# rgl-epfl/large-steps-pytorch

Measured on AMD Instinct MI355X. Metric: from_differential_solves_per_sec, higher is better.
Workload: dtype f32; 1 GPU; cfg4_plane1m: 1000x1000 plane, V=1000000, nnz(M)=6992002, M=I+50*L_uniform, u=M v, k=3, factor once (not timed), re-solve timed; method=nested-dissection, device=AMD Radeon Graphics

## Files before the change

include/largesteps_hip.h:

```cpp
#ifndef LARGESTEPS_HIP_H
#define LARGESTEPS_HIP_H

#include <stddef.h>
#include <stdint.h>

#ifdef __cplusplus
extern "C" {
#endif

#define LS_VERSION 110

#define LS_OK 0
#define LS_E_INVALID (-1)
#define LS_E_INDEX (-2)
#define LS_E_WORKSPACE (-3)
#define LS_E_OVERFLOW (-4)
#define LS_E_STATE (-5)
#define LS_E_NOT_CONVERGED (-6)

#define LS_LAPLACIAN_UNIFORM 0
#define LS_LAPLACIAN_COT 1

int ls_version(void);
const char* ls_last_error(void);

int ls_assemble_workspace_bytes(int64_t V, int64_t F, size_t* h_bytes);
int ls_assemble_pattern(const void* faces, int idx_bytes, int64_t F, int64_t V, const float* verts,
                        int kind, float a, float b, void* workspace, size_t workspace_bytes,
                        int32_t* rowptr, int64_t* h_nnz, int device, void* stream);
int ls_assemble_fill(const void* workspace, size_t workspace_bytes, int64_t V, int64_t F, const int32_t* rowptr,
                     int32_t* col, float* val, int64_t* coo_idx, int64_t nnz, float* dinv, int device,
                     void* stream);

int ls_csr_from_coo(const int64_t* coo_rows, const int64_t* coo_cols, const float* vals, int64_t nnz,
                    int64_t V, int32_t* rowptr, int32_t* col, float* dinv, void* scratch,
                    size_t scratch_bytes, int device, void* stream);

int ls_spmv(const int32_t* rowptr, const int32_t* col, const float* val, int64_t V, int64_t nnz,
            const float* x, float* y, int k, int variant, int device, void* stream);

typedef struct ls_solver ls_solver;

typedef struct ls_solve_info {
    int32_t iterations;
    int32_t converged;
    double  rnorm[4];
    double  bnorm[4];
} ls_solve_info;

int ls_solver_create(const int32_t* rowptr, const int32_t* col, const float* val, int64_t V,
                     int64_t nnz, int kmax, int device, void* stream, ls_solver** h_out);
int ls_solver_destroy(ls_solver* s);
int ls_solver_solve(ls_solver* s, const float* b, const float* x0, float* x, int k, double rtol,
                    double atol, int max_iter, ls_solve_info* h_info, void* stream);
int ls_solver_set_spectrum(ls_solver* s, double a_min);
int ls_solver_set_uniform(ls_solver* s, float a, float b, void* stream);
int ls_solver_spectrum(const ls_solver* s, double* h_lmin, double* h_lmax);
int ls_solver_set_patches(ls_solver* s, const int32_t* h_table, int n_patches, const int32_t* h_ghost_gid, int64_t n_gid,
                          const uint16_t* h_cols16, int64_t n_cols, const float* h_diag, int64_t n_diag,
                          const int32_t* h_perm, int depth, int max_local, int max_rows, void* stream);
int ls_solver_chebyshev_iterations(const ls_solver* s, double reduction, int* h_n);
int ls_solver_solve_chebyshev(ls_solver* s, const float* b, const float* x0, float* x, int k, double rtol,
                              double atol, int max_iter, ls_solve_info* h_info, void* stream);
int ls_solver_set(ls_solver* s, const char* name, int value);
int ls_solver_profile(const ls_solver* s, double* h_ms3, int* h_iters);
int ls_solver_sell(ls_solver* s, const int32_t** h_slice_ptr, const void** h_cv, int64_t* h_entries);
int ls_solver_workspace_bytes(const ls_solver* s, size_t* h_bytes);

int ls_solver_create_ext(const int32_t* rowptr, const int32_t* col, const float* val, int64_t n_rows,
                         int64_t n_cols, int64_t nnz, int kmax, int device, void* stream, ls_solver** h_out);
int ls_solver_phase(ls_solver* s, int phase, const float* b, float* x, int k, double rtol, double atol,
                    int it, void* stream);
int ls_solver_buffers(ls_solver* s, float** h_p, double** h_part, int* h_grid, int* h_part_stride);
int ls_solver_bind(ls_solver* s, float* p_ext, double* part);
int ls_shard_cheb_steps(ls_solver* s, const float* b, float* xa, float* xb, int k, int it0, int nsteps,
                        const float* h_c1, const float* h_c2, int64_t n_rows, void* stream);
int ls_shard_resnorm(ls_solver* s, const float* b, const float* x, int k, int64_t n_rows, void* stream);
int ls_solver_poll(ls_solver* s, int k, int n_enqueued, ls_solve_info* h_info, void* stream);
int ls_gather_rows(const float* src, const int32_t* idx, int64_t n, int k, float* dst, int device, void* stream);

typedef struct ls_patch_plan ls_patch_plan;
int ls_patch_plan_create(int64_t V, const int32_t* h_rowptr, const int32_t* h_col, const float* h_diag, const float* h_positions,
                         int patch_size, int depth, int cap_local, int min_depth, int cap_rows, ls_patch_plan** out);
int ls_patch_plan_destroy(ls_patch_plan* p);
int ls_patch_plan_info(const ls_patch_plan* p, int* n_patches, int* depth, int* max_local, int* max_rows, int* max_width, int64_t* n_gid,
                       int64_t* n_cols, int64_t* n_diag, double* seconds);
int ls_patch_plan_arrays(const ls_patch_plan* p, int32_t* table, int32_t* ghost_gid, uint16_t* cols16, float* diag, int32_t* perm);

typedef struct ls_shard_plan ls_shard_plan;
int ls_shard_plan_create(int64_t V, const int32_t* h_rowptr, const int32_t* h_col, const float* h_val, int P, int rank, int depth,
                         ls_shard_plan** out);
int ls_shard_plan_destroy(ls_shard_plan* s);
int ls_shard_plan_info(const ls_shard_plan* s, int64_t* lo, int64_t* hi, int64_t* n_inner, int64_t* n_ghosts, int64_t* n_entries,
                       int* n_recv, int* n_send, int64_t* n_send_ids);
int ls_shard_plan_arrays(const ls_shard_plan* s, int32_t* rowptr, int32_t* col, float* val, int32_t* ghosts, int32_t* recv3,
                         int32_t* send_ptr, int32_t* send_dst, int32_t* send_ids);
int ls_shard_layer_sizes(int64_t V, const int32_t* h_rowptr, const int32_t* h_col, int64_t lo, int64_t hi, int depth, int64_t* h_sizes);

typedef struct ls_nd_plan ls_nd_plan;
int ls_nd_plan_create(int64_t V, const int32_t* h_rowptr, const int32_t* h_col, const float* h_positions, int leaf_size,
                      int arity, int smooth, ls_nd_plan** out);
int ls_nd_plan_create_device(const int32_t* d_rowptr, const int32_t* d_col, const float* d_positions, int64_t V, int64_t nnz,
                             int leaf_size, int arity, int smooth, int device, void* stream, ls_nd_plan** out);
#define LS_ND_ORDER_AUTO (-1)
#define LS_ND_ORDER_LONGEST 0
#define LS_ND_ORDER_MINSEP 1
int ls_nd_plan_create_ordered(int64_t V, const int32_t* h_rowptr, const int32_t* h_col, const float* h_positions, int leaf_size,
                              int arity, int smooth, int ordering, ls_nd_plan** out);
int ls_nd_plan_create_device_ordered(const int32_t* d_rowptr, const int32_t* d_col, const float* d_positions, int64_t V, int64_t nnz,
                                     int leaf_size, int arity, int smooth, int ordering, int device, void* stream, ls_nd_plan** out);
int ls_nd_plan_quality(const ls_nd_plan* p, int* h_ordering, double* h_words_per_vertex, double* h_spread, double* h_words_other);
int ls_nd_plan_destroy(ls_nd_plan* p);
int ls_nd_plan_info(const ls_nd_plan* p, int* levels, int* arity, int* n_nodes, int64_t* n_bnd, int64_t* n_front, double* seconds);
int ls_nd_plan_arrays(const ls_nd_plan* p, int32_t* perm, int32_t* s, int32_t* b, int32_t* own_start, int32_t* parent,
                      int32_t* bnd, int32_t* ppos, int32_t* push_ptr, int32_t* push_tgt);

typedef struct ls_direct ls_direct;
#define LS_DIRECT_NODE_COLS 12
typedef struct ls_direct_arrays {
    int64_t V;
    int32_t levels, arity;
    const int64_t* h_nodes;
    const int32_t* h_perm;
    const int32_t* h_ppos;
    int64_t n_bnd;
    const int32_t* h_push_ptr;
    const int32_t* h_push_tgt;
    int64_t n_front;
    const float* d_finv;
    const float* d_wf;
    const float* d_wb;
    const float* d_u4;
    const float* d_d4;
    const float* d_tri;
    const int32_t* d_sp_ptr;
    const void* d_sp_ent;
    int64_t n_sp_ptr, n_sp_ent;
    int32_t shard_rank, shard_count;
    int32_t tier_waves;
} ls_direct_arrays;
int ls_direct_create(const ls_direct_arrays* arrays, int device, void* stream, ls_direct** out);
int ls_direct_pick_tree(int64_t V, int* leaf_size, int* arity);
int ls_direct_tier_lds_bytes(int levels, int arity, const int32_t* h_s, const int32_t* h_b, const int32_t* h_own_start, int tier_levels,
                             int sparse_leaves, int waves, size_t* h_bytes);
int ls_direct_factor(const int32_t* d_rowptr, const int32_t* d_col, const float* d_val, int64_t V, int64_t nnz,
                     const float* d_positions, int leaf_size, int arity, int tier_levels, int sparse_leaves, int shard_rank,
                     int shard_count, int device, void* stream, ls_direct** out);
typedef struct ls_direct_options {
    int32_t struct_bytes;
    int32_t leaf_size, arity, tier_levels, sparse_leaves, shard_rank, shard_count;
    int32_t ordering;
    int32_t tier_waves;
} ls_direct_options;
int ls_direct_options_default(ls_direct_options* opt);
int ls_direct_factor_ex(const int32_t* d_rowptr, const int32_t* d_col, const float* d_val, int64_t V, int64_t nnz,
                        const float* d_positions, const ls_direct_options* opt, int device, void* stream, ls_direct** out);
int ls_direct_factor_refactorable(const int32_t* d_rowptr, const int32_t* d_col, const float* d_val, int64_t V, int64_t nnz,
                                  const float* d_positions, const ls_direct_options* opt, int device, void* stream, ls_direct** out);
int ls_direct_refactor(ls_direct* d, const int32_t* d_rowptr, const int32_t* d_col, const float* d_val, int64_t V, int64_t nnz,
                       void* stream);
int ls_direct_refactorable(const ls_direct* d, int* h_yes, size_t* h_retained_device_bytes);
int ls_release_scratch(int device);
int ls_direct_shape(const ls_direct* d, int* h_levels, int* h_arity, int* h_tier_levels, int* h_tier_workgroups,
                    int64_t* h_words_up, int64_t* h_words_down, int64_t* h_n_bnd);
int ls_direct_level_words(const ls_direct* d, int cap, int64_t* h_up, int64_t* h_down);
int ls_direct_level_rows(const ls_direct* d, int cap, int64_t* h_rows, int64_t* h_bnd);
int ls_direct_level_index_bytes(const ls_direct* d, int cap, int64_t* h_up, int64_t* h_down);
int ls_direct_tier_balance(const ls_direct* d, double* h_words4);
int ls_direct_launch_profile(const ls_direct* d, int cap, int* h_n, double* h_ms, int64_t* h_words, int32_t* h_level_lo,
                             int32_t* h_level_hi, int32_t* h_sweep);
int ls_direct_plan_quality(const ls_direct* d, int* h_ordering, double* h_words_per_vertex, double* h_spread, double* h_words_other);
int ls_direct_factor_seconds(const ls_direct* d, double* h_s3);
int ls_csr_is_symmetric(const int32_t* d_rowptr, const int32_t* d_col, const float* d_val, int64_t V, int64_t nnz, float tol,
                        int* h_symmetric, int device, void* stream);
int ls_direct_destroy(ls_direct* d);
int ls_direct_solve(ls_direct* d, const float* b, float* x, int k, void* stream);
int ls_direct_solve_part(ls_direct* d, const float* b, float* x, int k, int part, float* exchange, void* stream);
int ls_direct_shard_info(const ls_direct* d, int* h_rank, int* h_count, int* h_cut_level, int64_t* h_exchange_floats_per_column,
                         unsigned char* h_owned_rows);
int ls_direct_exchange_region(ls_direct* d, int k, float** h_region, int64_t* h_floats);

typedef struct ls_dist ls_dist;
int ls_dist_unique_id(void* h_id128);
int ls_dist_create(const void* h_id128, int rank, int world, int device, ls_dist** out);
int ls_dist_destroy(ls_dist* c);
int ls_dist_allreduce_sum(ls_dist* c, float* d_buf, int64_t n, void* stream);
int ls_dist_info(const ls_dist* c, int* h_rank, int* h_world);
int ls_dist_direct_solve(ls_dist* c, ls_direct* d, const float* b, float* x, int k, void* stream);
int ls_direct_set(ls_direct* d, const char* name, int value);
int ls_direct_info(const ls_direct* d, int64_t* h_factor_entries, int* h_launches, double* h_ms3);

int ls_remove_duplicates_workspace_bytes(int64_t V, size_t* h_bytes);
int ls_remove_duplicates(const float* verts, int64_t V, const void* faces, int idx_bytes, int64_t F, float* unique_verts,
                         int64_t* inverse, int64_t* new_faces, int64_t* h_n_unique, void* workspace, size_t ws_bytes, int device,
                         void* stream);

int ls_csr_transpose_workspace_bytes(int64_t V, int64_t nnz, size_t* h_bytes);
int ls_csr_transpose(const int32_t* rowptr, const int32_t* col, const float* val, int64_t V, int64_t nnz, int32_t* t_rowptr,
                     int32_t* t_col, float* t_val, void* workspace, size_t ws_bytes, int device, void* stream);
int ls_corner_ranks_workspace_bytes(int64_t F, int64_t V, size_t* h_bytes);
int ls_corner_ranks(const void* faces, int idx_bytes, int64_t F, int64_t V, int32_t* vptr, int32_t* cpos, void* workspace,
                    size_t ws_bytes, int device, void* stream);

int ls_normals_workspace_bytes(int64_t F, int64_t V, size_t* h_bytes);
int ls_face_normals(const float* verts, const void* faces, int idx_bytes, int64_t F, int64_t V, float* fn, int device, void* stream);
int ls_face_normals_backward(const float* verts, const void* faces, int idx_bytes, int64_t F, int64_t V, const int32_t* vptr,
                             const int32_t* cpos, const float* g_fn, float* grad_verts, void* workspace, size_t ws_bytes,
                             int device, void* stream);
int ls_vertex_normals(const float* verts, const void* faces, int idx_bytes, int64_t F, int64_t V, const int32_t* vptr,
                      const int32_t* cpos, const float* fn, float* out, float* raw, float* norms, void* workspace,
                      size_t ws_bytes, int device, void* stream);
int ls_vertex_normals_backward(const float* verts, const void* faces, int idx_bytes, int64_t F, int64_t V, const int32_t* vptr,
                               const int32_t* cpos, const float* fn, const float* raw, const float* norms, const float* g_out,
                               float* grad_verts, float* grad_fn, void* workspace, size_t ws_bytes, int device, void* stream);
int ls_face_normals_with_norms(const float* verts, const void* faces, int idx_bytes, int64_t F, int64_t V, float* fn, float* norms,
                               void* workspace, size_t ws_bytes, int device, void* stream);
int ls_vertex_normals_from_norms(const float* verts, const void* faces, int idx_bytes, int64_t F, int64_t V, const int32_t* vptr,
                                 const int32_t* cpos, const float* norms, float* out, float* raw, void* workspace, size_t ws_bytes,
                                 int device, void* stream);
int ls_vertex_normals_gathered(const float* verts, const void* faces, int idx_bytes, int64_t F, int64_t V, const int32_t* vptr,
                               const int32_t* order, const float* norms, float* out, float* raw, int device, void* stream);
int ls_normals_pair_backward_faces(const float* verts, const void* faces, int idx_bytes, int64_t F, int64_t V, const float* raw,
                                   const float* norms, const float* g_out, float* g_raw, float* gN, float* grad_fn, void* workspace,
                                   size_t ws_bytes, int device, void* stream);
int ls_normals_pair_backward_verts(const float* verts, const void* faces, int idx_bytes, int64_t F, int64_t V, const int32_t* vptr,
                                   const int32_t* cpos, const float* norms, const float* g_raw, const float* gN, const float* g_fn,
                                   float* grad_verts, void* workspace, size_t ws_bytes, int device, void* stream);

int ls_meshgeom_workspace_bytes(int64_t F, int64_t V, size_t* h_bytes);
int ls_massmatrix_voronoi(const float* verts, const void* faces, int idx_bytes, int64_t F, int64_t V, const int32_t* vptr,
                          const int32_t* order, float* mass, int device, void* stream);
int ls_massmatrix_voronoi_backward(const float* verts, const void* faces, int idx_bytes, int64_t F, int64_t V, const int32_t* vptr,
                                   const int32_t* cpos, const float* g_mass, float* grad_verts, void* workspace, size_t ws_bytes,
                                   int device, void* stream);
int ls_average_edge_length(const float* verts, const void* faces, int idx_bytes, int64_t F, int64_t V, float* out, void* workspace,
                           size_t ws_bytes, int device, void* stream);
int ls_average_edge_length_backward(const float* verts, const void* faces, int idx_bytes, int64_t F, int64_t V, const int32_t* vptr,
                                    const int32_t* cpos, const float* g_out, float* grad_verts, void* workspace, size_t ws_bytes,
                                    int device, void* stream);

#define LS_REMESH_SPLIT 0
#define LS_REMESH_COLLAPSE 1
#define LS_REMESH_FLIP 2
#define LS_REMESH_RELAX 3
#define LS_REMESH_PROJECT 4
int ls_remesh_create(const float* verts, int64_t V, const void* faces, int idx_bytes, int64_t F, float h, int project, int device,
                     void* stream, void** handle);
int ls_remesh_run(void* handle, int iterations);
int ls_remesh_phase(void* handle, int phase, int max_rounds);
int ls_remesh_info(void* handle, int64_t* V, int64_t* F, int64_t* counters, double* seconds);
int ls_remesh_copy_out(void* handle, float* verts, void* faces, int idx_bytes);
int ls_remesh_destroy(void* handle);

int ls_mesh_distance_create(const float* verts, int64_t V, const void* faces, int idx_bytes, int64_t F, int device, void* stream,
                            void** handle);
int ls_mesh_distance_query(void* handle, const float* P, int64_t n, double* sqrD, int64_t* I, double* C, void* stream);
int ls_mesh_distance_max(void* handle, const float* P, int64_t n, double* out_sqd, void* stream);
int ls_mesh_distance_destroy(void* handle);
int ls_mesh_distance_weights(void* handle, const float* P, int64_t n, const int64_t* I, double* W, void* stream);
int ls_mesh_distance_backward_workspace_bytes(int64_t n, int64_t F, size_t* bytes);
int ls_mesh_distance_backward(void* handle, const float* P, int64_t n, const int64_t* I, const double* C, const double* g,
                              const int32_t* vptr, const int32_t* corner_order, float* gP, float* gV, void* ws, size_t ws_bytes,
                              void* stream);
int ls_mesh_distance_update(void* handle, const float* verts, void* stream);

int ls_adam_uniform_step(float* param, const float* grad, float* g1, float* g2, int64_t n, float lr,
                         float beta1, float beta2, int step, void* scratch, int device, void* stream);
int ls_adam_uniform_step_device(float* param, const float* grad, float* g1, float* g2, int64_t n, float lr, float beta1,
                                float beta2, int32_t* d_step, void* scratch, int device, void* stream);

int ls_raster_workspace_bytes(int64_t B, int64_t F, int H, int W, int C, size_t* bytes);
int ls_raster_forward(const float* pos, int64_t B, int64_t V, const int32_t* tri, int64_t F, int H, int W, float* rast, void* ws,
                      size_t ws_bytes, int device, void* stream);
int ls_raster_pixel_order(const float* rast, int64_t B, int64_t F, int H, int W, int32_t* order, int32_t* seg, void* ws, size_t ws_bytes,
                          int device, void* stream);
int ls_raster_backward(const float* pos, int64_t B, int64_t V, const int32_t* tri, int64_t F, int H, int W, const float* grad_rast,
                       const int32_t* order, const int32_t* seg, const int32_t* vptr, const int32_t* corner_order, float* grad_pos,
                       void* ws, size_t ws_bytes, int device, void* stream);
int ls_raster_interpolate(const float* attr, int64_t attr_batch, int64_t V, int C, const float* rast, int64_t B, int H, int W,
                          const int32_t* tri, int64_t F, float* out, int device, void* stream);
int ls_raster_interpolate_backward(const float* attr, int64_t attr_batch, int64_t V, int C, const float* rast, int64_t B, int H, int W,
                                   const int32_t* tri, int64_t F, const float* grad_out, const int32_t* order, const int32_t* seg,
                                   const int32_t* vptr, const int32_t* corner_order, float* grad_attr, float* grad_rast, void* ws,
                                   size_t ws_bytes, int device, void* stream);
int ls_raster_adjacency_workspace_bytes(int64_t F, size_t* bytes);
int ls_raster_adjacency(const int32_t* tri, int64_t F, int32_t* adj, void* ws, size_t ws_bytes, int device, void* stream);
int ls_raster_antialias(const float* color, int C, const float* rast, const float* pos, int64_t B, int64_t V, int H, int W,
                        const int32_t* tri, int64_t F, const int32_t* adj, float* out, int device, void* stream);
int ls_raster_antialias_backward(const float* color, int C, const float* rast, const float* pos, int64_t B, int64_t V, int H, int W,
                                 const int32_t* tri, int64_t F, const int32_t* adj, const float* grad_out, float boost,
                                 const int32_t* order, const int32_t* seg, const int32_t* vptr, const int32_t* corner_order,
                                 float* grad_color, float* grad_pos, void* ws, size_t ws_bytes, int device, void* stream);

#define LS_TEXTURE_NEAREST 0
#define LS_TEXTURE_LINEAR 1
#define LS_TEXTURE_WRAP 0
#define LS_TEXTURE_CLAMP 1
#define LS_TEXTURE_ZERO 2
int ls_texture_workspace_bytes(int64_t B, int H, int W, size_t* bytes);
int ls_texture_forward(const float* tex, int64_t Bt, int Ht, int Wt, int C, const float* uv, int64_t B, int H, int W, int filter,
                       int boundary, float* out, int device, void* stream);
int ls_texture_order(const float* uv, int64_t B, int H, int W, int64_t Bt, int Ht, int Wt, int filter, int boundary, int32_t* order,
                     int32_t* seg, void* ws, size_t ws_bytes, int device, void* stream);
int ls_texture_backward(const float* tex, int64_t Bt, int Ht, int Wt, int C, const float* uv, int64_t B, int H, int W, int filter,
                        int boundary, const float* grad_out, const int32_t* order, const int32_t* seg, float* grad_tex, float* grad_uv,
                        int device, void* stream);

#define LS_MIP_NEAREST 0
#define LS_MIP_LINEAR 1
int ls_mip_workspace_bytes(int64_t B, int H, int W, size_t* bytes);
int ls_mip_build(const float* tex, int64_t Bt, int Ht, int Wt, int C, int Lmax, float* pyr, int device, void* stream);
int ls_mip_fold(float* grad_tex, int64_t Bt, int Ht, int Wt, int C, int Lmax, float* grad_pyr, int device, void* stream);
int ls_mip_pixel_differentials(const float* rast, const float* pos, int64_t B, int64_t V, const int32_t* tri, int64_t F, int H, int W,
                               float* out, int device, void* stream);
int ls_mip_interpolate_da(const float* attr, int64_t attr_batch, int64_t V, int C, const float* rast, const float* rast_db, int64_t B,
                          int H, int W, const int32_t* tri, int64_t F, float* out, int device, void* stream);
int ls_mip_forward(const float* tex, const float* pyr, int64_t Bt, int Ht, int Wt, int C, int Lmax, const float* uv, const float* uv_da,
// ... 13 lines not shown
```

large-steps-pytorch_amd/csrc/direct.hip:

```cpp
#include "common.h"
#include <vector>
#include <chrono>
#include <algorithm>
#include <atomic>
#include <string.h>
#include <memory>
#include <mutex>

namespace ls {

struct alignas(64) Tile {
    int store;
    int row0, s, b, own_start, bnd_off, front_off;
    int leaf;
    int pfront_off, cix;
    int forward;
    int arity;
    long long finv_off, w_off;
};

static_assert(sizeof(Tile) == 64, "Tile layout");
__device__ __forceinline__ Tile load_tile(const Tile* __restrict__ tiles, int idx) {
    const int lane = threadIdx.x & 63;
    const int w = lane < 16 ? reinterpret_cast<const int*>(tiles)[(size_t)idx * 16 + lane] : 0;
// ... 565 lines not shown
        const size_t g = perm ? (size_t)perm[first + r] : (size_t)(first + r);
        float v[K];
#pragma unroll
        for (int q = 0; q < K; ++q) v[q] = b_in[g * K + q];
        if (!t.leaf) {
            const size_t f = (size_t)(t.d[h].front_off + j);
            float raw[A * K], u[K];
            load_slots<K, A>(slots, f, raw);
            sum_slots<K, A>(raw, mask[f], u);
#pragma unroll
            for (int q = 0; q < K; ++q) v[q] -= u[q];
        }
#pragma unroll
        for (int q = 0; q < K; ++q) { sb[r * K + q] = v[q]; bprime[(size_t)(first + r) * K + q] = v[q]; }
    }
}

template <int K>
__global__ __launch_bounds__(64) void k_nd_up_p(const PackedTile* __restrict__ tiles, const int* __restrict__ perm,
                                                const unsigned char* __restrict__ mask, const int* __restrict__ ppos,
                                                const float* __restrict__ wf, const float* __restrict__ b_in,
                                                float* __restrict__ bprime, float* slots) {
    extern __shared__ __attribute__((aligned(16))) float sm[];
    float* sb = sm;
    const PackedTile& t = tiles[blockIdx.x];
    const int lane = threadIdx.x;
    const bool row = lane < t.row0[t.n];
    const int g = find_group(t.row0, t.n, lane);
    const NodeP d = t.d[g];
    const int i = lane - t.row0[g];
    const float* __restrict__ col = wf + d.w_off + (row ? i : 0);
    float pre[LS_ND_UNROLL];
    prefetch_strided<false>(col, (size_t)d.b, 0, row ? d.s : 0, pre);
    int pp = 0;
    float pass[K];
#pragma unroll
    for (int q = 0; q < K; ++q) pass[q] = 0.0f;
    if (row) {
        pp = ppos[d.bnd_off + i];
        if (!t.leaf) pull_slots<K>(slots, mask, (size_t)(d.front_off + d.s + i), t.arity, pass);
    }
    if (t.arity == 4) packed_fill<K, 4>(t, perm, mask, slots, b_in, bprime, sb);
    else if (t.arity == 2) packed_fill<K, 2>(t, perm, mask, slots, b_in, bprime, sb);
    else packed_fill<K, 8>(t, perm, mask, slots, b_in, bprime, sb);
    __syncthreads();
    if (row) {
        float acc[K];
#pragma unroll
        for (int q = 0; q < K; ++q) acc[q] = 0.0f;
        dot_strided<K, false>(col, (size_t)d.b, 0, d.s, sb + (size_t)t.sb0[g] * K, pre, acc);
        const size_t dst = ((size_t)(d.pfront_off + pp) * t.arity + d.cix) * K;
#pragma unroll
        for (int q = 0; q < K; ++q) slots[dst + q] = acc[q] + pass[q];
    }
}

template <int K>
__global__ __launch_bounds__(64) void k_nd_down_p(const PackedTile* __restrict__ tiles, const int* __restrict__ perm,
                                                  const int* __restrict__ push_ptr, const int* __restrict__ push_tgt,
                                                  const float* __restrict__ finv, const float* __restrict__ wb,
                                                  const float* __restrict__ bprime, float* xb, float* __restrict__ x_out, int s_sum_cap) {
    extern __shared__ __attribute__((aligned(16))) float sm[];
    float* sb = sm;
    float* sx = sm + (size_t)s_sum_cap * K;
    const PackedTile& t = tiles[blockIdx.x];
    const int lane = threadIdx.x;
    const bool row = lane < t.row0[t.n];
    const int g = find_group(t.row0, t.n, lane);
    const NodeP d = t.d[g];
    const int j = lane - t.row0[g];
    const float* __restrict__ fcol = finv + d.finv_off + (row ? j : 0);
    const float* __restrict__ wcol = wb + d.w_off + (row ? j : 0);
    float pre_f[LS_ND_UNROLL], pre_w[LS_ND_UNROLL];
    prefetch_strided<false>(fcol, (size_t)d.s, 0, row ? d.s : 0, pre_f);
    prefetch_strided<false>(wcol, (size_t)d.s, 0, row ? d.b : 0, pre_w);
    int p0 = 0, p1 = 0;
    size_t gx = 0;
    if (row) {
        gx = (size_t)perm[d.own_start + j];
        if (!t.leaf) { p0 = push_ptr[d.front_off + j]; p1 = push_ptr[d.front_off + j + 1]; }
    }
    const int S = t.sb0[t.n], B = t.sx0[t.n], first = t.d[0].own_start, bfirst = t.d[0].bnd_off;
    for (int r = threadIdx.x; r < S; r += blockDim.x) {
#pragma unroll
        for (int q = 0; q < K; ++q) sb[r * K + q] = bprime[(size_t)(first + r) * K + q];
    }
    for (int r = threadIdx.x; r < B; r += blockDim.x) {
#pragma unroll
        for (int q = 0; q < K; ++q) sx[r * K + q] = -xb[(size_t)(bfirst + r) * K + q];
    }
    __syncthreads();
    if (!t.leaf) {
        for (int r = threadIdx.x; r < B; r += blockDim.x) {
            const int h = find_group(t.sx0, t.n, r);
            const size_t f = (size_t)(t.d[h].front_off + t.d[h].s + (r - t.sx0[h]));
            const int q0 = push_ptr[f], q1 = push_ptr[f + 1];
            float v[K];
#pragma unroll
            for (int q = 0; q < K; ++q) v[q] = -sx[r * K + q];
            push_down<K>(push_tgt, q0, q1, xb, v);
        }
    }
    if (row) {
        float acc[K];
#pragma unroll
        for (int q = 0; q < K; ++q) acc[q] = 0.0f;
        dot_strided<K, false>(fcol, (size_t)d.s, 0, d.s, sb + (size_t)t.sb0[g] * K, pre_f, acc);
        dot_strided<K, false>(wcol, (size_t)d.s, 0, d.b, sx + (size_t)t.sx0[g] * K, pre_w, acc);
#pragma unroll
        for (int q = 0; q < K; ++q) x_out[gx * K + q] = acc[q];
        push_down<K>(push_tgt, p0, p1, xb, acc);
    }
}

}
#include "nd_tier.h"
namespace ls {

struct LevelPlan { int up_first = 0, up_tiles = 0, up_nw = 1, down_first = 0, down_tiles = 0, down_nw = 1, s_cap = 0, b_cap = 0, up_b = 0, down_b = 0, up_chunks = 1, down_chunks = 1, up_s = 0,
                   up_p = 0, down_p = 0, up_p_first = 0, up_p_tiles = 0, down_p_first = 0, down_p_tiles = 0, up_p_lds = 0, down_p_s = 0, down_p_lds = 0; };

}

using namespace ls;

namespace ls {
struct RefactorState;
void refactor_state_free(RefactorState* R);
size_t refactor_state_bytes(const RefactorState* R);
int refactor_run(RefactorState* R, const int32_t* d_rowptr, const int32_t* d_col, const float* d_val, int64_t V, int64_t nnz, hipStream_t st,
                 bool* touched);
}

struct ls_direct {
    int device = 0, levels = 0, arity = 2, n_nodes = 0, kmax = 4;
    int64_t V = 0, n_bnd = 0, n_front = 0;
    int *perm = nullptr, *ppos = nullptr, *push_ptr = nullptr, *push_tgt = nullptr;
    unsigned char* mask = nullptr;
    Tile* tiles = nullptr;
    PackedTile* ptiles = nullptr;
    const float *finv = nullptr, *wf = nullptr, *wb = nullptr;
    const float *u4 = nullptr, *d4 = nullptr;
    const float* tri = nullptr;
    const int* sp_ptr = nullptr;
    const SpEnt* sp_ent = nullptr;
    float* braw = nullptr;
    float *bp = nullptr, *slots = nullptr, *xb = nullptr;
    int upper_lo = 0;
    int tier_root = 0, tier_phases = 0, tier_wgs = 0, tier_region = 0, tier_vec = 0, tier_tri = 0, tier_waves = TIER_WAVES;
    TierItem* d_items = nullptr;
    int* pull = nullptr;
    int64_t pull_base = 0;
    TierWG* d_wgs = nullptr;
    hipEvent_t busy = nullptr;
    hipStream_t last_stream = nullptr;
    bool used = false;
    std::vector<std::pair<void*, size_t>> tables;
    ls::RefactorState* refac = nullptr;
    bool factored = true;
    int shard_rank = 0, shard_count = 1, cut = 0;
    int64_t exch_f0 = 0, exch_f1 = 0;
    std::vector<unsigned char> owned_rows;
    bool nt_levels = false, nt_tier = false, nt_rule[2] = {false, false};
    double factor_s[3] = {0, 0, 0};
    double plan_q[4] = {0, 0, 0, 0};
    std::vector<LevelPlan> plan;
    int64_t factor_entries = 0, words_up = 0, words_down = 0;
    int profile = 0;
    std::vector<hipEvent_t> ev;
    struct LaunchMeta { int lo, hi, sweep; };
    std::vector<hipEvent_t> lev;
    std::vector<LaunchMeta> lmeta;
    std::vector<double> launch_ms;
    std::vector<int64_t> lvl_up, lvl_down;
    std::vector<int64_t> lvl_rows, lvl_bnd;
    std::vector<int64_t> lvl_idx_up, lvl_idx_down;
    double tier_balance[4] = {0, 0, 0, 0};
    double prof_ms[3] = {0, 0, 0};
#ifdef LS_TIER_STAMPS
    long long* stamps = nullptr;
#endif
};

static int pick_nw(int len, int target) {
    int nw = 1;
    while (nw < 16 && len > nw * target) nw *= 2;
    return nw;
}

namespace ls {
hipStream_t side_stream(int device, int which) {
    static std::mutex mu;
    static hipStream_t streams[64][2] = {{nullptr, nullptr}};
    if (device < 0 || device >= 64 || which < 0 || which > 1) return nullptr;
    std::lock_guard<std::mutex> lk(mu);
    if (!streams[device][which]) {
        DeviceGuard dg(device);
        if (dg.err != hipSuccess || hipStreamCreateWithFlags(&streams[device][which], hipStreamNonBlocking) != hipSuccess) streams[device][which] = nullptr;
    }
    return streams[device][which];
}
namespace {
struct DevicePool {
    std::mutex mu;
    struct Entry { void* p; size_t bytes; int device; };
    std::vector<Entry> held;
    static size_t cap(int device) {
        double gb = env_pool_gb();
        if (!(gb > 0.0)) return 0;
        static std::mutex mu;
        static double total_gb[64];
        double t = 0.0;
        if (device >= 0 && device < 64) {
            std::lock_guard<std::mutex> lk(mu);
            if (total_gb[device] == 0.0) {
                size_t free_b = 0, total_b = 0;
                DeviceGuard dg(device);
                total_gb[device] = (hipMemGetInfo(&free_b, &total_b) == hipSuccess && total_b) ? (double)total_b / 1073741824.0 : -1.0;
            }
            t = total_gb[device];
        }
        if (t > 0.0) gb = std::min(gb, t / 4.0);
        return (size_t)(gb * 1073741824.0);
    }
};
DevicePool g_pool;
}

void* pool_take(int device, size_t bytes, size_t* capacity) {
    if (bytes < POOL_FROM) return nullptr;
    std::lock_guard<std::mutex> g(g_pool.mu);
    int best = -1;
    for (int i = 0; i < (int)g_pool.held.size(); ++i) {
        const DevicePool::Entry& e = g_pool.held[(size_t)i];
        if (e.device == device && e.bytes >= bytes && e.bytes <= bytes + bytes / 2 + POOL_SLACK && (best < 0 || e.bytes < g_pool.held[(size_t)best].bytes)) best = i;
    }
    if (best < 0) return nullptr;
    void* p = g_pool.held[(size_t)best].p;
    if (capacity) *capacity = g_pool.held[(size_t)best].bytes;
    g_pool.held.erase(g_pool.held.begin() + best);
    return p;
}

bool pool_give(int device, void* p, size_t bytes) {
    if (!p || bytes < POOL_FROM) return false;
    const size_t limit = DevicePool::cap(device);
    if (bytes > limit) return false;
    std::lock_guard<std::mutex> g(g_pool.mu);
    size_t total = bytes;
    for (const DevicePool::Entry& e : g_pool.held) if (e.device == device) total += e.bytes;
    size_t count = 1;
    for (const DevicePool::Entry& e : g_pool.held) if (e.device == device) ++count;
    for (size_t i = 0; (total > limit || count > 512) && i < g_pool.held.size();) {
        if (g_pool.held[i].device != device) { ++i; continue; }
        --count;
        total -= g_pool.held[i].bytes;
        DeviceGuard dg(device);
        (void)hipFree(g_pool.held[i].p);
        g_pool.held.erase(g_pool.held.begin() + (long)i);
    }
    g_pool.held.push_back(DevicePool::Entry{p, bytes, device});
    return true;
}

std::atomic<long long> g_malloc_calls{0}, g_malloc_us{0}, g_malloc_bytes{0};
hipError_t pool_alloc(int device, void** p, size_t bytes) {
    const auto t0 = std::chrono::steady_clock::now();
    hipError_t e = hipMalloc(p, bytes);
    g_malloc_calls += 1; g_malloc_bytes += (long long)bytes;
    g_malloc_us += (long long)std::chrono::duration<double, std::micro>(std::chrono::steady_clock::now() - t0).count();
    if (e != hipErrorOutOfMemory && e != hipErrorMemoryAllocation) return e;
    (void)hipGetLastError();
    (void)ls_release_scratch(device);
    return hipMalloc(p, bytes);
}
}

extern "C" int ls_release_scratch(int device) {
    std::lock_guard<std::mutex> g(ls::g_pool.mu);
    for (size_t i = 0; i < ls::g_pool.held.size();) {
        if (device < 0 || ls::g_pool.held[i].device == device) {
            ls::DeviceGuard dg(ls::g_pool.held[i].device);
            (void)hipFree(ls::g_pool.held[i].p);
            ls::g_pool.held.erase(ls::g_pool.held.begin() + (long)i);
        } else ++i;
    }
    return LS_OK;
}

static size_t plan_tier(const std::vector<NodeD>& nd, const std::vector<int64_t>& level_off, int levels, int arity, int root, int64_t q_lo,
                        int64_t q_hi, std::vector<TierItem>& items, std::vector<TierWG>& wgs, int& vec_floats, int& tri_floats, int waves = TIER_WAVES) {
    const int H = levels - root;
    items.clear(); wgs.assign((size_t)(q_hi - q_lo), TierWG());
    int vec_need = 0, pbuf_need = 0, leaf_need = 0, tri_cap = 0;
    for (int64_t i = level_off[levels - 1]; i < level_off[levels]; ++i)
        if (nd[i].flags & NODE_SPARSE) {
            const int sc = (nd[i].s + 15) & ~15;
            tri_cap = std::max(tri_cap, (sc * (sc + 1) / 2 + 3) & ~3);
        }
    tri_floats = tri_cap;
    for (int64_t q = q_lo; q < q_hi; ++q) {
        TierWG& g = wgs[(size_t)(q - q_lo)];
        g.up_split = g.down_split = g.up_leaf = g.down_leaf = 0;
        g.n_dense = 0; g.pad = 0;
        for (int t = 0; t < 2 * TIER_MAX_H; ++t) g.dense_rng[t] = 0;
        for (int lv = root, t = 0; lv < levels - 1; ++lv, ++t) {
            int64_t span = 1;
            for (int u = root; u < lv; ++u) span *= arity;
            const int64_t first = level_off[lv] + q * span;
            int lo = -1, hi = -1;
            for (int64_t i = first; i < first + span; ++i)
                if (!(nd[i].flags & NODE_SPARSE) && nd[i].s > 0) { if (lo < 0) lo = nd[i].own_start; hi = nd[i].own_start + nd[i].s; }
            if (lo >= 0) { g.dense_rng[2 * t] = lo; g.dense_rng[2 * t + 1] = hi - lo; g.n_dense += hi - lo; }
        }
        for (int sweep = 0; sweep < 2; ++sweep) {
            const bool up = sweep == 0;
            int* off = up ? g.up_off : g.down_off;
            for (int ph = 0; ph < H; ++ph) {
                off[ph] = (int)items.size();
                const int lv = up ? levels - 1 - ph : root + ph;
                int64_t span = 1;
                for (int t = root; t < lv; ++t) span *= arity;
                const int64_t first = level_off[lv] + q * span;
                int base = 0;
                bool sparse = false;
                for (int64_t i = first; i < first + span; ++i) {
                    const NodeD& n = nd[i];
                    if (n.flags & NODE_SPARSE) { sparse = true; continue; }
                    if (n.s == 0 && n.b == 0) continue;
                    base += std::max(1, div_up(up ? n.b : n.s, WAVE));
                }
                bool all_sparse = span > 0;
                for (int64_t i = first; i < first + span; ++i) {
                    const NodeD& n = nd[i];
                    if (!(n.flags & NODE_SPARSE) && (n.s || n.b)) all_sparse = false;
                    TierItem it;
                    memset(&it, 0, sizeof(it));
                    it.s = n.s; it.b = n.b; it.own_start = n.own_start; it.bnd_off = n.bnd_off; it.front_off = n.front_off;
                    it.pfront_off = n.pfront_off; it.cix = n.cix; it.flags = n.flags | (lv > root ? NODE_UPC : 0); it.finv_off = n.finv_off; it.w_off = n.w_off;
                    it.spb_off = n.spb_off; it.sps_off = n.sps_off; it.nparts = 1;
                    if (n.flags & NODE_SPARSE) {
                        items.push_back(it);
                        leaf_need = std::max(leaf_need, std::max(tri_cap, (4 * n.b + 3) & ~3) + 256);
                        continue;
                    }
                    if (n.s == 0 && n.b == 0) continue;
                    const int rows = up ? n.b : n.s, L = up ? ((n.s + 3) & ~3) : ((n.s + 3) & ~3) + ((n.b + 3) & ~3);
                    int nparts = 1;
                    if (!sparse && base < waves) nparts = std::max(1, std::min(waves / std::max(base, 1), L / 16));
                    for (int r = 0; r < std::max(rows, 1); r += WAVE)
                        for (int pt = 0; pt < nparts; ++pt) {
                            it.row0 = r; it.r0 = (int)((int64_t)(L / 4) * pt / nparts) * 4; it.r1 = (int)((int64_t)(L / 4) * (pt + 1) / nparts) * 4;
                            it.part = pt; it.nparts = nparts;
                            items.push_back(it);
                            vec_need = std::max(vec_need, 4 * (it.r1 - it.r0 + 32));
                        }
                    if (nparts > 1) { if (up) g.up_split |= 1u << ph; else g.down_split |= 1u << ph; }
                }
                if (all_sparse) { if (up) g.up_leaf |= 1u << ph; else g.down_leaf |= 1u << ph; }
                else if (sparse) return 0;
                const int n_items = (int)items.size() - off[ph];
                if (((up ? g.up_split : g.down_split) >> ph) & 1u) pbuf_need = std::max(pbuf_need, div_up(n_items, waves) * 256);
            }
            off[H] = (int)items.size();
        }
    }
    vec_floats = (vec_need + 3) & ~3;
    return (size_t)std::max(vec_floats + pbuf_need, leaf_need);
}


static size_t direct_tier_lds(int levels, int arity, const int* s, const int* b, const int* own_start, int tier_levels, bool sparse_leaves, int waves) {
    std::vector<int64_t> level_off((size_t)levels + 1);
    int64_t cnt = 1, off = 1;
    for (int lv = 0; lv <= levels; ++lv) { level_off[lv] = off; off += cnt; cnt *= arity; }
    const int64_t n_nodes = level_off[levels] - 1;
    std::vector<NodeD> nd((size_t)n_nodes + 1);
    memset(nd.data(), 0, nd.size() * sizeof(NodeD));
    const int root = levels - tier_levels;
    for (int lv = root; lv < levels; ++lv)
        for (int64_t i = level_off[lv]; i < level_off[lv + 1]; ++i) {
            NodeD& q = nd[(size_t)i];
            q.s = s[i]; q.b = b[i]; q.own_start = own_start[i];
            const bool sparse = sparse_leaves && lv == levels - 1 && q.s >= 1;
            q.flags = (lv + 1 >= levels ? NODE_LEAF : 0) | (sparse ? NODE_SPARSE : NODE_QUAD);
        }
    std::vector<TierItem> items;
    std::vector<TierWG> wgs;
    int vec = 0, tri = 0;
    const size_t region = plan_tier(nd, level_off, levels, arity, root, 0, level_off[root + 1] - level_off[root], items, wgs, vec, tri, waves);
    return region ? ((region + 3) & ~(size_t)3) * sizeof(float) * waves : 0;
}

bool direct_tier_fits(int levels, int arity, const int* s, const int* b, const int* own_start, int tier_levels, bool sparse_leaves, int waves) {
    if (tier_levels <= 0) return true;
    if (tier_levels > levels || tier_levels > TIER_MAX_H) return false;
    const size_t bytes = direct_tier_lds(levels, arity, s, b, own_start, tier_levels, sparse_leaves, waves);
    return bytes && bytes <= (size_t)(waves == TIER_WAVES_FULL ? TIER_LDS_FULL : TIER_LDS);
}

extern "C" int ls_direct_tier_lds_bytes(int levels, int arity, const int32_t* h_s, const int32_t* h_b, const int32_t* h_own_start, int tier_levels,
                                        int sparse_leaves, int waves, size_t* h_bytes) {
    LS_REQUIRE(h_s && h_b && h_own_start && h_bytes && levels >= 1 && levels <= 30 && (arity == 2 || arity == 4 || arity == 8) &&
               tier_levels >= 1 && tier_levels <= levels && tier_levels <= TIER_MAX_H && (waves == TIER_WAVES || waves == TIER_WAVES_WIDE || waves == TIER_WAVES_FULL),
               LS_E_INVALID, "ls_direct_tier_lds_bytes: bad argument (1 <= tier_levels <= min(levels, %d); waves 4, 8 or 16)", TIER_MAX_H);
    *h_bytes = direct_tier_lds(levels, arity, h_s, h_b, h_own_start, tier_levels, sparse_leaves != 0, waves);
    return LS_OK;
}

bool direct_tier_full16(int64_t V, int arity, int levels, int tier_levels, int shard_count, int tier_waves) {
    if (tier_waves == TIER_WAVES_FULL) return tier_levels >= 2;
    if (tier_waves == TIER_WAVES || tier_waves == TIER_WAVES_WIDE) return false;
    return shard_count <= 1 && arity == 4 && levels >= 8 && V >= 800000 && tier_levels == levels - 4 && tier_levels <= TIER_MAX_H;
}


namespace {
struct CreatePlan {
    int levels = 0, arity = 0, cut = 0;
    int64_t sub_lo = 0, sub_hi = 1;
    std::vector<int64_t> level_off;
    std::vector<NodeD> nd;
    std::vector<int> parent;
    std::vector<unsigned char> mask;
    std::vector<TierItem> items;
    std::vector<TierWG> wgs;
    std::vector<int> pull;
    std::vector<Tile> tiles;
    std::vector<PackedTile> ptiles;
    int64_t span(int from, int to) const { int64_t s = 1; for (int t = from; t < to; ++t) s *= arity; return s; }
    bool active(int64_t i, int lv) const {
        if (lv < cut) return true;
        int64_t q = i - level_off[lv];
        for (int t = cut; t < lv; ++t) q /= arity;
        return q >= sub_lo && q < sub_hi;
    }
};

int read_nodes(const ls_direct_arrays* A, CreatePlan& T, ls_direct* d) {
    const int levels = T.levels, n_nodes = d->n_nodes;
    T.nd.assign((size_t)n_nodes + 1, NodeD());
    T.parent.assign((size_t)n_nodes + 1, 0);
    d->lvl_up.assign((size_t)levels, 0); d->lvl_down.assign((size_t)levels, 0); d->lvl_rows.assign((size_t)levels, 0); d->lvl_bnd.assign((size_t)levels, 0);
    int64_t fe = 0, fe_up = 0, fe_down = 0;
    for (int i = 1; i <= n_nodes; ++i) {
        const int64_t* r = A->h_nodes + (size_t)i * LS_DIRECT_NODE_COLS;
        NodeD& n = T.nd[i];
        n.s = (int)r[0]; n.b = (int)r[1]; n.own_start = (int)r[2]; n.bnd_off = (int)r[3]; n.front_off = (int)r[4];
        n.finv_off = r[5]; n.w_off = r[6];
        const int parent = T.parent[i] = (int)r[7];
        const bool sparse = r[8] >= 0, quad = r[11] != 0;
        if (n.s < 0 || n.b < 0 || n.own_start < 0 || (int64_t)n.own_start + n.s > d->V || (int64_t)n.bnd_off + n.b > d->n_bnd ||
            (int64_t)n.front_off + n.s + n.b > d->n_front || (i == 1 ? n.b != 0 : (parent < 1 || parent >= i)) ||
            (sparse && (i < T.level_off[levels - 1] || n.s > 64 || n.s < 1 || !A->d_tri || !A->d_sp_ptr || !A->d_sp_ent || (r[8] & 3))) ||
            (quad && (sparse || !A->d_u4 || !A->d_d4 || (n.finv_off & 3) || (n.w_off & 3)))) {
            set_error("ls_direct_create: node %d of the plan is inconsistent", i);
            return LS_E_INVALID;
        }
        const int64_t s4 = (n.s + 3) & ~3, b4 = (n.b + 3) & ~3, tri_w = ((int64_t)n.s * (n.s + 1) / 2 + 3) & ~(int64_t)3;
        const int64_t up_w = sparse ? tri_w : quad ? s4 * n.b : (int64_t)n.s * n.b;
        const int64_t down_w = sparse ? tri_w : quad ? (s4 + b4) * n.s : (int64_t)n.s * n.s + (int64_t)n.s * n.b;
        fe += up_w + down_w; fe_up += up_w; fe_down += down_w;
        int lv = 0;
        while (lv + 1 < levels && i >= T.level_off[lv + 1]) ++lv;
        d->lvl_up[(size_t)lv] += up_w; d->lvl_down[(size_t)lv] += down_w;
        d->lvl_rows[(size_t)lv] += n.s; d->lvl_bnd[(size_t)lv] += n.b;
        n.pfront_off = i > 1 ? T.nd[parent].front_off : -1;
        n.cix = lv ? (int)((i - T.level_off[lv]) % T.arity) : 0;
        n.flags = (lv + 1 >= levels ? NODE_LEAF : 0) | (sparse ? NODE_SPARSE : 0) | (quad ? NODE_QUAD : 0);
        if (sparse) n.finv_off = r[8];
        n.spb_off = (int)r[9]; n.sps_off = (int)r[10];
    }
    fe += 2 * A->n_sp_ent + A->n_sp_ptr;
    fe_up += A->n_sp_ent + A->n_sp_ptr / 2; fe_down += A->n_sp_ent + A->n_sp_ptr - A->n_sp_ptr / 2;
    d->lvl_up[(size_t)levels - 1] += A->n_sp_ent + A->n_sp_ptr / 2; d->lvl_down[(size_t)levels - 1] += A->n_sp_ent + A->n_sp_ptr - A->n_sp_ptr / 2;
    d->factor_entries = fe; d->words_up = fe_up; d->words_down = fe_down;
    {
        const double mb = 4e-6 * (double)fe;
        d->nt_rule[0] = d->nt_levels = mb > 256.0;
        d->nt_rule[1] = d->nt_tier = mb > 400.0;
    }
    for (int lv = 1; lv < levels; ++lv)
        for (int64_t i = T.level_off[lv]; i < T.level_off[lv + 1]; ++i) {
            const NodeD &n = T.nd[i], &p = T.nd[T.parent[i]];
            for (int k = 0; k < n.b; ++k) {
                const int pp = A->h_ppos[n.bnd_off + k];
                if (pp < 0 || pp >= p.s + p.b) {
                    set_error("ls_direct_create: ppos out of range at node %lld", (long long)i);
                    return LS_E_INVALID;
                }
                T.mask[(size_t)p.front_off + pp] |= (unsigned char)(1u << n.cix);
            }
        }
    return LS_OK;
}

int choose_tier(CreatePlan& T, const int32_t* h_ppos, int tier_waves, const NdEnv& env, ls_direct* d) {
    const int levels = T.levels;
    int root = levels;
    for (int lv = levels - 1; lv >= 0; --lv) {
        bool tiered = false, plain = false;
        for (int64_t i = T.level_off[lv]; i < T.level_off[lv + 1]; ++i) {
            if (T.nd[i].s == 0 && T.nd[i].b == 0) continue;
            if (T.nd[i].flags & (NODE_SPARSE | NODE_QUAD)) tiered = true; else plain = true;
        }
        if (tiered && plain) { set_error("ls_direct_create: level %d mixes tier-layout and plain nodes", lv); return LS_E_INVALID; }
        if (plain) break;
        if (tiered && root != lv + 1) { set_error("ls_direct_create: tier-layout levels must be the deepest ones"); return LS_E_INVALID; }
        if (tiered) root = lv;
    }
    for (int lv = 0; lv < root; ++lv)
        for (int64_t i = T.level_off[lv]; i < T.level_off[lv + 1]; ++i)
            if (T.nd[i].flags & (NODE_SPARSE | NODE_QUAD)) { set_error("ls_direct_create: tier-layout node above the tier"); return LS_E_INVALID; }
    d->tier_root = levels;
    if (root == levels) return LS_OK;
    const int H = levels - root;
    if (T.cut > root) { set_error("ls_direct_create: %d ranks need a cut below the tier's root level (tree too small)", d->shard_count); return LS_E_INVALID; }
    const int64_t span = T.span(T.cut, root), q_lo = T.sub_lo * span, q_hi = T.sub_hi * span;
    size_t region = 0;
    auto take_if_fits = [&](int waves, int budget) {
        std::vector<TierItem> items;
        std::vector<TierWG> wgs;
        int vec = 0, tri = 0;
        const size_t r = plan_tier(T.nd, T.level_off, levels, T.arity, root, q_lo, q_hi, items, wgs, vec, tri, waves);
        if (!r || ((r + 3) & ~(size_t)3) * sizeof(float) * waves > (size_t)budget) return;
        T.items.swap(items); T.wgs.swap(wgs); d->tier_vec = vec; d->tier_tri = tri; region = r; d->tier_waves = waves;
    };
    if (H <= TIER_MAX_H && direct_tier_full16(d->V, T.arity, levels, H, d->shard_count, tier_waves > 0 ? tier_waves : env.tier_waves.value_or(0)))
        take_if_fits(TIER_WAVES_FULL, TIER_LDS_FULL);
    if (!region) {
        region = H <= TIER_MAX_H ? plan_tier(T.nd, T.level_off, levels, T.arity, root, q_lo, q_hi, T.items, T.wgs, d->tier_vec, d->tier_tri) : 0;
        if (!region || region * sizeof(float) * TIER_WAVES > TIER_LDS) {
            set_error("ls_direct_create: a tier of %d levels does not fit the kernel (LDS per wave: %zu floats)", H, region);
            return LS_E_WORKSPACE;
        }
        if (H >= 2 && (int)T.wgs.size() <= 768 && (tier_waves > 0 ? tier_waves : env.tier_waves.value_or(TIER_WAVES_WIDE)) == TIER_WAVES_WIDE)
            take_if_fits(TIER_WAVES_WIDE, TIER_LDS_WIDE);
    }
    d->tier_root = root; d->tier_phases = H; d->tier_wgs = (int)T.wgs.size(); d->tier_region = (int)((region + 3) & ~(size_t)3);
    d->pull_base = T.nd[T.level_off[root]].front_off;
    T.pull.assign((size_t)std::max<int64_t>(0, T.nd[T.level_off[levels - 1]].front_off - d->pull_base) * T.arity, -1);
    for (int lv = root + 1; lv < levels; ++lv)
        for (int64_t i = T.level_off[lv]; i < T.level_off[lv + 1]; ++i) {
            const NodeD& n = T.nd[i];
            for (int k = 0; k < n.b; ++k) T.pull[(size_t)(n.pfront_off - d->pull_base + h_ppos[n.bnd_off + k]) * T.arity + n.cix] = n.bnd_off + k;
        }
    return LS_OK;
}

size_t plan_level(CreatePlan& T, int lv, int long_up, const NdEnv& env, int kmax, LevelPlan& p) {
    std::vector<Tile>& tiles = T.tiles;
    int64_t a0 = T.level_off[lv], a1 = T.level_off[lv + 1];
    if (lv >= T.cut) { const int64_t span = T.span(T.cut, lv); a0 = T.level_off[lv] + T.sub_lo * span; a1 = T.level_off[lv] + T.sub_hi * span; }
    auto tile_of = [&](int64_t i, int r, int forward) {
        const NodeD& n = T.nd[i];
        Tile t;
        t.store = 0; t.row0 = r; t.s = n.s; t.b = n.b; t.own_start = n.own_start; t.bnd_off = n.bnd_off; t.front_off = n.front_off;
        t.leaf = lv + 1 >= T.levels; t.pfront_off = n.pfront_off; t.cix = n.cix;
        t.forward = forward; t.arity = T.arity; t.finv_off = n.finv_off; t.w_off = n.w_off;
        return t;
    };
    int red_up = 0, red_down = 0;
    for (int64_t i = a0; i < a1; ++i) {
        p.s_cap = std::max(p.s_cap, T.nd[i].s); p.b_cap = std::max(p.b_cap, T.nd[i].b);
        red_up = std::max(red_up, T.nd[i].s); red_down = std::max(red_down, T.nd[i].s + T.nd[i].b);
    }
    p.up_b = red_up >= long_up; p.down_b = red_down >= env.long_red;
    const int up_bw = std::min(ND_BW, red_up >= 1400 ? 8 : 4), down_bw = std::min(ND_BW, red_down >= 1400 ? 8 : 4);
    p.up_nw = p.up_b ? up_bw : pick_nw(red_up, 32); p.down_nw = p.down_b ? down_bw : pick_nw(red_down, env.steps);
    int64_t rows_up = 0, rows_down = 0;
    for (int64_t i = a0; i < a1; ++i) { rows_up += T.nd[i].b; rows_down += T.nd[i].s; }
    auto pick_chunks = [&](int64_t rows, int bw) {
        int c = 4;
        while (c > 1 && rows / (ND_ROWS * bw * c) < 500) --c;
        return c;
    };
    p.up_chunks = pick_chunks(rows_up, up_bw);
    p.down_chunks = pick_chunks(rows_down, down_bw);
    const int up_rows = p.up_b ? ND_ROWS * up_bw * p.up_chunks : WAVE, down_rows = p.down_b ? ND_ROWS * down_bw * p.down_chunks : WAVE;
    const size_t up_s_bytes = ((size_t)p.s_cap * p.b_cap + (size_t)p.s_cap * kmax) * sizeof(float);
    p.up_s = p.b_cap <= 256 && p.s_cap <= 256 && up_s_bytes <= 40 * 1024 && !env.no_small;
    if (p.up_s) { p.up_b = 0; p.up_nw = std::max(1, div_up(p.b_cap, WAVE)); }
    p.up_p = !env.no_pack && p.b_cap <= WAVE && p.s_cap <= 256 && lv > 0;
    p.down_p = !env.no_pack && p.s_cap <= WAVE / 2;
    auto pack_level = [&](bool up_sweep, int& first, int& count, int& lds_rows_s, int& lds_rows_b) {
        first = (int)T.ptiles.size();
        lds_rows_s = lds_rows_b = 0;
        int64_t i = a0;
        while (i < a1) {
            PackedTile t;
            memset(&t, 0, sizeof(t));
            t.leaf = lv + 1 >= T.levels; t.arity = T.arity;
            int rows = 0;
            while (i < a1 && t.n < ND_PACK) {
                const NodeD& nd = T.nd[i];
                const int r = up_sweep ? nd.b : nd.s;
                if (t.n && rows + r > WAVE) break;
                NodeP& q = t.d[t.n];
                q.s = nd.s; q.b = nd.b; q.own_start = nd.own_start; q.bnd_off = nd.bnd_off; q.front_off = nd.front_off;
                q.pfront_off = nd.pfront_off; q.cix = nd.cix; q.pad = 0; q.finv_off = nd.finv_off; q.w_off = nd.w_off;
                t.row0[t.n + 1] = t.row0[t.n] + r;
                t.sb0[t.n + 1] = t.sb0[t.n] + nd.s;
                t.sx0[t.n + 1] = t.sx0[t.n] + nd.b;
                rows += r; ++t.n; ++i;
            }
            for (int c = t.n + 1; c <= ND_PACK; ++c) { t.row0[c] = t.row0[t.n]; t.sb0[c] = t.sb0[t.n]; t.sx0[c] = t.sx0[t.n]; }
            lds_rows_s = std::max(lds_rows_s, t.sb0[t.n]); lds_rows_b = std::max(lds_rows_b, t.sx0[t.n]);
            T.ptiles.push_back(t);
        }
        count = (int)T.ptiles.size() - first;
    };
    int dummy = 0;
    if (p.up_p) { pack_level(true, p.up_p_first, p.up_p_tiles, p.up_p_lds, dummy); p.up_s = 0; p.up_b = 0; }
    if (p.down_p) { pack_level(false, p.down_p_first, p.down_p_tiles, p.down_p_s, p.down_p_lds); p.down_b = 0; }
    p.up_first = (int)tiles.size();
    const int up_threads = WAVE * p.up_nw;
    std::vector<int> up_nodes;
    for (int64_t i = a0; i < a1; ++i) {
        const bool store_tiles = !p.up_s && T.nd[i].s > 2 * up_threads;
        const int rows = std::max(T.nd[i].b, (T.nd[i].s && !store_tiles) ? 1 : 0);
        for (int r = 0; r < rows; r += (p.up_s ? 1 << 30 : up_rows)) {
            tiles.push_back(tile_of(i, r, 0));
            tiles.back().store = (r == 0 && !store_tiles) ? 1 : 0;
            up_nodes.push_back((int)(i - a0));
        }
        if (store_tiles)
            for (int r = 0; r < T.nd[i].s; r += up_threads) { tiles.push_back(tile_of(i, r, 0)); tiles.back().store = 2; up_nodes.push_back((int)(i - a0)); }
    }
    auto xcd_order = [&](int first, std::vector<int>& node_of_tile) {
        const int n = (int)tiles.size() - first;
        if (a1 - a0 < 8 || n < 16) return;
        std::vector<std::vector<Tile>> bucket(8);
        for (int t = 0; t < n; ++t) bucket[(size_t)(node_of_tile[(size_t)t] & 7)].push_back(tiles[(size_t)(first + t)]);
        size_t longest = 0;
        for (auto& bk : bucket) longest = std::max(longest, bk.size());
        Tile idle;
        memset(&idle, 0, sizeof(idle));
        idle.store = 3; idle.forward = 2;
        tiles.resize((size_t)first);
        for (size_t r = 0; r < longest; ++r)
            for (int x = 0; x < 8; ++x) tiles.push_back(r < bucket[(size_t)x].size() ? bucket[(size_t)x][r] : idle);
    };
    xcd_order(p.up_first, up_nodes);
    p.up_tiles = (int)tiles.size() - p.up_first;
    p.down_first = (int)tiles.size();
    std::vector<int> down_nodes;
    for (int64_t i = a0; i < a1; ++i)
        for (int r = 0; r < T.nd[i].s; r += down_rows) { tiles.push_back(tile_of(i, r, 0)); down_nodes.push_back((int)(i - a0)); }
    if (lv + 1 < T.levels)
        for (int64_t i = a0; i < a1; ++i)
            for (int r = 0; r < T.nd[i].b; r += WAVE * p.down_nw) { tiles.push_back(tile_of(i, r, 1)); down_nodes.push_back((int)(i - a0)); }
    xcd_order(p.down_first, down_nodes);
    p.down_tiles = (int)tiles.size() - p.down_first;
    return ((size_t)p.s_cap + p.b_cap + 16 * WAVE) * kmax * sizeof(float);
}

void account_index_bytes(const CreatePlan& T, ls_direct* d) {
    const int levels = T.levels, arity = T.arity;
    d->lvl_idx_up.assign((size_t)levels, 0); d->lvl_idx_down.assign((size_t)levels, 0);
    std::vector<int64_t> fpos((size_t)levels, 0), bsum((size_t)levels + 1, 0);
    for (int lv = 0; lv < levels; ++lv)
        for (int64_t i = T.level_off[lv]; i < T.level_off[lv + 1]; ++i)
            if (T.active(i, lv)) { fpos[(size_t)lv] += T.nd[i].s + T.nd[i].b; bsum[(size_t)lv] += T.nd[i].b; }
    for (int lv = 0; lv < d->tier_root; ++lv) {
        const LevelPlan& p = d->plan[lv];
        d->lvl_idx_up[(size_t)lv] = (p.up_p ? (int64_t)p.up_p_tiles * (int64_t)sizeof(PackedTile) : (int64_t)p.up_tiles * (int64_t)sizeof(Tile)) + fpos[(size_t)lv] + 4 * bsum[(size_t)lv];
        d->lvl_idx_down[(size_t)lv] = (p.down_p ? (int64_t)p.down_p_tiles * (int64_t)sizeof(PackedTile) : (int64_t)p.down_tiles * (int64_t)sizeof(Tile)) + 4 * fpos[(size_t)lv] +
                                      4 * bsum[(size_t)lv + 1];
    }
    if (d->tier_root >= levels) return;
    const int H = levels - d->tier_root;
    for (const TierWG& g : T.wgs)
        for (int ph = 0; ph < H; ++ph) {
            d->lvl_idx_up[(size_t)(levels - 1 - ph)] += (int64_t)(g.up_off[ph + 1] - g.up_off[ph]) * (int64_t)sizeof(TierItem);
            d->lvl_idx_down[(size_t)(d->tier_root + ph)] += (int64_t)(g.down_off[ph + 1] - g.down_off[ph]) * (int64_t)sizeof(TierItem);
        }
    d->lvl_idx_up[(size_t)d->tier_root] += (int64_t)T.wgs.size() * (int64_t)sizeof(TierWG);
    d->lvl_idx_down[(size_t)d->tier_root] += (int64_t)T.wgs.size() * (int64_t)sizeof(TierWG);
    for (int lv = d->tier_root; lv < levels; ++lv) {
        const bool inner = lv + 1 < levels;
        if (inner) d->lvl_idx_up[(size_t)lv] += 4 * (int64_t)arity * fpos[(size_t)lv];
        if (lv == d->tier_root || !inner) d->lvl_idx_up[(size_t)lv] += 4 * bsum[(size_t)lv];
        if (inner) d->lvl_idx_down[(size_t)lv] += 4 * fpos[(size_t)lv] + 4 * bsum[(size_t)lv + 1];
    }
    const int64_t q0 = T.sub_lo * T.span(T.cut, d->tier_root);
    double mx[2] = {0, 0}, sum[2] = {0, 0};
    for (size_t w = 0; w < T.wgs.size(); ++w) {
        double wu = 0, wd = 0;
        int64_t span = 1;
        for (int lv = d->tier_root; lv < levels; ++lv) {
            const int64_t first = T.level_off[lv] + (q0 + (int64_t)w) * span;
            for (int64_t i = first; i < first + span; ++i) {
                const NodeD& n = T.nd[i];
                const double s4 = (n.s + 3) & ~3, b4 = (n.b + 3) & ~3, tri_w = ((int64_t)n.s * (n.s + 1) / 2 + 3) & ~(int64_t)3;
                if (n.flags & NODE_SPARSE) { wu += tri_w + 3.0 * n.b; wd += tri_w + 3.0 * n.b; }
                else { wu += s4 * n.b; wd += (s4 + b4) * n.s; }
            }
            span *= arity;
        }
        mx[0] = std::max(mx[0], wu); mx[1] = std::max(mx[1], wd); sum[0] += wu; sum[1] += wd;
    }
    const double nw = (double)std::max<size_t>(T.wgs.size(), 1);
    d->tier_balance[0] = mx[0]; d->tier_balance[1] = sum[0] / nw; d->tier_balance[2] = mx[1]; d->tier_balance[3] = sum[1] / nw;
}

}

extern "C" int ls_direct_create(const ls_direct_arrays* A, int device, void* stream, ls_direct** out) {
    LS_REQUIRE(A && out, LS_E_INVALID, "ls_direct_create: null argument");
    LS_REQUIRE(A->tier_waves == 0 || A->tier_waves == TIER_WAVES || A->tier_waves == TIER_WAVES_WIDE || A->tier_waves == TIER_WAVES_FULL, LS_E_INVALID,
               "ls_direct_create: tier_waves must be 0 (library's rule), 4, 8 or 16");
    const int64_t V = A->V, n_bnd = A->n_bnd, n_front = A->n_front;
    const int levels = A->levels, arity = A->arity;
    LS_REQUIRE(A->h_nodes && A->h_perm && A->h_push_ptr && V > 0 && levels >= 1 && levels <= 30 && n_bnd >= 0 && n_front >= V &&
               (arity == 2 || arity == 4 || arity == 8), LS_E_INVALID, "ls_direct_create: bad argument");
    LS_REQUIRE(V < INT32_MAX && n_bnd < INT32_MAX && n_front * arity < INT32_MAX, LS_E_OVERFLOW, "ls_direct_create: plan exceeds int32 offsets");
    *out = nullptr;
    CreatePlan T{levels, arity};
    T.level_off.resize((size_t)levels + 1);
    {
        int64_t cnt = 1, off = 1;
        for (int lv = 0; lv <= levels; ++lv) {
            T.level_off[lv] = off; off += cnt; cnt *= arity;
            LS_REQUIRE(off < ((int64_t)1 << 30), LS_E_OVERFLOW, "ls_direct_create: tree too large");
        }
    }
    DeviceGuard g(device);
    LS_HIP(g.err);
    hipStream_t st = (hipStream_t)stream;
    const bool timing = env_plan_timing();
    const NdEnv env = nd_env();
    const auto t_create = std::chrono::steady_clock::now();
    auto lap = [&](const char* what) { if (timing) fprintf(stderr, "[ls_direct_create] %-28s %.2f ms\n", what, std::chrono::duration<double, std::milli>(std::chrono::steady_clock::now() - t_create).count()); };
    std::unique_ptr<ls_direct, int (*)(ls_direct*)> d(new ls_direct(), ls_direct_destroy);
    d->device = device; d->levels = levels; d->arity = arity; d->n_nodes = (int)(T.level_off[levels] - 1); d->V = V; d->n_bnd = n_bnd; d->n_front = n_front;
    d->finv = A->d_finv; d->wf = A->d_wf; d->wb = A->d_wb;
    d->u4 = A->d_u4; d->d4 = A->d_d4;
    d->tri = A->d_tri; d->sp_ptr = A->d_sp_ptr; d->sp_ent = (const SpEnt*)A->d_sp_ent;
    const int n_ranks = std::max(1, (int)A->shard_count), rank = std::min(std::max(0, (int)A->shard_rank), n_ranks - 1);
    int cut = 0;
    while (cut + 1 < levels && T.level_off[cut + 1] - T.level_off[cut] < n_ranks) ++cut;
    if (n_ranks == 1) cut = 0;
    const int64_t n_sub = T.level_off[cut + 1] - T.level_off[cut];
    T.sub_lo = n_sub * rank / n_ranks; T.sub_hi = n_sub * (rank + 1) / n_ranks;
    d->shard_rank = rank; d->shard_count = n_ranks; d->cut = T.cut = cut;
    T.mask.assign((size_t)n_front, 0);
    int rc = LS_OK;
    if ((rc = read_nodes(A, T, d.get())) || (rc = choose_tier(T, A->h_ppos, A->tier_waves, env, d.get()))) return rc;
    d->upper_lo = (d->tier_root < levels && d->tier_root > 0) ? T.nd[T.level_off[d->tier_root - 1]].own_start : (int)V;
    d->plan.resize(levels);
    size_t lds_max = 0;
    const int long_up = env.long_up > 0 ? env.long_up : levels >= 8 ? 256 : 64;
    for (int lv = 0; lv < d->tier_root; ++lv) lds_max = std::max(lds_max, plan_level(T, lv, long_up, env, d->kmax, d->plan[lv]));
    account_index_bytes(T, d.get());
    if (lds_max > LEVEL_LDS) {
        set_error("ls_direct_create: a front needs %zu bytes of LDS (separator too large for this kernel)", lds_max);
        return LS_E_INVALID;
    }
    if (n_ranks > 1 && cut >= 1) {
        d->exch_f0 = T.nd[T.level_off[cut - 1]].front_off;
        d->exch_f1 = T.nd[T.level_off[cut]].front_off;
    }
    if (n_ranks > 1) {
        d->owned_rows.assign((size_t)V, 0);
        for (int lv = 0; lv < levels; ++lv)
            for (int64_t i = T.level_off[lv]; i < T.level_off[lv + 1]; ++i)
                if (lv < cut ? rank == 0 : T.active(i, lv))
                    for (int r = 0; r < T.nd[i].s; ++r) d->owned_rows[(size_t)A->h_perm[T.nd[i].own_start + r]] = 1;
    }
    lap("tables built (host)");
    hipStream_t su = side_stream(device, 0);
    LS_REQUIRE(su, LS_E_STATE, "ls_direct_create: no side stream on this device");
    auto table = [&](void** dst, size_t bytes) -> hipError_t {
        size_t cap = bytes;
        *dst = pool_take(device, bytes, &cap);
        if (!*dst) { const hipError_t e = pool_alloc(device, dst, bytes); if (e != hipSuccess) return e; }
        d->tables.emplace_back(*dst, cap);
        return hipSuccess;
    };
    auto up = [&](auto** dst, const auto* src, size_t n) -> int {
        LS_HIP(table((void**)dst, std::max<size_t>(n, 1) * sizeof(**dst)));
        if (n) LS_HIP(hipMemcpyAsync(*dst, src, n * sizeof(**dst), hipMemcpyHostToDevice, su));
        return LS_OK;
    };
    if ((rc = up(&d->tiles, T.tiles.data(), T.tiles.size())) || (rc = up(&d->ptiles, T.ptiles.data(), T.ptiles.size())) ||
        (rc = up(&d->perm, A->h_perm, (size_t)V)) ||
        (rc = up(&d->ppos, A->h_ppos, (size_t)n_bnd)) || (rc = up(&d->push_ptr, A->h_push_ptr, (size_t)n_front + 1)) ||
        (rc = up(&d->push_tgt, A->h_push_tgt, (size_t)n_bnd)) || (rc = up(&d->mask, T.mask.data(), T.mask.size())) ||
        (rc = up(&d->d_items, T.items.data(), T.items.size())) || (rc = up(&d->pull, T.pull.data(), T.pull.size())) ||
        (rc = up(&d->d_wgs, T.wgs.data(), T.wgs.size())))
        return rc;
    hipError_t e = table((void**)&d->bp, sizeof(float) * (size_t)V * d->kmax);
    if (e == hipSuccess) e = table((void**)&d->braw, sizeof(float) * (size_t)V * d->kmax);
    if (e == hipSuccess) e = table((void**)&d->slots, sizeof(float) * (size_t)n_front * d->arity * d->kmax);
    if (e == hipSuccess) e = table((void**)&d->xb, sizeof(float) * (size_t)std::max<int64_t>(n_bnd, 1) * d->kmax);
    if (e == hipSuccess) e = hipEventCreateWithFlags(&d->busy, hipEventDisableTiming);
    lap("uploads enqueued, vectors allocated");
    if (e == hipSuccess) e = hipEventRecord(d->busy, su);
    if (e == hipSuccess) e = hipStreamWaitEvent(st, d->busy, 0);
    if (e == hipSuccess) e = hipStreamSynchronize(su);
    lap("uploads done");
    if (e != hipSuccess) return hip_fail(e, "ls_direct_create allocations", __FILE__, __LINE__);
    static const void* const kernels[] = {
#define LS_OPTIN(KK)                                                                                                                \
        (const void*)k_nd_up<KK, false>, (const void*)k_nd_down<KK, false>, (const void*)k_nd_up_b<KK, false>,                      \
        (const void*)k_nd_down_b<KK, false>, (const void*)k_nd_up<KK, true>, (const void*)k_nd_down<KK, true>,                      \
        (const void*)k_nd_up_b<KK, true>, (const void*)k_nd_down_b<KK, true>, (const void*)k_nd_up_s<KK>,
        LS_OPTIN(1) LS_OPTIN(2) LS_OPTIN(3) LS_OPTIN(4)
#undef LS_OPTIN
#define LS_OPTIN(KK)                                                                                                                \
        (const void*)k_nd_tier<KK, true, TIER_WAVES, false>, (const void*)k_nd_tier<KK, false, TIER_WAVES, false>,                  \
        (const void*)k_nd_tier<KK, true, TIER_WAVES, true>, (const void*)k_nd_tier<KK, false, TIER_WAVES, true>,                    \
        (const void*)k_nd_tier<KK, true, TIER_WAVES_WIDE, false>, (const void*)k_nd_tier<KK, false, TIER_WAVES_WIDE, false>,        \
        (const void*)k_nd_tier<KK, true, TIER_WAVES_FULL, false>, (const void*)k_nd_tier<KK, false, TIER_WAVES_FULL, false>,        \
        (const void*)k_nd_tier<KK, true, TIER_WAVES_FULL, true>, (const void*)k_nd_tier<KK, false, TIER_WAVES_FULL, true>,
        LS_OPTIN(1) LS_OPTIN(2) LS_OPTIN(3) LS_OPTIN(4)
#undef LS_OPTIN
    };
    for (const void* k : kernels) (void)hipFuncSetAttribute(k, hipFuncAttributeMaxDynamicSharedMemorySize, LDS_OPTIN);
    lap("kernel attributes set");
    *out = d.release();
    return LS_OK;
}

extern "C" int ls_direct_destroy(ls_direct* d) {
    if (!d) return LS_OK;
    DeviceGuard g(d->device);
    if (d->busy) (void)hipEventDestroy(d->busy);
    if (!d->tables.empty()) (void)hipDeviceSynchronize();
    for (const auto& t : d->tables)
        if (!ls::pool_give(d->device, t.first, t.second)) (void)hipFree(t.first);
    ls::refactor_state_free(d->refac);
    for (hipEvent_t e : d->ev) (void)hipEventDestroy(e);
#ifdef LS_TIER_STAMPS
    if (d->stamps) (void)hipFree(d->stamps);
#endif
    for (hipEvent_t e : d->lev) (void)hipEventDestroy(e);
    delete d;
    return LS_OK;
}

template <int K>
static int direct_solve_k(ls_direct* d, const float* b, float* x, hipStream_t st, int part, float* exchange) {
    const int top = d->tier_root - 1;
    TierArgs ta;
    ta.items = d->d_items; ta.wgs = d->d_wgs; ta.perm = d->perm; ta.mask = d->mask; ta.ppos = d->ppos;
    ta.pull = d->pull ? d->pull - (size_t)d->pull_base * d->arity : nullptr; ta.push_ptr = d->push_ptr; ta.push_tgt = d->push_tgt; ta.u4 = d->u4; ta.d4 = d->d4; ta.tri = d->tri;
    ta.sp_ptr = d->sp_ptr; ta.sp_ent = d->sp_ent; ta.bprime = d->bp; ta.braw = d->braw; ta.slots = d->slots; ta.xb = d->xb;
    ta.arity = d->arity; ta.phases = d->tier_phases; ta.region_floats = d->tier_region; ta.vec_floats = d->tier_vec;
    ta.upper_lo = d->upper_lo; ta.upper_hi = (int)d->V;
#ifdef LS_TIER_STAMPS
    const size_t stamp_n = (size_t)d->tier_wgs * d->tier_waves * TIER_STAMP_SLOTS;
    if (d->profile == 2 && !d->stamps && stamp_n) LS_HIP(hipMalloc((void**)&d->stamps, 2 * stamp_n * sizeof(long long)));
    if (d->profile == 2 && d->stamps) LS_HIP(hipMemsetAsync(d->stamps, 0, 2 * stamp_n * sizeof(long long), st));
    ta.stamps = d->profile == 2 ? d->stamps : nullptr;
#endif
    const size_t tier_lds = (size_t)d->tier_region * d->tier_waves * sizeof(float);
    const bool nt_tier = d->nt_tier && d->tier_waves != TIER_WAVES_WIDE, nt = d->nt_levels;
    int n_mark = 0;
    auto mark = [&](int lo, int hi, int sweep) -> hipError_t {
        if (d->profile != 3) return hipSuccess;
        while ((int)d->lev.size() <= n_mark + 1) { hipEvent_t e; const hipError_t r = hipEventCreate(&e); if (r != hipSuccess) return r; d->lev.push_back(e); }
        if ((int)d->lmeta.size() <= n_mark) d->lmeta.resize((size_t)n_mark + 1);
        d->lmeta[(size_t)n_mark] = {lo, hi, sweep};
        return hipEventRecord(d->lev[(size_t)n_mark++], st);
    };
    auto mark_end = [&]() -> hipError_t {
        if (d->profile != 3) return hipSuccess;
        hipError_t r = hipEventRecord(d->lev[(size_t)n_mark], st);
        if (r == hipSuccess) r = hipStreamSynchronize(st);
        d->launch_ms.assign((size_t)n_mark, 0.0);
        d->lmeta.resize((size_t)n_mark);
        for (int i = 0; i < n_mark && r == hipSuccess; ++i) { float ms = 0; r = hipEventElapsedTime(&ms, d->lev[(size_t)i], d->lev[(size_t)i + 1]); d->launch_ms[(size_t)i] = ms; }
        return r;
    };
    const size_t exch_off = (size_t)d->exch_f0 * d->arity * K, exch_n = (size_t)(d->exch_f1 - d->exch_f0) * d->arity * K;
    if (part != 1) {
    if (d->profile) LS_HIP(hipEventRecord(d->ev[0], st));
    if (part == 0 && exch_n) LS_HIP(hipMemsetAsync(d->slots + exch_off, 0, exch_n * sizeof(float), st));
    if (d->tier_wgs) {
        LS_HIP(mark(d->tier_root, d->levels - 1, 0));
        if (d->tier_waves == TIER_WAVES_FULL && nt_tier) hipLaunchKernelGGL((k_nd_tier<K, true, TIER_WAVES_FULL, true>), dim3(d->tier_wgs), dim3(WAVE * TIER_WAVES_FULL), tier_lds, st, ta, b, x, d->tier_tri);
        else if (d->tier_waves == TIER_WAVES_FULL) hipLaunchKernelGGL((k_nd_tier<K, true, TIER_WAVES_FULL, false>), dim3(d->tier_wgs), dim3(WAVE * TIER_WAVES_FULL), tier_lds, st, ta, b, x, d->tier_tri);
        else if (d->tier_waves == TIER_WAVES_WIDE) hipLaunchKernelGGL((k_nd_tier<K, true, TIER_WAVES_WIDE, false>), dim3(d->tier_wgs), dim3(WAVE * TIER_WAVES_WIDE), tier_lds, st, ta, b, x, d->tier_tri);
        else if (nt_tier) hipLaunchKernelGGL((k_nd_tier<K, true, TIER_WAVES, true>), dim3(d->tier_wgs), dim3(WAVE * TIER_WAVES), tier_lds, st, ta, b, x, d->tier_tri);
        else hipLaunchKernelGGL((k_nd_tier<K, true, TIER_WAVES, false>), dim3(d->tier_wgs), dim3(WAVE * TIER_WAVES), tier_lds, st, ta, b, x, d->tier_tri);
    }
    }
    if (part == 1 && exch_n && exchange != d->slots + exch_off)
        LS_HIP(hipMemcpyAsync(d->slots + exch_off, exchange, exch_n * sizeof(float), hipMemcpyDeviceToDevice, st));
    const int* up_perm = d->tier_wgs ? nullptr : d->perm;
    const float* up_b = d->tier_wgs ? d->braw : b;
    const bool fuse_root = top >= 0 && !d->plan[0].down_p;
    const RootFill rf = fuse_root ? RootFill{up_perm, d->mask, d->slots, up_b} : RootFill{nullptr, nullptr, nullptr, nullptr};
    for (int lv = (part == 1 ? std::min(top, d->cut - 1) : top); lv >= (part == 0 ? d->cut : 0); --lv) {
        const LevelPlan& p = d->plan[lv];
        if (!(p.up_p ? p.up_p_tiles : p.up_tiles)) continue;
        if (lv == 0 && fuse_root) continue;
        LS_HIP(mark(lv, lv, 0));
        if (p.up_p)
            hipLaunchKernelGGL(k_nd_up_p<K>, dim3(p.up_p_tiles), dim3(WAVE), (size_t)std::max(p.up_p_lds, 1) * K * sizeof(float), st,
                               d->ptiles + p.up_p_first, up_perm, d->mask, d->ppos, d->wf, up_b, d->bp, d->slots);
        else if (p.up_s)
            hipLaunchKernelGGL(k_nd_up_s<K>, dim3(p.up_tiles), dim3(WAVE * p.up_nw), ((size_t)p.s_cap * p.b_cap + (size_t)p.s_cap * K) * sizeof(float), st,
                               d->tiles + p.up_first, up_perm, d->mask, d->ppos, d->wf, up_b, d->bp, d->slots, p.s_cap, p.b_cap);
        else if (p.up_b)
            hipLaunchKernelGGL((nt ? k_nd_up_b<K, true> : k_nd_up_b<K, false>), dim3(p.up_tiles), dim3(WAVE * p.up_nw), ((size_t)p.s_cap * K + 16) * sizeof(float), st,
                               d->tiles + p.up_first, up_perm, d->mask, d->ppos, d->wb, up_b, d->bp, d->slots, p.s_cap, p.up_chunks);
        else
            hipLaunchKernelGGL((nt ? k_nd_up<K, true> : k_nd_up<K, false>), dim3(p.up_tiles), dim3(WAVE * p.up_nw),
                               ((size_t)p.s_cap + (size_t)(p.up_nw - 1) * WAVE) * K * sizeof(float),
                               st, d->tiles + p.up_first, up_perm, d->mask, d->ppos, d->wf, up_b, d->bp, d->slots, p.s_cap);
    }
    if (part == 0) {
        if (exch_n && exchange != d->slots + exch_off)
            LS_HIP(hipMemcpyAsync(exchange, d->slots + exch_off, exch_n * sizeof(float), hipMemcpyDeviceToDevice, st));
        LS_HIP(hipGetLastError());
        return LS_OK;
    }
    if (d->profile) LS_HIP(hipEventRecord(d->ev[1], st));
    for (int lv = 0; lv <= top; ++lv) {
        const LevelPlan& p = d->plan[lv];
        if (!(p.down_p ? p.down_p_tiles : p.down_tiles)) continue;
        LS_HIP(mark(lv, lv, 1));
        if (p.down_p)
            hipLaunchKernelGGL(k_nd_down_p<K>, dim3(p.down_p_tiles), dim3(WAVE), (size_t)std::max(p.down_p_s + p.down_p_lds, 1) * K * sizeof(float), st,
                               d->ptiles + p.down_p_first, d->perm, d->push_ptr, d->push_tgt, d->finv, d->wb, (const float*)d->bp, d->xb, x,
                               p.down_p_s);
        else if (p.down_b)
            hipLaunchKernelGGL((nt ? k_nd_down_b<K, true> : k_nd_down_b<K, false>), dim3(p.down_tiles), dim3(WAVE * p.down_nw), (((size_t)p.s_cap + p.b_cap) * K + 32) * sizeof(float), st,
                               d->tiles + p.down_first, d->perm, d->push_ptr, d->push_tgt, d->finv, d->wf, (const float*)d->bp, d->xb, x,
                               p.s_cap, p.b_cap, p.down_chunks, lv == 0 ? rf : RootFill{nullptr, nullptr, nullptr, nullptr});
        else
            hipLaunchKernelGGL((nt ? k_nd_down<K, true> : k_nd_down<K, false>), dim3(p.down_tiles), dim3(WAVE * p.down_nw),
                               ((size_t)p.s_cap + p.b_cap + (size_t)(p.down_nw - 1) * WAVE) * K * sizeof(float), st, d->tiles + p.down_first,
                               d->perm, d->push_ptr, d->push_tgt, d->finv, d->wb, (const float*)d->bp, d->xb, x, p.s_cap, p.b_cap,
                               lv == 0 ? rf : RootFill{nullptr, nullptr, nullptr, nullptr});
    }
#ifdef LS_TIER_STAMPS
    if (ta.stamps) ta.stamps += stamp_n;
#endif
    if (d->tier_wgs) {
        LS_HIP(mark(d->tier_root, d->levels - 1, 1));
        if (d->tier_waves == TIER_WAVES_FULL && nt_tier) hipLaunchKernelGGL((k_nd_tier<K, false, TIER_WAVES_FULL, true>), dim3(d->tier_wgs), dim3(WAVE * TIER_WAVES_FULL), tier_lds, st, ta, b, x, d->tier_tri);
        else if (d->tier_waves == TIER_WAVES_FULL) hipLaunchKernelGGL((k_nd_tier<K, false, TIER_WAVES_FULL, false>), dim3(d->tier_wgs), dim3(WAVE * TIER_WAVES_FULL), tier_lds, st, ta, b, x, d->tier_tri);
        else if (d->tier_waves == TIER_WAVES_WIDE) hipLaunchKernelGGL((k_nd_tier<K, false, TIER_WAVES_WIDE, false>), dim3(d->tier_wgs), dim3(WAVE * TIER_WAVES_WIDE), tier_lds, st, ta, b, x, d->tier_tri);
        else if (nt_tier) hipLaunchKernelGGL((k_nd_tier<K, false, TIER_WAVES, true>), dim3(d->tier_wgs), dim3(WAVE * TIER_WAVES), tier_lds, st, ta, b, x, d->tier_tri);
        else hipLaunchKernelGGL((k_nd_tier<K, false, TIER_WAVES, false>), dim3(d->tier_wgs), dim3(WAVE * TIER_WAVES), tier_lds, st, ta, b, x, d->tier_tri);
    }
    if (d->profile) LS_HIP(hipEventRecord(d->ev[2], st));
    LS_HIP(hipGetLastError());
    LS_HIP(mark_end());
    if (d->profile) {
        LS_HIP(hipStreamSynchronize(st));
        float a = 0, c = 0;
        LS_HIP(hipEventElapsedTime(&a, d->ev[0], d->ev[1]));
        LS_HIP(hipEventElapsedTime(&c, d->ev[1], d->ev[2]));
        d->prof_ms[0] = a; d->prof_ms[1] = c; d->prof_ms[2] = 0.0;
    }
    return LS_OK;
}

extern "C" int ls_direct_solve(ls_direct* d, const float* b, float* x, int k, void* stream) {
    LS_REQUIRE(d && b && x && k >= 1 && k <= d->kmax, LS_E_INVALID, "ls_direct_solve: bad argument (1 <= k <= %d)", d ? d->kmax : 4);
    LS_REQUIRE(b != x, LS_E_INVALID, "ls_direct_solve: b and x must not alias");
    LS_REQUIRE(d->factored, LS_E_STATE, "ls_direct_solve: the handle is unfactored (its last ls_direct_refactor failed)");
    DeviceGuard g(d->device);
    LS_HIP(g.err);
    hipStream_t st = (hipStream_t)stream;
    hipStreamCaptureStatus cap = hipStreamCaptureStatusNone;
    if (st) (void)hipStreamIsCapturing(st, &cap);
    const bool capturing = cap == hipStreamCaptureStatusActive;
    if (!capturing && d->used && st != d->last_stream) LS_HIP(hipStreamWaitEvent(st, d->busy, 0));
    int rc;
    switch (k) {
        case 1: rc = direct_solve_k<1>(d, b, x, st, -1, nullptr); break;
        case 2: rc = direct_solve_k<2>(d, b, x, st, -1, nullptr); break;
        case 3: rc = direct_solve_k<3>(d, b, x, st, -1, nullptr); break;
        default: rc = direct_solve_k<4>(d, b, x, st, -1, nullptr); break;
    }
    if (rc == LS_OK && !capturing) { LS_HIP(hipEventRecord(d->busy, st)); d->last_stream = st; d->used = true; }
    return rc;
}

extern "C" int ls_direct_solve_part(ls_direct* d, const float* b, float* x, int k, int part, float* exchange, void* stream) {
    LS_REQUIRE(d && b && x && k >= 1 && k <= d->kmax && (part == 0 || part == 1), LS_E_INVALID, "ls_direct_solve_part: bad argument");
    LS_REQUIRE(b != x, LS_E_INVALID, "ls_direct_solve_part: b and x must not alias");
    LS_REQUIRE(d->factored, LS_E_STATE, "ls_direct_solve_part: the handle is unfactored (its last ls_direct_refactor failed)");
    LS_REQUIRE(exchange || d->exch_f1 == d->exch_f0, LS_E_INVALID, "ls_direct_solve_part: the exchange buffer is missing");
    DeviceGuard g(d->device);
    LS_HIP(g.err);
    hipStream_t st = (hipStream_t)stream;
    hipStreamCaptureStatus cap = hipStreamCaptureStatusNone;
    if (st) (void)hipStreamIsCapturing(st, &cap);
    const bool capturing = cap == hipStreamCaptureStatusActive;
    if (!capturing && d->used && st != d->last_stream) LS_HIP(hipStreamWaitEvent(st, d->busy, 0));
    int rc;
    switch (k) {
        case 1: rc = direct_solve_k<1>(d, b, x, st, part, exchange); break;
        case 2: rc = direct_solve_k<2>(d, b, x, st, part, exchange); break;
        case 3: rc = direct_solve_k<3>(d, b, x, st, part, exchange); break;
        default: rc = direct_solve_k<4>(d, b, x, st, part, exchange); break;
    }
    if (rc == LS_OK && !capturing) { LS_HIP(hipEventRecord(d->busy, st)); d->last_stream = st; d->used = true; }
    return rc;
}

extern "C" int ls_direct_exchange_region(ls_direct* d, int k, float** region, int64_t* floats) {
    LS_REQUIRE(d && region && floats && k >= 1 && k <= d->kmax, LS_E_INVALID, "ls_direct_exchange_region: bad argument");
    *region = d->slots + (size_t)d->exch_f0 * d->arity * k;
    *floats = (d->exch_f1 - d->exch_f0) * d->arity * k;
    return LS_OK;
}

extern "C" int ls_direct_shard_info(const ls_direct* d, int* h_rank, int* h_count, int* h_cut_level, int64_t* h_exchange_floats_per_column,
                                    unsigned char* h_owned_rows) {
    LS_REQUIRE(d, LS_E_INVALID, "ls_direct_shard_info: bad argument");
    if (h_rank) *h_rank = d->shard_rank;
    if (h_count) *h_count = d->shard_count;
    if (h_cut_level) *h_cut_level = d->cut;
    if (h_exchange_floats_per_column) *h_exchange_floats_per_column = (d->exch_f1 - d->exch_f0) * d->arity;
    if (h_owned_rows) { if (d->owned_rows.empty()) memset(h_owned_rows, 1, (size_t)d->V); else memcpy(h_owned_rows, d->owned_rows.data(), (size_t)d->V); }
    return LS_OK;
}

extern "C" int ls_direct_set(ls_direct* d, const char* name, int value) {
    LS_REQUIRE(d && name, LS_E_INVALID, "ls_direct_set: bad argument");
    if (!strcmp(name, "profile")) {
        DeviceGuard g(d->device);
        LS_HIP(g.err);
#ifndef LS_TIER_STAMPS
        LS_REQUIRE(value != 2, LS_E_INVALID, "ls_direct_set: profile 2 (per-wave clock stamps of the tier kernels) exists in the experiments build only (tools/build_variant.sh stamps -DLS_TIER_STAMPS)");
#endif
        d->profile = value < 0 ? 0 : std::min(value, 3);
        while (d->profile && d->ev.size() < 4) { hipEvent_t e; LS_HIP(hipEventCreate(&e)); d->ev.push_back(e); }
        return LS_OK;
    }
    if (!strcmp(name, "nt")) {
        d->nt_levels = value < 0 ? d->nt_rule[0] : value != 0;
        d->nt_tier = value < 0 ? d->nt_rule[1] : value != 0;
        return LS_OK;
    }
    set_error("ls_direct_set: unknown option '%s'", name);
    return LS_E_INVALID;
}

int ls_direct_adopt(ls_direct* d, std::vector<std::pair<void*, size_t>> owned, const double* seconds3, const double* quality4, ls::RefactorState* refac) {
    d->tables.insert(d->tables.end(), owned.begin(), owned.end());
    d->refac = refac;
    for (int i = 0; i < 3; ++i) d->factor_s[i] = seconds3[i];
    for (int i = 0; i < 4; ++i) d->plan_q[i] = quality4[i];
    return LS_OK;
}

extern "C" int ls_direct_refactor(ls_direct* d, const int32_t* d_rowptr, const int32_t* d_col, const float* d_val, int64_t V, int64_t nnz,
                                  void* stream) {
    LS_REQUIRE(d && d_rowptr && d_col && d_val && V > 0 && nnz > 0, LS_E_INVALID, "ls_direct_refactor: bad argument");
    LS_REQUIRE(d->refac, LS_E_STATE, "ls_direct_refactor: %s", d->shard_count > 1 ? "a sharded handle cannot refactor"
                                                                                  : "the handle was not made by ls_direct_factor_refactorable");
    DeviceGuard g(d->device);
    LS_HIP(g.err);
    hipStream_t st = (hipStream_t)stream;
    hipStreamCaptureStatus cap = hipStreamCaptureStatusNone;
    if (st) (void)hipStreamIsCapturing(st, &cap);
    LS_REQUIRE(cap == hipStreamCaptureStatusNone, LS_E_STATE, "ls_direct_refactor: not capturable (it synchronises the stream)");
    if (d->used && st != d->last_stream) LS_HIP(hipStreamWaitEvent(st, d->busy, 0));
    bool touched = false;
    const int rc = ls::refactor_run(d->refac, d_rowptr, d_col, d_val, V, nnz, st, &touched);
    if (rc == LS_OK) d->factored = true;
    else if (touched) d->factored = false;
    return rc;
}

extern "C" int ls_direct_refactorable(const ls_direct* d, int* h_yes, size_t* h_retained_device_bytes) {
    LS_REQUIRE(d, LS_E_INVALID, "ls_direct_refactorable: bad argument");
    if (h_yes) *h_yes = d->refac ? 1 : 0;
    if (h_retained_device_bytes) *h_retained_device_bytes = ls::refactor_state_bytes(d->refac);
    return LS_OK;
}

extern "C" int ls_direct_plan_quality(const ls_direct* d, int* h_ordering, double* h_words_per_vertex, double* h_spread, double* h_words_other) {
    LS_REQUIRE(d, LS_E_INVALID, "ls_direct_plan_quality: bad argument");
    if (h_ordering) *h_ordering = (int)d->plan_q[0];
    if (h_words_per_vertex) *h_words_per_vertex = d->plan_q[1];
    if (h_spread) *h_spread = d->plan_q[2];
    if (h_words_other) *h_words_other = d->plan_q[3];
    return LS_OK;
}

extern "C" int ls_direct_shape(const ls_direct* d, int* h_levels, int* h_arity, int* h_tier_levels, int* h_tier_workgroups,
                               int64_t* h_words_up, int64_t* h_words_down, int64_t* h_n_bnd) {
    LS_REQUIRE(d, LS_E_INVALID, "ls_direct_shape: bad argument");
    if (h_words_up) *h_words_up = d->words_up;
    if (h_words_down) *h_words_down = d->words_down;
    if (h_n_bnd) *h_n_bnd = d->n_bnd;
    if (h_levels) *h_levels = d->levels;
    if (h_arity) *h_arity = d->arity;
    if (h_tier_levels) *h_tier_levels = d->tier_phases;
    if (h_tier_workgroups) *h_tier_workgroups = d->tier_wgs;
    return LS_OK;
}

extern "C" int ls_direct_factor_seconds(const ls_direct* d, double* h_s3) {
    LS_REQUIRE(d && h_s3, LS_E_INVALID, "ls_direct_factor_seconds: bad argument");
    for (int i = 0; i < 3; ++i) h_s3[i] = d->factor_s[i];
    return LS_OK;
}

extern "C" int ls_direct_level_words(const ls_direct* d, int cap, int64_t* h_up, int64_t* h_down) {
    LS_REQUIRE(d && cap >= 0, LS_E_INVALID, "ls_direct_level_words: bad argument");
    for (int lv = 0; lv < cap && lv < d->levels; ++lv) {
        if (h_up) h_up[lv] = lv < (int)d->lvl_up.size() ? d->lvl_up[(size_t)lv] : 0;
        if (h_down) h_down[lv] = lv < (int)d->lvl_down.size() ? d->lvl_down[(size_t)lv] : 0;
    }
    return LS_OK;
}

extern "C" int ls_direct_level_rows(const ls_direct* d, int cap, int64_t* h_rows, int64_t* h_bnd) {
    LS_REQUIRE(d && cap >= 0, LS_E_INVALID, "ls_direct_level_rows: bad argument");
    for (int lv = 0; lv < cap && lv < d->levels; ++lv) {
        if (h_rows) h_rows[lv] = lv < (int)d->lvl_rows.size() ? d->lvl_rows[(size_t)lv] : 0;
        if (h_bnd) h_bnd[lv] = lv < (int)d->lvl_bnd.size() ? d->lvl_bnd[(size_t)lv] : 0;
    }
    return LS_OK;
}

#ifdef LS_TIER_STAMPS
extern "C" int ls_direct_tier_stamps(ls_direct* d, long long* h_out, int64_t n) {
    LS_REQUIRE(d && h_out && d->stamps, LS_E_STATE, "ls_direct_tier_stamps: no stamps (solve with \"profile\" = 2 first)");
    const int64_t have = 2 * (int64_t)d->tier_wgs * d->tier_waves * TIER_STAMP_SLOTS;
    LS_REQUIRE(n >= have, LS_E_WORKSPACE, "ls_direct_tier_stamps: %lld entries needed", (long long)have);
    DeviceGuard g(d->device);
    LS_HIP(hipDeviceSynchronize());
    LS_HIP(hipMemcpy(h_out, d->stamps, (size_t)have * sizeof(long long), hipMemcpyDeviceToHost));
    return LS_OK;
}
#endif

extern "C" int ls_direct_level_index_bytes(const ls_direct* d, int cap, int64_t* h_up, int64_t* h_down) {
    LS_REQUIRE(d && cap >= 0, LS_E_INVALID, "ls_direct_level_index_bytes: bad argument");
    for (int lv = 0; lv < cap && lv < d->levels; ++lv) {
        if (h_up) h_up[lv] = lv < (int)d->lvl_idx_up.size() ? d->lvl_idx_up[(size_t)lv] : 0;
        if (h_down) h_down[lv] = lv < (int)d->lvl_idx_down.size() ? d->lvl_idx_down[(size_t)lv] : 0;
    }
    return LS_OK;
}

extern "C" int ls_direct_tier_balance(const ls_direct* d, double* h_words4) {
    LS_REQUIRE(d && h_words4, LS_E_INVALID, "ls_direct_tier_balance: bad argument");
    for (int i = 0; i < 4; ++i) h_words4[i] = d->tier_balance[i];
    return LS_OK;
}

extern "C" int ls_direct_launch_profile(const ls_direct* d, int cap, int* h_n, double* h_ms, int64_t* h_words, int32_t* h_level_lo,
                                        int32_t* h_level_hi, int32_t* h_sweep) {
    LS_REQUIRE(d && cap >= 0, LS_E_INVALID, "ls_direct_launch_profile: bad argument");
    const int n = (int)d->launch_ms.size();
    if (h_n) *h_n = n;
    for (int i = 0; i < n && i < cap; ++i) {
        const ls_direct::LaunchMeta m = d->lmeta[(size_t)i];
        int64_t w = 0;
        for (int lv = std::max(m.lo, 0); lv <= m.hi && lv < d->levels; ++lv) {
            if (m.sweep != 1) w += d->lvl_up[(size_t)lv];
            if (m.sweep != 0) w += d->lvl_down[(size_t)lv];
        }
        if (h_ms) h_ms[i] = d->launch_ms[(size_t)i];
        if (h_words) h_words[i] = w;
        if (h_level_lo) h_level_lo[i] = m.lo;
        if (h_level_hi) h_level_hi[i] = m.hi;
        if (h_sweep) h_sweep[i] = m.sweep;
    }
    return LS_OK;
}

extern "C" int ls_direct_info(const ls_direct* d, int64_t* h_factor_entries, int* h_launches, double* h_ms3) {
    LS_REQUIRE(d, LS_E_INVALID, "ls_direct_info: bad argument");
    if (h_factor_entries) *h_factor_entries = d->factor_entries;
    if (h_launches) {
        int n = 0;
        for (int lv = 0; lv < d->levels; ++lv) {
            const LevelPlan& p = d->plan[lv];
            const bool fused = lv == 0 && d->tier_root > 0 && !p.down_p;
            n += (((p.up_p ? p.up_p_tiles : p.up_tiles) && !fused) ? 1 : 0) + ((p.down_p ? p.down_p_tiles : p.down_tiles) ? 1 : 0);
        }
        *h_launches = n + (d->tier_wgs ? 2 : 0);
    }
    if (h_ms3) for (int i = 0; i < 3; ++i) h_ms3[i] = d->prof_ms[i];
    return LS_OK;
}
```

large-steps-pytorch_amd/csrc/nd_tier.h:

```cpp
#pragma once

namespace ls {

constexpr int TIER_MAX_H = 6;
constexpr int TIER_WAVES = 4;
constexpr int TIER_WAVES_WIDE = 8;
constexpr int TIER_WAVES_FULL = 16;
constexpr int TIER_LDS_FULL = 160 * 1024;
constexpr int TIER_LDS = 150 * 1024;
constexpr int TIER_LDS_WIDE = 80 * 1024;
constexpr int LEVEL_LDS = 150 * 1024;
constexpr int LDS_OPTIN = 160 * 1024;
constexpr int TIER_TRI4 = 9;
constexpr int TIER_SPE = 4;

enum : int { NODE_LEAF = 1, NODE_SPARSE = 2, NODE_QUAD = 4, NODE_UPC = 8 };

struct SpEnt { float val; int idx; };

struct NodeD {
    int s, b, own_start, bnd_off, front_off, pfront_off, cix, flags;
    long long finv_off, w_off;
    int spb_off, sps_off;
};

struct alignas(32) TierItem {
    int s, b, own_start, bnd_off, front_off, pfront_off, cix, flags;
    long long finv_off, w_off;
    int spb_off, sps_off;
    int row0, r0, r1, part, nparts, pad0, pad1, pad2;
};
static_assert(sizeof(TierItem) == 96, "TierItem layout");

struct alignas(64) TierWG {
    int up_off[TIER_MAX_H + 1];
    int down_off[TIER_MAX_H + 1];
    unsigned up_split, down_split;
    unsigned up_leaf, down_leaf;
    int n_dense, pad;
    int dense_rng[2 * TIER_MAX_H];
};
static_assert(sizeof(TierWG) == 128, "TierWG layout (read as 32 dwords)");

struct TierArgs {
    const TierItem* items;
    const TierWG* wgs;
    const int* perm;
    const unsigned char* mask;
    const int* ppos;
    const int* pull;
    const int* push_ptr;
    const int* push_tgt;
    const float* u4;
    const float* d4;
    const float* tri;
    const int* sp_ptr;
    const SpEnt* sp_ent;
    float* bprime;
    int upper_lo, upper_hi;
    float* braw;
    float* slots;
    float* xb;
    int arity, phases, region_floats, vec_floats;
#ifdef LS_TIER_STAMPS
    long long* stamps;
#endif
};

constexpr int TIER_STAMP_SLOTS = 32;
#ifdef LS_TIER_STAMPS
#define LS_STAMP(slot) do { if (a.stamps && lane == 0) stamp_base[(slot)] = (long long)wall_clock64(); } while (0)
#define LS_STAMP_VAL(slot, v) do { if (a.stamps && lane == 0) stamp_base[(slot)] = (long long)(v); } while (0)
#else
#define LS_STAMP(slot) do { } while (0)
#define LS_STAMP_VAL(slot, v) do { } while (0)
#endif

constexpr int ITEM_DWORDS = 24;
__device__ __forceinline__ int rec_load(const TierItem* items, int k, int lane) {
    return lane < ITEM_DWORDS ? reinterpret_cast<const int*>(items)[(size_t)k * ITEM_DWORDS + lane] : 0;
}
__device__ __forceinline__ int rl(int v, int i) { return __builtin_amdgcn_readlane(v, i); }
__device__ __forceinline__ TierItem rec_unpack(int r) {
    TierItem t;
    t.s = rl(r, 0); t.b = rl(r, 1); t.own_start = rl(r, 2); t.bnd_off = rl(r, 3); t.front_off = rl(r, 4); t.pfront_off = rl(r, 5);
    t.cix = rl(r, 6); t.flags = rl(r, 7);
    t.finv_off = (long long)(((unsigned long long)(unsigned)rl(r, 9) << 32) | (unsigned)rl(r, 8));
    t.w_off = (long long)(((unsigned long long)(unsigned)rl(r, 11) << 32) | (unsigned)rl(r, 10));
    t.spb_off = rl(r, 12); t.sps_off = rl(r, 13); t.row0 = rl(r, 14); t.r0 = rl(r, 15); t.r1 = rl(r, 16); t.part = rl(r, 17);
    t.nparts = rl(r, 18); t.pad0 = t.pad1 = t.pad2 = 0;
    return t;
}

__device__ __forceinline__ void wave_lds_sync() {
    __builtin_amdgcn_fence(__ATOMIC_RELEASE, "wavefront");
    __builtin_amdgcn_wave_barrier();
    __builtin_amdgcn_fence(__ATOMIC_ACQUIRE, "wavefront");
}

__device__ __forceinline__ float bcast_lane(float v, int c) {
    return __int_as_float(__builtin_amdgcn_readlane(__float_as_int(v), c));
}

template <int K>
__device__ __forceinline__ void pull_compact(const TierArgs& a, size_t f, float (&v)[K]) {
#pragma unroll
    for (int q = 0; q < K; ++q) v[q] = 0.0f;
    const int* pl = a.pull + f * a.arity;
    for (int c = 0; c < a.arity; ++c) {
        const int idx = pl[c];
        if (idx >= 0) {
#pragma unroll
            for (int q = 0; q < K; ++q) v[q] += a.xb[(size_t)idx * K + q];
        }
    }
}

template <int K>
__device__ __forceinline__ void pull_values(const TierArgs& a, const int (&pl)[4], float (&v)[K]) {
#pragma unroll
    for (int q = 0; q < K; ++q) v[q] = 0.0f;
#pragma unroll
    for (int c = 0; c < 4; ++c) {
        if (pl[c] >= 0) {
#pragma unroll
            for (int q = 0; q < K; ++q) v[q] += a.xb[(size_t)pl[c] * K + q];
        }
    }
}
__device__ __forceinline__ void pull_indices(const TierArgs& a, size_t f, bool on, int (&pl)[4]) {
#pragma unroll
    for (int c = 0; c < 4; ++c) pl[c] = on ? a.pull[f * 4 + c] : -1;
}

struct LeafIdx {
    int g, p0, p1, pp;
};
template <int K>
struct LeafDat {
    float4 t[TIER_TRI4];
    float v[K];
    float xv[K];
    SpEnt e[TIER_SPE];
};

template <bool UP>
__device__ __forceinline__ void leaf_idx(const TierArgs& a, const TierItem& n, int lane, LeafIdx& ix) {
    ix.g = lane < n.s ? a.perm[n.own_start + lane] : 0;
    if (UP) {
        const bool r = lane < n.b;
        ix.p0 = r ? a.sp_ptr[n.spb_off + lane] : 0;
        ix.p1 = r ? a.sp_ptr[n.spb_off + lane + 1] : 0;
        ix.pp = r ? a.ppos[n.bnd_off + lane] : 0;
    } else {
        const bool r = lane < n.s;
        ix.p0 = r ? a.sp_ptr[n.sps_off + lane] : 0;
        ix.p1 = r ? a.sp_ptr[n.sps_off + lane + 1] : 0;
        ix.pp = 0;
    }
}

template <int K, bool UP, bool NT>
__device__ __forceinline__ void leaf_dat(const TierArgs& a, const TierItem& n, const LeafIdx& ix, const float* __restrict__ b_in,
                                         int lane, LeafDat<K>& d) {
    if (!UP) {
#pragma unroll
        for (int q = 0; q < K; ++q) d.xv[q] = lane < n.b ? a.xb[(size_t)(n.bnd_off + lane) * K + q] : 0.0f;
    }
    const float2* __restrict__ ent = reinterpret_cast<const float2*>(a.sp_ent);
    if (!UP) {
#pragma unroll
        for (int t = 0; t < TIER_SPE; ++t) {
            const bool ok = ix.p0 + t < ix.p1;
            const float2 r = ld_stream2<NT>(ent + (ok ? ix.p0 + t : 0));
            d.e[t].val = ok ? r.x : 0.0f;
            d.e[t].idx = ok ? __float_as_int(r.y) : 0;
        }
    }
    const float4* __restrict__ p = reinterpret_cast<const float4*>(a.tri + n.finv_off);
    const int n4 = (n.s * (n.s + 1) / 2 + 3) >> 2;
#pragma unroll
    for (int e = 0; e < TIER_TRI4; ++e) {
        const int i = lane + e * 64;
        d.t[e] = i < n4 ? p[i] : make_float4(0.f, 0.f, 0.f, 0.f);
    }
#pragma unroll
    for (int q = 0; q < K; ++q) {
        if (UP) d.v[q] = lane < n.s ? b_in[(size_t)ix.g * K + q] : 0.0f;
        else d.v[q] = lane < n.s ? a.bprime[(size_t)(n.own_start + lane) * K + q] : 0.0f;
    }
    if (UP) {
#pragma unroll
        for (int t = 0; t < TIER_SPE; ++t) {
            const bool ok = ix.p0 + t < ix.p1;
            const float2 r = ld_stream2<NT>(ent + (ok ? ix.p0 + t : 0));
// ... 21 lines not shown
    return __builtin_amdgcn_mfma_f32_4x4x1f32(vec16, m, acc, 4, E, 0);
}

template <int C>
__device__ __forceinline__ float tri_select(float lo, float hi) {
    if (C == 0) return lo;
    unsigned long long mask;
    asm volatile("s_lshl_b64 %0, -1, %1" : "=s"(mask) : "n"(C) : "scc");
    return __builtin_amdgcn_inverse_ballot_w64(mask) ? lo : hi;
}
template <int T, int E>
__device__ __forceinline__ float tri_element(const float* stage, int j, int tj) {
    constexpr int c = 16 * T + E;
    const float lo = stage[tj + c];
    if (c == 0) return lo;
    const float hi = stage[c * (c + 1) / 2 + j];
    return tri_select<c>(lo, hi);
}
template <int T>
__device__ __forceinline__ void tri_chunk(const float* stage, const float* vec4, int s, int lane, int j, int tj, f32x4& a0, f32x4& a1) {
    if (16 * T >= s) return;
    const float v16 = vec4[64 * T + lane];
    float m[16];
    {
    m[0] = tri_element<T, 0>(stage, j, tj);   m[1] = tri_element<T, 1>(stage, j, tj);   m[2] = tri_element<T, 2>(stage, j, tj);   m[3] = tri_element<T, 3>(stage, j, tj);
    m[4] = tri_element<T, 4>(stage, j, tj);   m[5] = tri_element<T, 5>(stage, j, tj);   m[6] = tri_element<T, 6>(stage, j, tj);   m[7] = tri_element<T, 7>(stage, j, tj);
    m[8] = tri_element<T, 8>(stage, j, tj);   m[9] = tri_element<T, 9>(stage, j, tj);   m[10] = tri_element<T, 10>(stage, j, tj); m[11] = tri_element<T, 11>(stage, j, tj);
    m[12] = tri_element<T, 12>(stage, j, tj); m[13] = tri_element<T, 13>(stage, j, tj); m[14] = tri_element<T, 14>(stage, j, tj); m[15] = tri_element<T, 15>(stage, j, tj);
    }
    a0 = mv_step<0>(v16, m[0], a0);   a1 = mv_step<1>(v16, m[1], a1);   a0 = mv_step<2>(v16, m[2], a0);   a1 = mv_step<3>(v16, m[3], a1);
    a0 = mv_step<4>(v16, m[4], a0);   a1 = mv_step<5>(v16, m[5], a1);   a0 = mv_step<6>(v16, m[6], a0);   a1 = mv_step<7>(v16, m[7], a1);
    a0 = mv_step<8>(v16, m[8], a0);   a1 = mv_step<9>(v16, m[9], a1);   a0 = mv_step<10>(v16, m[10], a0); a1 = mv_step<11>(v16, m[11], a1);
    a0 = mv_step<12>(v16, m[12], a0); a1 = mv_step<13>(v16, m[13], a1); a0 = mv_step<14>(v16, m[14], a0); a1 = mv_step<15>(v16, m[15], a1);
}
template <int K>
__device__ __forceinline__ void tri_matvec(const float* stage, const float* vec4, int s, int lane, float (&acc)[K]) {
    const int j = min(lane, s - 1);
    const int tj = j * (j + 1) / 2;
    f32x4 a0 = {0.f, 0.f, 0.f, 0.f}, a1 = {0.f, 0.f, 0.f, 0.f};
    tri_chunk<0>(stage, vec4, s, lane, j, tj, a0, a1);
    tri_chunk<1>(stage, vec4, s, lane, j, tj, a0, a1);
    tri_chunk<2>(stage, vec4, s, lane, j, tj, a0, a1);
    tri_chunk<3>(stage, vec4, s, lane, j, tj, a0, a1);
#pragma unroll
    for (int q = 0; q < K; ++q) acc[q] = a0[q] + a1[q];
}

template <int K>
__device__ __forceinline__ void sparse_row(const TierArgs& a, const LeafIdx& ix, const SpEnt (&e)[TIER_SPE], const float* vec4, float (&u)[K]) {
#pragma unroll
    for (int q = 0; q < K; ++q) u[q] = 0.0f;
#pragma unroll
    for (int t = 0; t < TIER_SPE; ++t) {
        if (ix.p0 + t < ix.p1) {
#pragma unroll
            for (int q = 0; q < K; ++q) u[q] = fmaf(e[t].val, vec4[e[t].idx * 4 + q], u[q]);
        }
    }
    for (int p = ix.p0 + TIER_SPE; p < ix.p1; ++p) {
        const SpEnt z = a.sp_ent[p];
#pragma unroll
        for (int q = 0; q < K; ++q) u[q] = fmaf(z.val, vec4[z.idx * 4 + q], u[q]);
    }
}

template <int K>
__device__ __forceinline__ void leaf_up_compute(const TierArgs& a, const TierItem& n, const LeafIdx& ix, const float (&bj)[K],
                                                const SpEnt (&e)[TIER_SPE], float* region, int tri_floats) {
    const int lane = threadIdx.x & 63, s = n.s, b = n.b;
    float* yv = region + tri_floats;
    {
        float4 w = make_float4(0.f, 0.f, 0.f, 0.f);
        if (lane < s) { w.x = bj[0]; if (K > 1) w.y = bj[K > 1 ? 1 : 0]; if (K > 2) w.z = bj[K > 2 ? 2 : 0]; if (K > 3) w.w = bj[K > 3 ? 3 : 0]; }
        reinterpret_cast<float4*>(yv)[lane] = w;
    }
    wave_lds_sync();
    float y[K];
    tri_matvec<K>(region, yv, s, lane, y);
    wave_lds_sync();
    if (lane < s) {
#pragma unroll
        for (int q = 0; q < K; ++q) { yv[lane * 4 + q] = y[q]; a.bprime[(size_t)(n.own_start + lane) * K + q] = y[q]; }
    }
    wave_lds_sync();
    if (n.pfront_off >= 0) {
        const bool upc = n.flags & NODE_UPC;
        if (lane < b) {
            float u[K];
            sparse_row<K>(a, ix, e, yv, u);
            const size_t dst = upc ? (size_t)(n.bnd_off + lane) * K : ((size_t)(n.pfront_off + ix.pp) * a.arity + n.cix) * K;
            float* out = upc ? a.xb : a.slots;
#pragma unroll
            for (int q = 0; q < K; ++q) out[dst + q] = u[q];
        }
        for (int i = lane + 64; i < b; i += 64) {
            const int p0 = a.sp_ptr[n.spb_off + i], p1 = a.sp_ptr[n.spb_off + i + 1], pp = a.ppos[n.bnd_off + i];
            float u[K];
#pragma unroll
            for (int q = 0; q < K; ++q) u[q] = 0.0f;
            for (int p = p0; p < p1; ++p) {
                const SpEnt z = a.sp_ent[p];
#pragma unroll
                for (int q = 0; q < K; ++q) u[q] = fmaf(z.val, yv[z.idx * 4 + q], u[q]);
            }
            const size_t dst = upc ? (size_t)(n.bnd_off + i) * K : ((size_t)(n.pfront_off + pp) * a.arity + n.cix) * K;
            float* out = upc ? a.xb : a.slots;
#pragma unroll
            for (int q = 0; q < K; ++q) out[dst + q] = u[q];
        }
    }
    wave_lds_sync();
}

template <int K>
__device__ __forceinline__ void leaf_down_head(const TierArgs& a, const TierItem& n, const LeafIdx& ix, const float (&xv)[K],
                                               const SpEnt (&e)[TIER_SPE], float* region, float (&t)[K]) {
    const int lane = threadIdx.x & 63, b = n.b;
    float* xbv = region;
    if (lane < b) {
#pragma unroll
        for (int q = 0; q < K; ++q) xbv[lane * 4 + q] = xv[q];
    }
    for (int i = lane + 64; i < b; i += 64) {
#pragma unroll
        for (int q = 0; q < K; ++q) xbv[i * 4 + q] = a.xb[(size_t)(n.bnd_off + i) * K + q];
    }
    wave_lds_sync();
    sparse_row<K>(a, ix, e, xbv, t);
    wave_lds_sync();
}

template <int K>
__device__ __forceinline__ void leaf_down_vec(const TierItem& n, const float (&t)[K], float* region, int tri_floats) {
    const int lane = threadIdx.x & 63;
    float4 w = make_float4(0.f, 0.f, 0.f, 0.f);
    if (lane < n.s) { w.x = t[0]; if (K > 1) w.y = t[K > 1 ? 1 : 0]; if (K > 2) w.z = t[K > 2 ? 2 : 0]; if (K > 3) w.w = t[K > 3 ? 3 : 0]; }
    reinterpret_cast<float4*>(region + tri_floats)[lane] = w;
}

template <int K>
__device__ __forceinline__ void leaf_down_tail(const TierItem& n, const LeafIdx& ix, const float (&yj)[K], float* __restrict__ x_out,
                                               float* region, int tri_floats) {
    const int lane = threadIdx.x & 63, s = n.s;
    float z[K];
    tri_matvec<K>(region, region + tri_floats, s, lane, z);
    if (lane < s) {
#pragma unroll
        for (int q = 0; q < K; ++q) x_out[(size_t)ix.g * K + q] = yj[q] - z[q];
    }
    wave_lds_sync();
}

template <int K, bool UP, int W, bool NT>
__device__ __forceinline__ void leaf_phase(const TierArgs& a, int k0, int k1, const float* __restrict__ b_in, float* __restrict__ x_out,
                                           float* region, int tri_floats, long long* stamp_base) {
    const int lane = threadIdx.x & 63;
    int leaf_no = 0;
    (void)leaf_no; (void)stamp_base;
    if (k0 >= k1) return;
    constexpr int S = W;
    TierItem it = rec_unpack(rec_load(a.items, k0, lane));
    int rec_n = k0 + S < k1 ? rec_load(a.items, k0 + S, lane) : 0;
    LeafIdx ix;
    leaf_idx<UP>(a, it, lane, ix);
    for (int k = k0; k < k1; k += S) {
        float v[K];
        SpEnt e[TIER_SPE];
        float t[K];
        {
            LeafDat<K> d;
            leaf_dat<K, UP, NT>(a, it, ix, b_in, lane, d);
            if (!UP) leaf_down_head<K>(a, it, ix, d.xv, d.e, region, t);
            tri_stage<K>(d, it.s, lane, region);
#pragma unroll
            for (int q = 0; q < K; ++q) v[q] = d.v[q];
#pragma unroll
            for (int u = 0; u < TIER_SPE; ++u) e[u] = d.e[u];
        }
        if (!UP) leaf_down_vec<K>(it, t, region, tri_floats);
        wave_lds_sync();
        const bool more = k + S < k1;
        TierItem it_n = it;
        LeafIdx ix_n = ix;
        if (more) { it_n = rec_unpack(rec_n); leaf_idx<UP>(a, it_n, lane, ix_n); }
        rec_n = k + 2 * S < k1 ? rec_load(a.items, k + 2 * S, lane) : 0;
        if (UP) leaf_up_compute<K>(a, it, ix, v, e, region, tri_floats);
        else leaf_down_tail<K>(it, ix, v, x_out, region, tri_floats);
        if (leaf_no < 8) LS_STAMP(16 + leaf_no);
        ++leaf_no;
        it = it_n; ix = ix_n;
    }
}

#ifndef LS_TIER_Q
#define LS_TIER_Q 4
#endif
constexpr int TIER_Q = LS_TIER_Q;

template <bool NT>
__device__ __forceinline__ void tier_prefetch(const float4* __restrict__ col, size_t rows, int q0, int q1, float4 (&cur)[TIER_Q]) {
#pragma unroll
    for (int e = 0; e < TIER_Q; ++e) cur[e] = (q0 + e < q1) ? ld_stream4<NT>(col + (size_t)(q0 + e) * rows) : make_float4(0.f, 0.f, 0.f, 0.f);
}

__device__ __forceinline__ void tier_mv16(float v16, const float4& a, const float4& b, const float4& c, const float4& d, int n, f32x4& acc) {
    acc = mv_step<0>(v16, a.x, acc); acc = mv_step<1>(v16, a.y, acc); acc = mv_step<2>(v16, a.z, acc); acc = mv_step<3>(v16, a.w, acc);
    if (n > 1) { acc = mv_step<4>(v16, b.x, acc); acc = mv_step<5>(v16, b.y, acc); acc = mv_step<6>(v16, b.z, acc); acc = mv_step<7>(v16, b.w, acc); }
    if (n > 2) { acc = mv_step<8>(v16, c.x, acc); acc = mv_step<9>(v16, c.y, acc); acc = mv_step<10>(v16, c.z, acc); acc = mv_step<11>(v16, c.w, acc); }
    if (n > 3) { acc = mv_step<12>(v16, d.x, acc); acc = mv_step<13>(v16, d.y, acc); acc = mv_step<14>(v16, d.z, acc); acc = mv_step<15>(v16, d.w, acc); }
}

__device__ __forceinline__ void tier_mv_batch(const float* sv4, int base, int q, int q1, const float4 (&c)[TIER_Q], f32x4& acc) {
    const int lane = threadIdx.x & 63;
    const float4 z = make_float4(0.f, 0.f, 0.f, 0.f);
    if (TIER_Q == 2) tier_mv16(sv4[(4 * q - base) * 4 + lane], c[0], c[1], z, z, min(2, q1 - q), acc);
    if (TIER_Q >= 4) tier_mv16(sv4[(4 * q - base) * 4 + lane], c[0], c[1], c[TIER_Q >= 4 ? 2 : 0], c[TIER_Q >= 4 ? 3 : 0], q1 - q, acc);
    if (TIER_Q >= 8 && q + 4 < q1) tier_mv16(sv4[(4 * q + 16 - base) * 4 + lane], c[TIER_Q >= 8 ? 4 : 0], c[TIER_Q >= 8 ? 5 : 0],
                                             c[TIER_Q >= 8 ? 6 : 0], c[TIER_Q >= 8 ? 7 : 0], q1 - q - 4, acc);
}
template <bool NT>
__device__ __forceinline__ void tier_dot(const float4* __restrict__ col, size_t rows, int q0, int q1, const float* sv4, int base,
                                         float4 (&A)[TIER_Q], float4 (&B)[TIER_Q], f32x4& acc) {
    for (int q = q0; q < q1; q += 2 * TIER_Q) {
        tier_mv_batch(sv4, base, q, q1, A, acc);
        tier_prefetch<NT>(col, rows, q + 2 * TIER_Q, q1, A);
        if (q + TIER_Q < q1) tier_mv_batch(sv4, base, q + TIER_Q, q1, B, acc);
        tier_prefetch<NT>(col, rows, q + 3 * TIER_Q, q1, B);
    }
}

template <int K>
__device__ __forceinline__ void node_up_finish(const TierArgs& a, const TierItem& n, int i, int pp, const float (&acc)[K]) {
    if (i >= n.b || n.pfront_off < 0) return;
    if (n.flags & NODE_UPC) {
#pragma unroll
        for (int q = 0; q < K; ++q) a.xb[(size_t)(n.bnd_off + i) * K + q] = acc[q];
        return;
    }
    const size_t dst = ((size_t)(n.pfront_off + pp) * a.arity + n.cix) * K;
#pragma unroll
    for (int q = 0; q < K; ++q) a.slots[dst + q] = acc[q];
}

template <int K>
struct DensePre {
    float4 cur[TIER_Q];
    float v[K];
    int idx;
    int plo[4], plb[4];
    int fw0, fw1;
};

__device__ __forceinline__ void fwd_slice(const TierItem& it, int& f0, int& f1) {
    const int chunks = (max(it.s, 1) + 63) >> 6, total = chunks * it.nparts, ord = (it.row0 >> 6) * it.nparts + it.part;
    f0 = (int)((long long)it.b * ord / total);
    f1 = (int)((long long)it.b * (ord + 1) / total);
}

template <int K, bool NT>
__device__ __forceinline__ void node_up_pre(const TierArgs& a, const TierItem& it, DensePre<K>& P) {
    const int lane = threadIdx.x & 63, i = it.row0 + lane;
    const bool row = i < it.b;
    const float4* col = reinterpret_cast<const float4*>(a.u4 + it.w_off) + (row ? i : 0);
    tier_prefetch<NT>(col, (size_t)it.b, it.r0 >> 2, row ? it.r1 >> 2 : it.r0 >> 2, P.cur);
    const bool fin = it.part == 0 && row && it.pfront_off >= 0;
    P.idx = (fin && !(it.flags & NODE_UPC)) ? a.ppos[it.bnd_off + i] : 0;
    const bool inner = !(it.flags & NODE_LEAF) && a.arity == 4;
    const int j = it.r0 + lane;
    pull_indices(a, (size_t)(it.front_off + j), inner && j < it.r1 && j < it.s, P.plo);
    if (K <= 3) pull_indices(a, (size_t)(it.front_off + it.s + i), inner && fin, P.plb);
}

template <int K, bool NT>
__device__ __forceinline__ void node_up(const TierArgs& a, const TierItem& it, DensePre<K>& P, const float* __restrict__ b_in, float* region, float* pbuf) {
    const int lane = threadIdx.x & 63, b = it.b;
    const int i = it.row0 + lane;
    const bool row = i < b;
    float* sv4 = region;
    const float4* __restrict__ col = reinterpret_cast<const float4*>(a.u4 + it.w_off) + (row ? i : 0);
    float4 B[TIER_Q];
    tier_prefetch<NT>(col, (size_t)b, (it.r0 >> 2) + TIER_Q, it.r1 >> 2, B);
    float pass[K];
#pragma unroll
    for (int q = 0; q < K; ++q) pass[q] = 0.0f;
    const bool fin = it.part == 0 && row && it.pfront_off >= 0;
    const bool pre4 = a.arity == 4;
    if (fin && !(it.flags & NODE_LEAF)) {
        if (pre4 && K <= 3) pull_values<K>(a, P.plb, pass); else pull_compact<K>(a, (size_t)(it.front_off + it.s + i), pass);
    }
    for (int j = it.r0 + lane; j < it.r1; j += 64) {
        float v[K];
        if (j >= it.s) {
#pragma unroll
            for (int q = 0; q < K; ++q) sv4[(j - it.r0) * 4 + q] = 0.0f;
            continue;
        }
        if (it.flags & NODE_LEAF) {
            const size_t g = (size_t)a.perm[it.own_start + j];
#pragma unroll
            for (int q = 0; q < K; ++q) v[q] = b_in[g * K + q];
        } else {
#pragma unroll
            for (int q = 0; q < K; ++q) v[q] = a.braw[(size_t)(it.own_start + j) * K + q];
        }
        if (!(it.flags & NODE_LEAF)) {
            float u[K];
            if (pre4 && j == it.r0 + lane) pull_values<K>(a, P.plo, u); else pull_compact<K>(a, (size_t)(it.front_off + j), u);
#pragma unroll
            for (int q = 0; q < K; ++q) v[q] -= u[q];
        }
#pragma unroll
        for (int q = 0; q < K; ++q) sv4[(j - it.r0) * 4 + q] = v[q];
        if (it.row0 == 0) {
#pragma unroll
            for (int q = 0; q < K; ++q) a.bprime[(size_t)(it.own_start + j) * K + q] = v[q];
        }
    }
    wave_lds_sync();
    f32x4 a4 = {0.f, 0.f, 0.f, 0.f};
    tier_dot<NT>(col, (size_t)b, it.r0 >> 2, it.r1 >> 2, sv4, it.r0, P.cur, B, a4);
    float acc[K];
#pragma unroll
    for (int q = 0; q < K; ++q) acc[q] = a4[q];
    if (it.nparts == 1) {
        if (fin) {
            const bool upc = it.flags & NODE_UPC;
            const size_t dst = upc ? (size_t)(it.bnd_off + i) * K : ((size_t)(it.pfront_off + P.idx) * a.arity + it.cix) * K;
            float* out = upc ? a.xb : a.slots;
#pragma unroll
            for (int q = 0; q < K; ++q) out[dst + q] = acc[q] + pass[q];
        }
    } else {
#pragma unroll
        for (int q = 0; q < K; ++q) pbuf[lane * 4 + q] = acc[q] + pass[q];
    }
    wave_lds_sync();
}

template <int K>
__device__ __forceinline__ void node_down_store(const TierArgs& a, const TierItem& it, int g, int p0, int p1, const int (&tg)[4],
                                                float* __restrict__ x_out, const float (&acc)[K]) {
    const int j = it.row0 + (threadIdx.x & 63);
    if (j >= it.s) return;
#pragma unroll
    for (int q = 0; q < K; ++q) x_out[(size_t)g * K + q] = acc[q];
    if (it.flags & NODE_LEAF) return;
#pragma unroll
    for (int c = 0; c < 4; ++c) {
        if (tg[c] >= 0) {
#pragma unroll
            for (int q = 0; q < K; ++q) a.xb[(size_t)tg[c] * K + q] = acc[q];
        }
    }
    if (p1 - p0 > 4) push_down<K>(a.push_tgt, p0 + 4, p1, a.xb, acc);
}

template <int K>
__device__ __forceinline__ void node_down_finish(const TierArgs& a, const TierItem& it, float* __restrict__ x_out, const float (&acc)[K]) {
    const int j = it.row0 + (threadIdx.x & 63);
    if (j >= it.s) return;
    const size_t g = (size_t)a.perm[it.own_start + j];
#pragma unroll
    for (int q = 0; q < K; ++q) x_out[g * K + q] = acc[q];
    if (!(it.flags & NODE_LEAF)) push_down<K>(a.push_tgt, a.push_ptr[it.front_off + j], a.push_ptr[it.front_off + j + 1], a.xb, acc);
}

template <int K, bool NT>
__device__ __forceinline__ void node_down_pre(const TierArgs& a, const TierItem& it, DensePre<K>& P) {
    const int lane = threadIdx.x & 63, s = it.s, j = it.row0 + lane;
    const bool row = j < s;
    tier_prefetch<NT>(reinterpret_cast<const float4*>(a.d4 + it.finv_off) + (row ? j : 0), (size_t)s, it.r0 >> 2, row ? it.r1 >> 2 : it.r0 >> 2, P.cur);
    const int t = it.r0 + lane;
#pragma unroll
    for (int q = 0; q < K; ++q) P.v[q] = (t < it.r1 && t < s) ? a.bprime[(size_t)(it.own_start + t) * K + q] : 0.0f;
    const bool fin = it.part == 0 && row;
    const bool push = fin && !(it.flags & NODE_LEAF);
    P.idx = fin ? a.perm[it.own_start + j] : 0;
    P.plo[0] = push ? a.push_ptr[it.front_off + j] : 0;
    P.plo[1] = push ? a.push_ptr[it.front_off + j + 1] : 0;
    int f0, f1;
    fwd_slice(it, f0, f1);
    const bool fw = !(it.flags & NODE_LEAF) && f0 + lane < f1;
    P.fw0 = fw ? a.push_ptr[it.front_off + s + f0 + lane] : 1;
    P.fw1 = fw ? a.push_ptr[it.front_off + s + f0 + lane + 1] : 0;
}

template <int K, bool NT>
__device__ __forceinline__ void node_down(const TierArgs& a, const TierItem& it, DensePre<K>& P, float* __restrict__ x_out, float* region, float* pbuf) {
    const int lane = threadIdx.x & 63, s = it.s;
    const int j = it.row0 + lane;
    const bool row = j < s;
    float* sv4 = region;
    const float4* __restrict__ col = reinterpret_cast<const float4*>(a.d4 + it.finv_off) + (row ? j : 0);
    float4 B[TIER_Q];
    tier_prefetch<NT>(col, (size_t)s, (it.r0 >> 2) + TIER_Q, it.r1 >> 2, B);
    int f0, f1;
    fwd_slice(it, f0, f1);
    const bool fw = P.fw0 <= P.fw1;
    float fv[K];
    int ftg[2];
#pragma unroll
    for (int q = 0; q < K; ++q) fv[q] = fw ? a.xb[(size_t)(it.bnd_off + f0 + lane) * K + q] : 0.0f;
#pragma unroll
    for (int c = 0; c < 2; ++c) ftg[c] = (fw && P.fw0 + c < P.fw1) ? a.push_tgt[P.fw0 + c] : -1;
    const int s4 = (s + 3) & ~3;
    for (int t = it.r0 + lane; t < it.r1; t += 64) {
        float v[K];
        if (t < s) {
            if (t == it.r0 + lane) {
#pragma unroll
                for (int q = 0; q < K; ++q) v[q] = P.v[q];
            } else {
#pragma unroll
                for (int q = 0; q < K; ++q) v[q] = a.bprime[(size_t)(it.own_start + t) * K + q];
            }
        } else if (t >= s4 && t - s4 < it.b) {
#pragma unroll
            for (int q = 0; q < K; ++q) v[q] = -a.xb[(size_t)(it.bnd_off + t - s4) * K + q];
        } else {
#pragma unroll
            for (int q = 0; q < K; ++q) v[q] = 0.0f;
        }
#pragma unroll
        for (int q = 0; q < K; ++q) sv4[(t - it.r0) * 4 + q] = v[q];
    }
    wave_lds_sync();
#pragma unroll
    for (int c = 0; c < 4; ++c) P.plb[c] = (it.nparts == 1 && P.plo[0] + c < P.plo[1]) ? a.push_tgt[P.plo[0] + c] : -1;
    f32x4 a4 = {0.f, 0.f, 0.f, 0.f};
    tier_dot<NT>(col, (size_t)s, it.r0 >> 2, it.r1 >> 2, sv4, it.r0, P.cur, B, a4);
    float acc[K];
#pragma unroll
    for (int q = 0; q < K; ++q) acc[q] = a4[q];
    if (it.nparts == 1) node_down_store<K>(a, it, P.idx, P.plo[0], P.plo[1], P.plb, x_out, acc);
    else {
#pragma unroll
        for (int q = 0; q < K; ++q) pbuf[lane * 4 + q] = acc[q];
    }
#pragma unroll
    for (int c = 0; c < 2; ++c) {
        if (ftg[c] >= 0) {
#pragma unroll
            for (int q = 0; q < K; ++q) a.xb[(size_t)ftg[c] * K + q] = fv[q];
        }
    }
    if (fw && P.fw1 - P.fw0 > 2) push_down<K>(a.push_tgt, P.fw0 + 2, P.fw1, a.xb, fv);
    if (!(it.flags & NODE_LEAF)) {
        for (int i = f0 + 64 + lane; i < f1; i += 64) {
            const size_t f = (size_t)(it.front_off + s + i);
            const int p0 = a.push_ptr[f], p1 = a.push_ptr[f + 1];
            float v[K];
#pragma unroll
            for (int q = 0; q < K; ++q) v[q] = a.xb[(size_t)(it.bnd_off + i) * K + q];
            push_down<K>(a.push_tgt, p0, p1, a.xb, v);
        }
    }
    wave_lds_sync();
}

template <int K, bool UP, int W, bool NT>
__global__ __launch_bounds__(64 * W, 16 / W) void k_nd_tier(TierArgs a, const float* __restrict__ b_in, float* __restrict__ x_out,
                                                              int tri_floats) {
    extern __shared__ __attribute__((aligned(16))) float sm[];
    const int wave = __builtin_amdgcn_readfirstlane(threadIdx.x >> 6), lane = threadIdx.x & 63;
    float* region = sm + (size_t)wave * a.region_floats;
    for (int i = lane; 4 * i < a.region_floats; i += 64) reinterpret_cast<float4*>(region)[i] = make_float4(0.f, 0.f, 0.f, 0.f);
    wave_lds_sync();
    const int n_wg = (int)gridDim.x;
    const int sub = __builtin_expect((n_wg & 7) == 0, 1) ? (int)(blockIdx.x & 7) * (n_wg >> 3) + (int)(blockIdx.x >> 3) : (int)blockIdx.x;
#ifdef LS_TIER_STAMPS
    long long* stamp_base = a.stamps ? a.stamps + ((size_t)sub * W + wave) * TIER_STAMP_SLOTS : nullptr;
#else
    long long* stamp_base = nullptr;
#endif
    LS_STAMP(0);
    const int hdr = lane < 32 ? reinterpret_cast<const int*>(a.wgs + sub)[lane] : 0;
    const int obase = UP ? 0 : TIER_MAX_H + 1;
    const unsigned split = (unsigned)rl(hdr, UP ? 14 : 15), leafy = (unsigned)rl(hdr, UP ? 16 : 17);
    if (UP) {
        const int n_dense = rl(hdr, 18);
        for (int r = threadIdx.x; r < n_dense; r += blockDim.x) {
            int o = r, start = 0;
#pragma unroll
            for (int t = 0; t < TIER_MAX_H; ++t) {
                const int cnt = rl(hdr, 20 + 2 * t + 1);
                const bool here = o >= 0 && o < cnt;
                start = here ? rl(hdr, 20 + 2 * t) + o : start;
                o = here ? -1 : o - cnt;
            }
            const size_t g = (size_t)a.perm[start];
#pragma unroll
            for (int q = 0; q < K; ++q) a.braw[(size_t)start * K + q] = b_in[g * K + q];
        }
        for (int r = a.upper_lo + blockIdx.x * blockDim.x + threadIdx.x; r < a.upper_hi; r += gridDim.x * blockDim.x) {
            const size_t g = (size_t)a.perm[r];
#pragma unroll
            for (int q = 0; q < K; ++q) a.braw[(size_t)r * K + q] = b_in[g * K + q];
        }
    }
    LS_STAMP(1);
    DensePre<K> pre;
#pragma unroll
    for (int e = 0; e < TIER_Q; ++e) pre.cur[e] = make_float4(0.f, 0.f, 0.f, 0.f);
#pragma unroll
    for (int q = 0; q < K; ++q) pre.v[q] = 0.0f;
    pre.idx = 0; pre.fw0 = 1; pre.fw1 = 0;
#pragma unroll
    for (int c = 0; c < 4; ++c) { pre.plo[c] = -1; pre.plb[c] = -1; }
    TierItem it_pre = rec_unpack(0);
    bool pre_valid = false;
    for (int ph = 0; ph < a.phases; ++ph) {
        const int i0 = rl(hdr, obase + ph), i1 = rl(hdr, obase + ph + 1);
        int rec_nx = 0;
        bool has_nx = false;
        if (ph + 1 < a.phases && !((leafy >> (ph + 1)) & 1u)) {
            const int j0 = rl(hdr, obase + ph + 1) + wave;
            has_nx = j0 < rl(hdr, obase + ph + 2);
            if (has_nx) rec_nx = rec_load(a.items, j0, lane);
        }
        if ((leafy >> ph) & 1u) {
            leaf_phase<K, UP, W, NT>(a, i0 + wave, i1, b_in, x_out, region, tri_floats, stamp_base);
        } else {
            int rec = (!pre_valid && i0 + wave < i1) ? rec_load(a.items, i0 + wave, lane) : 0;
            int head_k = -1, head_idx = 0, head_p0 = 0, head_p1 = 0, head_flags = 0;
            for (int k = i0 + wave; k < i1; k += W) {
                const int rec_next = k + W < i1 ? rec_load(a.items, k + W, lane) : 0;
                const bool first = k == i0 + wave && pre_valid;
                const TierItem it = first ? it_pre : rec_unpack(rec);
                rec = rec_next;
                float* pbuf = region + a.vec_floats + ((k - i0) / W) * 256;
                if (!first) { if (UP) node_up_pre<K, NT>(a, it, pre); else node_down_pre<K, NT>(a, it, pre); }
                if (UP) node_up<K, NT>(a, it, pre, b_in, region, pbuf);
                else node_down<K, NT>(a, it, pre, x_out, region, pbuf);
                if (it.nparts > 1 && it.part == 0) {
                    head_k = k; head_idx = pre.idx; head_p0 = pre.plo[0]; head_p1 = pre.plo[1]; head_flags = it.flags;
                }
            }
            if ((split >> ph) & 1u) {
                const int rec_head = head_k >= 0 ? rec_load(a.items, head_k, lane) : 0;
                int head_tg[4];
#pragma unroll
                for (int c = 0; c < 4; ++c) head_tg[c] = (!UP && head_k >= 0 && head_p0 + c < head_p1 && !(head_flags & NODE_LEAF)) ? a.push_tgt[head_p0 + c] : -1;
                __syncthreads();
                for (int k = i0 + wave; k < i1; k += W) {
                    const bool mine = k == head_k;
                    const TierItem it = rec_unpack(mine ? rec_head : rec_load(a.items, k, lane));
                    if (it.nparts == 1 || it.part != 0) continue;
                    float acc[K];
#pragma unroll
                    for (int q = 0; q < K; ++q) acc[q] = 0.0f;
                    for (int p = 0; p < it.nparts; ++p) {
                        const int kp = k + p - i0;
                        const float* pb = sm + (size_t)(kp % W) * a.region_floats + a.vec_floats + (kp / W) * 256;
#pragma unroll
                        for (int q = 0; q < K; ++q) acc[q] += pb[lane * 4 + q];
                    }
                    if (UP) {
                        const int i = it.row0 + lane;
                        const int pp = mine ? head_idx : ((i < it.b && it.pfront_off >= 0 && !(it.flags & NODE_UPC)) ? a.ppos[it.bnd_off + i] : 0);
                        node_up_finish<K>(a, it, i, pp, acc);
                    } else if (mine) {
                        node_down_store<K>(a, it, head_idx, head_p0, head_p1, head_tg, x_out, acc);
                    }
                    else node_down_finish<K>(a, it, x_out, acc);
                }
            }
        }
        if (ph < 6) { LS_STAMP(2 + 2 * ph); LS_STAMP_VAL(24 + ph, (i1 - i0 - wave + W - 1) / W); }
        pre_valid = has_nx;
        it_pre = rec_unpack(rec_nx);
        if (pre_valid) {
            if (UP) node_up_pre<K, NT>(a, it_pre, pre); else node_down_pre<K, NT>(a, it_pre, pre);
        } else {
#pragma unroll
            for (int e = 0; e < TIER_Q; ++e) pre.cur[e] = make_float4(0.f, 0.f, 0.f, 0.f);
#pragma unroll
            for (int q = 0; q < K; ++q) pre.v[q] = 0.0f;
            pre.idx = 0; pre.fw0 = 1; pre.fw1 = 0;
#pragma unroll
            for (int c = 0; c < 4; ++c) { pre.plo[c] = -1; pre.plb[c] = -1; }
        }
        __syncthreads();
        if (ph < 6) LS_STAMP(3 + 2 * ph);
    }
}

}
```

large-steps-pytorch_amd/largesteps/_native.py:

```python
import ctypes
import os
import threading
import weakref

import torch

_HERE = os.path.dirname(os.path.abspath(__file__))
_LIB_PATH = os.environ.get("LARGESTEPS_HIP_LIB", os.path.join(_HERE, "..", "lib", "liblargesteps_hip.so"))

LS_E_INVALID, LS_E_INDEX, LS_E_WORKSPACE, LS_E_OVERFLOW, LS_E_STATE, LS_E_NOT_CONVERGED = -1, -2, -3, -4, -5, -6

_lib = None
_lib_lock = threading.Lock()

c_void_p, c_int, c_i64, c_float, c_double, c_size_t = (ctypes.c_void_p, ctypes.c_int, ctypes.c_int64, ctypes.c_float,
                                                        ctypes.c_double, ctypes.c_size_t)


class SolveInfo(ctypes.Structure):
    _fields_ = [("iterations", ctypes.c_int32), ("converged", ctypes.c_int32),
                ("rnorm", ctypes.c_double * 4), ("bnorm", ctypes.c_double * 4)]


class DirectOptions(ctypes.Structure):
    _fields_ = [("struct_bytes", ctypes.c_int32), ("leaf_size", ctypes.c_int32), ("arity", ctypes.c_int32), ("tier_levels", ctypes.c_int32),
                ("sparse_leaves", ctypes.c_int32), ("shard_rank", ctypes.c_int32), ("shard_count", ctypes.c_int32), ("ordering", ctypes.c_int32),
                ("tier_waves", ctypes.c_int32)]


_SIGNATURES = {
    "ls_version": (c_int, []),
    "ls_last_error": (ctypes.c_char_p, []),
    "ls_assemble_workspace_bytes": (c_int, [c_i64, c_i64, ctypes.POINTER(c_size_t)]),
    "ls_assemble_pattern": (c_int, [c_void_p, c_int, c_i64, c_i64, c_void_p, c_int, c_float, c_float, c_void_p, c_size_t,
                                    c_void_p, ctypes.POINTER(c_i64), c_int, c_void_p]),
    "ls_assemble_fill": (c_int, [c_void_p, c_size_t, c_i64, c_i64, c_void_p, c_void_p, c_void_p, c_void_p, c_i64, c_void_p,
                                 c_int, c_void_p]),
    "ls_csr_from_coo": (c_int, [c_void_p, c_void_p, c_void_p, c_i64, c_i64, c_void_p, c_void_p, c_void_p, c_void_p, c_size_t,
                                c_int, c_void_p]),
    "ls_spmv": (c_int, [c_void_p, c_void_p, c_void_p, c_i64, c_i64, c_void_p, c_void_p, c_int, c_int, c_int, c_void_p]),
    "ls_solver_create": (c_int, [c_void_p, c_void_p, c_void_p, c_i64, c_i64, c_int, c_int, c_void_p, ctypes.POINTER(c_void_p)]),
    "ls_solver_create_ext": (c_int, [c_void_p, c_void_p, c_void_p, c_i64, c_i64, c_i64, c_int, c_int, c_void_p,
                                     ctypes.POINTER(c_void_p)]),
    "ls_solver_phase": (c_int, [c_void_p, c_int, c_void_p, c_void_p, c_int, c_double, c_double, c_int, c_void_p]),
    "ls_solver_buffers": (c_int, [c_void_p, ctypes.POINTER(c_void_p), ctypes.POINTER(c_void_p), ctypes.POINTER(c_int),
                                  ctypes.POINTER(c_int)]),
    "ls_shard_cheb_steps": (c_int, [c_void_p, c_void_p, c_void_p, c_void_p, c_int, c_int, c_int, c_void_p, c_void_p, c_i64, c_void_p]),
    "ls_shard_resnorm": (c_int, [c_void_p, c_void_p, c_void_p, c_int, c_i64, c_void_p]),
    "ls_solver_bind": (c_int, [c_void_p, c_void_p, c_void_p]),
    "ls_solver_poll": (c_int, [c_void_p, c_int, c_int, ctypes.POINTER(SolveInfo), c_void_p]),
    "ls_gather_rows": (c_int, [c_void_p, c_void_p, c_i64, c_int, c_void_p, c_int, c_void_p]),
    "ls_solver_destroy": (c_int, [c_void_p]),
    "ls_direct_create": (c_int, [c_void_p, c_int, c_void_p, ctypes.POINTER(c_void_p)]),
    "ls_direct_destroy": (c_int, [c_void_p]),
    "ls_direct_solve": (c_int, [c_void_p, c_void_p, c_void_p, c_int, c_void_p]),
    "ls_direct_set": (c_int, [c_void_p, ctypes.c_char_p, c_int]),
    "ls_remove_duplicates_workspace_bytes": (c_int, [c_i64, ctypes.POINTER(c_size_t)]),
    "ls_remove_duplicates": (c_int, [c_void_p, c_i64, c_void_p, c_int, c_i64, c_void_p, c_void_p, c_void_p, ctypes.POINTER(c_i64), c_void_p,
                                     c_size_t, c_int, c_void_p]),
    "ls_csr_transpose_workspace_bytes": (c_int, [c_i64, c_i64, ctypes.POINTER(c_size_t)]),
    "ls_csr_transpose": (c_int, [c_void_p, c_void_p, c_void_p, c_i64, c_i64, c_void_p, c_void_p, c_void_p, c_void_p, c_size_t, c_int, c_void_p]),
    "ls_corner_ranks_workspace_bytes": (c_int, [c_i64, c_i64, ctypes.POINTER(c_size_t)]),
    "ls_corner_ranks": (c_int, [c_void_p, c_int, c_i64, c_i64, c_void_p, c_void_p, c_void_p, c_size_t, c_int, c_void_p]),
    "ls_normals_workspace_bytes": (c_int, [c_i64, c_i64, ctypes.POINTER(c_size_t)]),
    "ls_face_normals": (c_int, [c_void_p, c_void_p, c_int, c_i64, c_i64, c_void_p, c_int, c_void_p]),
    "ls_face_normals_backward": (c_int, [c_void_p, c_void_p, c_int, c_i64, c_i64, c_void_p, c_void_p, c_void_p, c_void_p, c_void_p,
                                         c_size_t, c_int, c_void_p]),
    "ls_vertex_normals": (c_int, [c_void_p, c_void_p, c_int, c_i64, c_i64, c_void_p, c_void_p, c_void_p, c_void_p, c_void_p, c_void_p,
                                  c_void_p, c_size_t, c_int, c_void_p]),
    "ls_vertex_normals_backward": (c_int, [c_void_p, c_void_p, c_int, c_i64, c_i64, c_void_p, c_void_p, c_void_p, c_void_p, c_void_p,
                                           c_void_p, c_void_p, c_void_p, c_void_p, c_size_t, c_int, c_void_p]),
    "ls_face_normals_with_norms": (c_int, [c_void_p, c_void_p, c_int, c_i64, c_i64, c_void_p, c_void_p, c_void_p, c_size_t, c_int, c_void_p]),
    "ls_vertex_normals_from_norms": (c_int, [c_void_p, c_void_p, c_int, c_i64, c_i64, c_void_p, c_void_p, c_void_p, c_void_p, c_void_p,
                                             c_void_p, c_size_t, c_int, c_void_p]),
    "ls_normals_pair_backward_faces": (c_int, [c_void_p, c_void_p, c_int, c_i64, c_i64, c_void_p, c_void_p, c_void_p, c_void_p, c_void_p,
                                               c_void_p, c_void_p, c_size_t, c_int, c_void_p]),
    "ls_normals_pair_backward_verts": (c_int, [c_void_p, c_void_p, c_int, c_i64, c_i64, c_void_p, c_void_p, c_void_p, c_void_p, c_void_p,
                                               c_void_p, c_void_p, c_void_p, c_size_t, c_int, c_void_p]),
    "ls_vertex_normals_gathered": (c_int, [c_void_p, c_void_p, c_int, c_i64, c_i64, c_void_p, c_void_p, c_void_p, c_void_p, c_void_p, c_int, c_void_p]),
    "ls_meshgeom_workspace_bytes": (c_int, [c_i64, c_i64, ctypes.POINTER(c_size_t)]),
    "ls_massmatrix_voronoi": (c_int, [c_void_p, c_void_p, c_int, c_i64, c_i64, c_void_p, c_void_p, c_void_p, c_int, c_void_p]),
    "ls_massmatrix_voronoi_backward": (c_int, [c_void_p, c_void_p, c_int, c_i64, c_i64, c_void_p, c_void_p, c_void_p, c_void_p, c_void_p,
                                               c_size_t, c_int, c_void_p]),
    "ls_average_edge_length": (c_int, [c_void_p, c_void_p, c_int, c_i64, c_i64, c_void_p, c_void_p, c_size_t, c_int, c_void_p]),
    "ls_average_edge_length_backward": (c_int, [c_void_p, c_void_p, c_int, c_i64, c_i64, c_void_p, c_void_p, c_void_p, c_void_p, c_void_p,
                                                c_size_t, c_int, c_void_p]),
    "ls_remesh_create": (c_int, [c_void_p, c_i64, c_void_p, c_int, c_i64, c_float, c_int, c_int, c_void_p, ctypes.POINTER(c_void_p)]),
    "ls_remesh_run": (c_int, [c_void_p, c_int]),
    "ls_remesh_phase": (c_int, [c_void_p, c_int, c_int]),
    "ls_remesh_info": (c_int, [c_void_p, ctypes.POINTER(c_i64), ctypes.POINTER(c_i64), ctypes.POINTER(c_i64 * 6), ctypes.POINTER(c_double * 5)]),
    "ls_remesh_copy_out": (c_int, [c_void_p, c_void_p, c_void_p, c_int]),
    "ls_remesh_destroy": (c_int, [c_void_p]),
    "ls_mesh_distance_create": (c_int, [c_void_p, c_i64, c_void_p, c_int, c_i64, c_int, c_void_p, ctypes.POINTER(c_void_p)]),
    "ls_mesh_distance_query": (c_int, [c_void_p, c_void_p, c_i64, c_void_p, c_void_p, c_void_p, c_void_p]),
    "ls_mesh_distance_max": (c_int, [c_void_p, c_void_p, c_i64, c_void_p, c_void_p]),
    "ls_mesh_distance_destroy": (c_int, [c_void_p]),
    "ls_mesh_distance_weights": (c_int, [c_void_p, c_void_p, c_i64, c_void_p, c_void_p, c_void_p]),
    "ls_mesh_distance_backward_workspace_bytes": (c_int, [c_i64, c_i64, ctypes.POINTER(c_size_t)]),
    "ls_mesh_distance_backward": (c_int, [c_void_p, c_void_p, c_i64, c_void_p, c_void_p, c_void_p, c_void_p, c_void_p, c_void_p, c_void_p,
                                          c_void_p, c_size_t, c_void_p]),
    "ls_mesh_distance_update": (c_int, [c_void_p, c_void_p, c_void_p]),
    "ls_shard_plan_create": (c_int, [c_i64, c_void_p, c_void_p, c_void_p, c_int, c_int, c_int, ctypes.POINTER(c_void_p)]),
    "ls_shard_plan_destroy": (c_int, [c_void_p]),
    "ls_shard_plan_info": (c_int, [c_void_p] + [ctypes.POINTER(c_i64)] * 5 + [ctypes.POINTER(c_int)] * 2 + [ctypes.POINTER(c_i64)]),
    "ls_shard_plan_arrays": (c_int, [c_void_p] + [c_void_p] * 8),
    "ls_shard_layer_sizes": (c_int, [c_i64, c_void_p, c_void_p, c_i64, c_i64, c_int, c_void_p]),
    "ls_patch_plan_create": (c_int, [c_i64, c_void_p, c_void_p, c_void_p, c_void_p, c_int, c_int, c_int, c_int, c_int, ctypes.POINTER(c_void_p)]),
    "ls_patch_plan_destroy": (c_int, [c_void_p]),
    "ls_patch_plan_info": (c_int, [c_void_p] + [ctypes.POINTER(c_int)] * 5 + [ctypes.POINTER(c_i64)] * 3 + [ctypes.POINTER(ctypes.c_double)]),
    "ls_patch_plan_arrays": (c_int, [c_void_p, c_void_p, c_void_p, c_void_p, c_void_p, c_void_p]),
    "ls_direct_level_words": (c_int, [c_void_p, c_int, c_void_p, c_void_p]),
    "ls_direct_tier_lds_bytes": (c_int, [c_int, c_int, c_void_p, c_void_p, c_void_p, c_int, c_int, c_int, ctypes.POINTER(c_size_t)]),
    "ls_direct_level_index_bytes": (c_int, [c_void_p, c_int, c_void_p, c_void_p]),
    "ls_direct_tier_balance": (c_int, [c_void_p, ctypes.POINTER(c_double * 4)]),
    "ls_direct_level_rows": (c_int, [c_void_p, c_int, c_void_p, c_void_p]),
    "ls_direct_exchange_region": (c_int, [c_void_p, c_int, ctypes.POINTER(c_void_p), ctypes.POINTER(c_i64)]),
    "ls_dist_unique_id": (c_int, [c_void_p]),
    "ls_dist_create": (c_int, [c_void_p, c_int, c_int, c_int, ctypes.POINTER(c_void_p)]),
    "ls_dist_destroy": (c_int, [c_void_p]),
    "ls_dist_allreduce_sum": (c_int, [c_void_p, c_void_p, c_i64, c_void_p]),
    "ls_dist_info": (c_int, [c_void_p, ctypes.POINTER(c_int), ctypes.POINTER(c_int)]),
    "ls_dist_direct_solve": (c_int, [c_void_p, c_void_p, c_void_p, c_void_p, c_int, c_void_p]),
    "ls_direct_launch_profile": (c_int, [c_void_p, c_int, c_void_p, c_void_p, c_void_p, c_void_p, c_void_p, c_void_p]),
    "ls_direct_factor": (c_int, [c_void_p, c_void_p, c_void_p, c_i64, c_i64, c_void_p, c_int, c_int, c_int, c_int, c_int, c_int, c_int,
                                 c_void_p, ctypes.POINTER(c_void_p)]),
    "ls_direct_factor_ex": (c_int, [c_void_p, c_void_p, c_void_p, c_i64, c_i64, c_void_p, c_void_p, c_int, c_void_p, ctypes.POINTER(c_void_p)]),
    "ls_direct_options_default": (c_int, [c_void_p]),
    "ls_direct_factor_refactorable": (c_int, [c_void_p, c_void_p, c_void_p, c_i64, c_i64, c_void_p, c_void_p, c_int, c_void_p,
                                              ctypes.POINTER(c_void_p)]),
    "ls_direct_refactor": (c_int, [c_void_p, c_void_p, c_void_p, c_void_p, c_i64, c_i64, c_void_p]),
    "ls_direct_refactorable": (c_int, [c_void_p, ctypes.POINTER(c_int), ctypes.POINTER(c_size_t)]),
    "ls_direct_solve_part": (c_int, [c_void_p, c_void_p, c_void_p, c_int, c_int, c_void_p, c_void_p]),
    "ls_direct_shard_info": (c_int, [c_void_p, ctypes.POINTER(c_int), ctypes.POINTER(c_int), ctypes.POINTER(c_int), ctypes.POINTER(c_i64),
                                     c_void_p]),
    "ls_direct_shape": (c_int, [c_void_p, ctypes.POINTER(c_int), ctypes.POINTER(c_int), ctypes.POINTER(c_int), ctypes.POINTER(c_int),
                                ctypes.POINTER(c_i64), ctypes.POINTER(c_i64), ctypes.POINTER(c_i64)]),
    "ls_direct_factor_seconds": (c_int, [c_void_p, ctypes.POINTER(c_double * 3)]),
    "ls_csr_is_symmetric": (c_int, [c_void_p, c_void_p, c_void_p, c_i64, c_i64, c_float, ctypes.POINTER(c_int), c_int, c_void_p]),
    "ls_direct_pick_tree": (c_int, [c_i64, ctypes.POINTER(c_int), ctypes.POINTER(c_int)]),
    "ls_release_scratch": (c_int, [c_int]),
    "ls_nd_plan_create": (c_int, [c_i64, c_void_p, c_void_p, c_void_p, c_int, c_int, c_int, ctypes.POINTER(c_void_p)]),
    "ls_nd_plan_create_device": (c_int, [c_void_p, c_void_p, c_void_p, c_i64, c_i64, c_int, c_int, c_int, c_int, c_void_p, ctypes.POINTER(c_void_p)]),
    "ls_nd_plan_create_ordered": (c_int, [c_i64, c_void_p, c_void_p, c_void_p, c_int, c_int, c_int, c_int, ctypes.POINTER(c_void_p)]),
    "ls_nd_plan_create_device_ordered": (c_int, [c_void_p, c_void_p, c_void_p, c_i64, c_i64, c_int, c_int, c_int, c_int, c_int, c_void_p, ctypes.POINTER(c_void_p)]),
    "ls_nd_plan_quality": (c_int, [c_void_p, ctypes.POINTER(c_int), ctypes.POINTER(c_double), ctypes.POINTER(c_double), ctypes.POINTER(c_double)]),
    "ls_direct_plan_quality": (c_int, [c_void_p, ctypes.POINTER(c_int), ctypes.POINTER(c_double), ctypes.POINTER(c_double), ctypes.POINTER(c_double)]),
    "ls_nd_plan_destroy": (c_int, [c_void_p]),
    "ls_nd_plan_info": (c_int, [c_void_p, ctypes.POINTER(c_int), ctypes.POINTER(c_int), ctypes.POINTER(c_int), ctypes.POINTER(c_i64),
                                ctypes.POINTER(c_i64), ctypes.POINTER(c_double)]),
    "ls_nd_plan_arrays": (c_int, [c_void_p] + [c_void_p] * 9),
    "ls_direct_info": (c_int, [c_void_p, ctypes.POINTER(c_i64), ctypes.POINTER(c_int), ctypes.POINTER(c_double * 3)]),
    "ls_solver_solve": (c_int, [c_void_p, c_void_p, c_void_p, c_void_p, c_int, c_double, c_double, c_int,
                                ctypes.POINTER(SolveInfo), c_void_p]),
    "ls_solver_set": (c_int, [c_void_p, ctypes.c_char_p, c_int]),
    "ls_solver_set_spectrum": (c_int, [c_void_p, c_double]),
    "ls_solver_chebyshev_iterations": (c_int, [c_void_p, c_double, ctypes.POINTER(c_int)]),
    "ls_solver_set_uniform": (c_int, [c_void_p, c_float, c_float, c_void_p]),
    "ls_solver_set_patches": (c_int, [c_void_p, c_void_p, c_int, c_void_p, c_i64, c_void_p, c_i64, c_void_p, c_i64, c_void_p, c_int,
                                      c_int, c_int, c_void_p]),
    "ls_solver_spectrum": (c_int, [c_void_p, ctypes.POINTER(c_double), ctypes.POINTER(c_double)]),
    "ls_solver_solve_chebyshev": (c_int, [c_void_p, c_void_p, c_void_p, c_void_p, c_int, c_double, c_double, c_int,
                                          ctypes.POINTER(SolveInfo), c_void_p]),
    "ls_solver_profile": (c_int, [c_void_p, ctypes.POINTER(c_double * 3), ctypes.POINTER(c_int)]),
    "ls_solver_sell": (c_int, [c_void_p, ctypes.POINTER(c_void_p), ctypes.POINTER(c_void_p), ctypes.POINTER(c_i64)]),
    "ls_solver_workspace_bytes": (c_int, [c_void_p, ctypes.POINTER(c_size_t)]),
    "ls_adam_uniform_step": (c_int, [c_void_p, c_void_p, c_void_p, c_void_p, c_i64, c_float, c_float, c_float, c_int,
                                     c_void_p, c_int, c_void_p]),
    "ls_adam_uniform_step_device": (c_int, [c_void_p, c_void_p, c_void_p, c_void_p, c_i64, c_float, c_float, c_float, c_void_p,
                                            c_void_p, c_int, c_void_p]),
    "ls_raster_workspace_bytes": (c_int, [c_i64, c_i64, c_int, c_int, c_int, ctypes.POINTER(c_size_t)]),
    "ls_raster_forward": (c_int, [c_void_p, c_i64, c_i64, c_void_p, c_i64, c_int, c_int, c_void_p, c_void_p, c_size_t, c_int, c_void_p]),
    "ls_raster_pixel_order": (c_int, [c_void_p, c_i64, c_i64, c_int, c_int, c_void_p, c_void_p, c_void_p, c_size_t, c_int, c_void_p]),
    "ls_raster_backward": (c_int, [c_void_p, c_i64, c_i64, c_void_p, c_i64, c_int, c_int, c_void_p, c_void_p, c_void_p, c_void_p, c_void_p,
                                   c_void_p, c_void_p, c_size_t, c_int, c_void_p]),
    "ls_raster_interpolate": (c_int, [c_void_p, c_i64, c_i64, c_int, c_void_p, c_i64, c_int, c_int, c_void_p, c_i64, c_void_p, c_int, c_void_p]),
    "ls_raster_interpolate_backward": (c_int, [c_void_p, c_i64, c_i64, c_int, c_void_p, c_i64, c_int, c_int, c_void_p, c_i64, c_void_p, c_void_p,
                                               c_void_p, c_void_p, c_void_p, c_void_p, c_void_p, c_void_p, c_size_t, c_int, c_void_p]),
    "ls_raster_adjacency_workspace_bytes": (c_int, [c_i64, ctypes.POINTER(c_size_t)]),
    "ls_raster_adjacency": (c_int, [c_void_p, c_i64, c_void_p, c_void_p, c_size_t, c_int, c_void_p]),
    "ls_raster_antialias": (c_int, [c_void_p, c_int, c_void_p, c_void_p, c_i64, c_i64, c_int, c_int, c_void_p, c_i64, c_void_p, c_void_p, c_int,
                                    c_void_p]),
    "ls_raster_antialias_backward": (c_int, [c_void_p, c_int, c_void_p, c_void_p, c_i64, c_i64, c_int, c_int, c_void_p, c_i64, c_void_p, c_void_p,
                                             c_float, c_void_p, c_void_p, c_void_p, c_void_p, c_void_p, c_void_p, c_void_p, c_size_t, c_int,
                                             c_void_p]),
    "ls_texture_workspace_bytes": (c_int, [c_i64, c_int, c_int, ctypes.POINTER(c_size_t)]),
    "ls_texture_forward": (c_int, [c_void_p, c_i64, c_int, c_int, c_int, c_void_p, c_i64, c_int, c_int, c_int, c_int, c_void_p, c_int, c_void_p]),
    "ls_texture_order": (c_int, [c_void_p, c_i64, c_int, c_int, c_i64, c_int, c_int, c_int, c_int, c_void_p, c_void_p, c_void_p, c_size_t, c_int,
                                 c_void_p]),
    "ls_texture_backward": (c_int, [c_void_p, c_i64, c_int, c_int, c_int, c_void_p, c_i64, c_int, c_int, c_int, c_int, c_void_p, c_void_p, c_void_p,
                                    c_void_p, c_void_p, c_int, c_void_p]),
    "ls_mip_workspace_bytes": (c_int, [c_i64, c_int, c_int, ctypes.POINTER(c_size_t)]),
    "ls_mip_build": (c_int, [c_void_p, c_i64, c_int, c_int, c_int, c_int, c_void_p, c_int, c_void_p]),
    "ls_mip_fold": (c_int, [c_void_p, c_i64, c_int, c_int, c_int, c_int, c_void_p, c_int, c_void_p]),
    "ls_mip_pixel_differentials": (c_int, [c_void_p, c_void_p, c_i64, c_i64, c_void_p, c_i64, c_int, c_int, c_void_p, c_int, c_void_p]),
    "ls_mip_interpolate_da": (c_int, [c_void_p, c_i64, c_i64, c_int, c_void_p, c_void_p, c_i64, c_int, c_int, c_void_p, c_i64, c_void_p, c_int,
                                      c_void_p]),
    "ls_mip_forward": (c_int, [c_void_p, c_void_p, c_i64, c_int, c_int, c_int, c_int, c_void_p, c_void_p, c_void_p, c_i64, c_int, c_int, c_int,
                               c_int, c_void_p, c_int, c_void_p]),
    "ls_mip_order": (c_int, [c_void_p, c_void_p, c_void_p, c_i64, c_int, c_int, c_i64, c_int, c_int, c_int, c_int, c_int, c_void_p, c_void_p,
                             c_void_p, c_size_t, c_int, c_void_p]),
    "ls_mip_backward": (c_int, [c_void_p, c_void_p, c_i64, c_int, c_int, c_int, c_int, c_void_p, c_void_p, c_void_p, c_i64, c_int, c_int, c_int,
                                c_int, c_void_p, c_void_p, c_void_p, c_void_p, c_void_p, c_void_p, c_void_p, c_void_p, c_int, c_void_p]),
}

EXPORTED_SYMBOLS = tuple(_SIGNATURES)


def lib_path():
    return os.path.abspath(_LIB_PATH)


def lib():
    global _lib
    if _lib is None:
        with _lib_lock:
            if _lib is None:
                path = lib_path()
                if not os.path.exists(path):
                    raise RuntimeError(
                        f"largesteps: native library not found at {path}. Build it with "
                        f"`make -C {os.path.join(_HERE, '..', 'csrc')}` (hipcc, gfx950) or `python -c "
                        f"'import __graft_entry__ as g; g.build()'` from the repository root. There is no CPU/PyTorch fallback.")
                handle = ctypes.CDLL(path)
                for name, (res, args) in _SIGNATURES.items():
                    fn = getattr(handle, name)
                    fn.restype = res
                    fn.argtypes = args
                _lib = handle
    return _lib


class NotConverged(RuntimeError):
    pass


def last_error():
    msg = lib().ls_last_error()
    return msg.decode("utf-8", "replace") if msg else ""


def check(rc):
    if rc == 0:
        return
    msg = last_error()
    if rc == LS_E_INVALID:
        raise ValueError(msg)
    if rc == LS_E_INDEX:
        raise IndexError(msg)
    if rc == LS_E_OVERFLOW:
        raise OverflowError(msg)
    if rc == LS_E_NOT_CONVERGED:
        raise NotConverged(msg)
    raise RuntimeError(f"largesteps native error {rc}: {msg}")


def require_device(t, what):
    if not isinstance(t, torch.Tensor):
        raise TypeError(f"{what} must be a torch.Tensor, got {type(t).__name__}")
    if not t.is_cuda:
        raise RuntimeError(f"largesteps (MI355X build): {what} must live on a HIP device ('cuda'), got device '{t.device}'. "
                           "There is no CPU path in this package.")
    return t


_raw_stream = getattr(torch._C, "_cuda_getCurrentRawStream", None)


# ... 160 lines not shown
```

large-steps-pytorch_amd/largesteps/solvers.py:

```python
import ctypes
import os
import types
import warnings

import numpy as np
import torch
from torch.autograd import Function

from . import _native

_KMAX = 4


class Solver:
    generation = 0

    def __init__(self, M):
        pass

    def solve(self, b, backward=False):
        raise NotImplementedError()


class PCGSolver(Solver):
# ... 78 lines not shown
        return ms[0], ms[1], ms[2], it.value

    def _solve_block(self, b, x0):
        csr = self._csr
        dev = csr.device
        x = torch.empty_like(b)
        info = _native.SolveInfo()
        lib = _native.lib()
        args = (self._handle, _native.ptr(b), _native.ptr(x0) if x0 is not None else None, _native.ptr(x), b.shape[1],
                self.rtol, self.atol, self.max_iter, ctypes.byref(info), _native.stream_of(dev))
        method = "pcg"
        with torch.cuda.device(dev):
            rc = None
            if self.chebyshev:
                rc = lib.ls_solver_solve_chebyshev(*args)
                method = "chebyshev"
                if rc in (_native.LS_E_NOT_CONVERGED, _native.LS_E_STATE):
                    warnings.warn(f"largesteps: {_native.last_error()}; falling back to PCG", RuntimeWarning, stacklevel=3)
                    rc = None
            if rc is None:
                rc = lib.ls_solver_solve(*args)
                method = "pcg"
        self.last_info = dict(iterations=info.iterations, converged=bool(info.converged), method=method,
                              rnorm=list(info.rnorm)[:b.shape[1]], bnorm=list(info.bnorm)[:b.shape[1]])
        if rc == _native.LS_E_NOT_CONVERGED:
            msg = _native.last_error()
            if "not converged" in msg:
                warnings.warn(f"largesteps: {msg}; returning the last iterate", RuntimeWarning, stacklevel=3)
            else:
                raise RuntimeError(f"largesteps: {msg}")
        else:
            _native.check(rc)
        return x

    @_native.retry_on_oom
    def solve(self, b, backward=False):
        _native.require_device(b, "b")
        csr = self._csr
        if b.device != csr.device:
            raise RuntimeError(f"matrix ({csr.device}) and b ({b.device}) must be on the same device")
        if b.dtype != torch.float32:
            raise TypeError(f"b must be float32, got {b.dtype}")
        if b.dim() not in (1, 2) or b.shape[0] != csr.V:
            raise ValueError(f"Invalid array shape {b.shape} for solve: expected ({csr.V}, k)")
        squeeze = b.dim() == 1
        b2 = (b.detach().unsqueeze(1) if squeeze else b.detach()).contiguous()
        k = b2.shape[1]
        x0 = None
        if self.warm_start:
            g = self.guess_bwd if backward else self.guess_fwd
            if g is not None and g.shape == b2.shape:
                x0 = g
        if k <= _KMAX:
            x = self._solve_block(b2, x0)
        else:
            x = torch.empty_like(b2)
            for c0 in range(0, k, _KMAX):
                c1 = min(c0 + _KMAX, k)
                g0 = x0[:, c0:c1].contiguous() if x0 is not None else None
                x[:, c0:c1] = self._solve_block(b2[:, c0:c1].contiguous(), g0)
        if self.warm_start:
            if backward:
                self.guess_bwd = x
            else:
                self.guess_fwd = x
        return x.squeeze(1) if squeeze else x


class IterativeCholeskySolver(PCGSolver):

    def __init__(self, M, rtol=1e-6, max_iter=10000, chebyshev=True, patch_columns=3):
        super().__init__(M, rtol=rtol, atol=0.0, max_iter=max_iter, warm_start=False, chebyshev=chebyshev,
                         patch_columns=patch_columns)


class _NativeDirect:

    _ORDERINGS = {None: -1, "auto": -1, "longest-axis": 0, "trial-cuts": 1}

    def __init__(self, csr, leaf_size, arity, tier_levels, sparse_leaves, shard=(0, 1), ordering=None, tier_waves=0, refactorable=False):
        self.device = csr.device
        self._h = ctypes.c_void_p(None)
        pos = csr.positions
        if pos is not None:
            pos = pos.detach().to(torch.float32).contiguous()
        dev = csr.device
        if ordering not in self._ORDERINGS:
            raise ValueError(f"ordering must be one of {sorted(k for k in self._ORDERINGS if k)} or None, got {ordering!r}")
        if tier_waves not in (0, 4, 8, 16):
            raise ValueError(f"tier_waves must be 0 (the library's rule), 4, 8 or 16, got {tier_waves!r}")
        lib = _native.lib()
        opt = _native.DirectOptions()
        _native.check(lib.ls_direct_options_default(ctypes.byref(opt)))
        opt.leaf_size, opt.arity, opt.tier_levels, opt.sparse_leaves = int(leaf_size or 0), int(arity or 0), int(tier_levels), int(bool(sparse_leaves))
        opt.shard_rank, opt.shard_count = int(shard[0]), int(shard[1])
        opt.ordering, opt.tier_waves = self._ORDERINGS[ordering], int(tier_waves)
        factor = lib.ls_direct_factor_refactorable if refactorable else lib.ls_direct_factor_ex
        with torch.cuda.device(dev):
            _native.check(factor(_native.ptr(csr.rowptr), _native.ptr(csr.col), _native.ptr(csr.val), csr.V, csr.nnz,
                                 _native.ptr(pos), ctypes.byref(opt), dev.index, _native.stream_of(dev), ctypes.byref(self._h)))
        self.factored = True
        yes, kept = ctypes.c_int(0), ctypes.c_size_t(0)
        _native.check(lib.ls_direct_refactorable(self._h, ctypes.byref(yes), ctypes.byref(kept)))
        self.refactorable, self.retained_bytes = bool(yes.value), int(kept.value)
        s3 = (ctypes.c_double * 3)()
        _native.check(_native.lib().ls_direct_factor_seconds(self._h, ctypes.byref(s3)))
        self.timings = dict(plan_seconds=s3[0], table_seconds=s3[1], factor_seconds=s3[2])
        self.tier_levels = int(tier_levels)
        self._solve = _native.lib().ls_direct_solve
        o, w, sp, wo = ctypes.c_int(0), ctypes.c_double(0), ctypes.c_double(0), ctypes.c_double(0)
        _native.check(_native.lib().ls_direct_plan_quality(self._h, ctypes.byref(o), ctypes.byref(w), ctypes.byref(sp), ctypes.byref(wo)))
        self.plan_quality = dict(ordering="trial-cuts" if o.value == 1 else "longest-axis", words_per_vertex=w.value, spread=sp.value,
                                 words_per_vertex_other=wo.value)

    def close(self):
        h = getattr(self, "_h", None)
        if h is not None and h.value:
            try:
                _native.lib().ls_direct_destroy(h)
            except Exception:
                pass
        self._h = ctypes.c_void_p(None)

    def __del__(self):
        self.close()

    def solve(self, b, x):
        if not self._h.value:
            raise RuntimeError("this solver was closed")
        rc = self._solve(self._h, b.data_ptr(), x.data_ptr(), b.shape[1], _native.raw_stream(self.device))
        if rc:
            _native.check(rc)

    def refactor(self, csr):
        if not self._h.value:
            raise RuntimeError("this solver was closed")
        with torch.cuda.device(self.device):
            rc = _native.lib().ls_direct_refactor(self._h, _native.ptr(csr.rowptr), _native.ptr(csr.col), _native.ptr(csr.val), csr.V, csr.nnz,
                                                  _native.stream_of(self.device))
        self.factored = rc == 0 or (self.factored and (rc == _native.LS_E_STATE or "the factor is unchanged" in _native.last_error()))
        _native.check(rc)

    def set_option(self, name, value):
        _native.check(_native.lib().ls_direct_set(self._h, name.encode(), int(value)))

    def info(self):
        fe, nl = ctypes.c_int64(0), ctypes.c_int(0)
        ms = (ctypes.c_double * 3)()
        _native.check(_native.lib().ls_direct_info(self._h, ctypes.byref(fe), ctypes.byref(nl), ms))
        lv, ar, th, tw = ctypes.c_int(0), ctypes.c_int(0), ctypes.c_int(0), ctypes.c_int(0)
        wu, wd, nb = ctypes.c_int64(0), ctypes.c_int64(0), ctypes.c_int64(0)
        _native.check(_native.lib().ls_direct_shape(self._h, ctypes.byref(lv), ctypes.byref(ar), ctypes.byref(th), ctypes.byref(tw),
                                                    ctypes.byref(wu), ctypes.byref(wd), ctypes.byref(nb)))
        return dict(factor_entries=fe.value, launches=nl.value, up_ms=ms[0], down_ms=ms[1], mid_ms=ms[2], levels=lv.value, arity=ar.value,
                    tier_levels=th.value, tier_workgroups=tw.value, words_up=wu.value, words_down=wd.value, n_bnd=nb.value)


    def level_words(self):
        n = self.info()["levels"]
        up, down = (ctypes.c_int64 * n)(), (ctypes.c_int64 * n)()
        _native.check(_native.lib().ls_direct_level_words(self._h, n, up, down))
        return list(up), list(down)

    def level_rows(self):
        n = self.info()["levels"]
        rows, bnd = (ctypes.c_int64 * n)(), (ctypes.c_int64 * n)()
        _native.check(_native.lib().ls_direct_level_rows(self._h, n, rows, bnd))
        return list(rows), list(bnd)

    def level_index_bytes(self):
        n = self.info()["levels"]
        up, down = (ctypes.c_int64 * n)(), (ctypes.c_int64 * n)()
        _native.check(_native.lib().ls_direct_level_index_bytes(self._h, n, up, down))
        return list(up), list(down)

    def tier_balance(self):
        w = (ctypes.c_double * 4)()
        _native.check(_native.lib().ls_direct_tier_balance(self._h, ctypes.byref(w)))
        tot_max, tot_mean = w[0] + w[2], w[1] + w[3]
        return dict(up_max=w[0], up_mean=w[1], down_max=w[2], down_mean=w[3], max_over_mean=(tot_max / tot_mean if tot_mean else None))

    def launch_profile(self):
        n = ctypes.c_int(0)
        _native.check(_native.lib().ls_direct_launch_profile(self._h, 0, ctypes.byref(n), None, None, None, None, None))
        ms, words = (ctypes.c_double * n.value)(), (ctypes.c_int64 * n.value)()
        lo, hi, sw = (ctypes.c_int32 * n.value)(), (ctypes.c_int32 * n.value)(), (ctypes.c_int32 * n.value)()
        _native.check(_native.lib().ls_direct_launch_profile(self._h, n.value, ctypes.byref(n), ms, words, lo, hi, sw))
        return [dict(ms=ms[i], words=words[i], levels=(lo[i], hi[i]), sweep=("up", "down", "both")[sw[i]]) for i in range(n.value)]


def release_scratch(device=None):
    idx = -1 if device is None else (device.index if isinstance(device, torch.device) else int(device))
    _native.check(_native.lib().ls_release_scratch(-1 if idx is None else idx))


_DIRECT_INFO = types.MappingProxyType(dict(iterations=0, converged=True, method="nested-dissection"))


def _refactor_operand(M_new, V, nnz, device, who):
    if not isinstance(M_new, torch.Tensor) or M_new.layout != torch.sparse_coo:
        raise TypeError(f"{who}: expected a torch sparse COO matrix (as returned by largesteps.geometry.compute_matrix)")
    if M_new.dim() != 2 or tuple(M_new.shape) != (V, V):
        raise ValueError(f"{who}: the new matrix has shape {tuple(M_new.shape)}, the solver's is ({V}, {V}) -- a new pattern needs a new solver")
    _native.require_device(M_new, "the new matrix")
    if M_new.device != device:
        raise RuntimeError(f"{who}: the solver lives on {device}, the new matrix on {M_new.device}")
    if nnz is not None and M_new.is_coalesced() and M_new._nnz() != nnz:
        raise ValueError(f"{who}: the new matrix has {M_new._nnz()} entries, the solver's pattern {nnz} -- a new pattern needs a new solver")
    return _native.csr_of(M_new)


class NestedDissectionSolver(Solver):

    AUTO_TRIAL_CUTS_AFTER = 1500
    _served = {}
    _suspect = {}

    @staticmethod
    def _size_class(V):
        import math
        return int(round(8.0 * math.log2(max(int(V), 1))))

    def _surface_key(self, csr):
        key = getattr(self, "_surface_key_cached", None)
        if key is None:
            box = ()
            if csr.positions is not None and csr.V:
                import math
                p = csr.positions.detach()
                ext = (p.amax(0) - p.amin(0)).tolist()
                box = tuple(int(round(4.0 * math.log2(e))) if e > 0 and math.isfinite(e) else -999 for e in ext)
            key = self._surface_key_cached = self._class_key + box
        return key

    def __init__(self, M, leaf_size=None, arity=None, shard=(0, 1), ordering=None, tier_waves=0, refactorable=False):
        import time
        csr = _native.csr_of(M)
        self.generation = 0
        self._csr = csr
        self.last_info = None
        self.solves_served = 0
        self._class_key = (csr.device.index, self._size_class(csr.V))
        self.ordering_requested = ordering
        if ordering is None and not os.environ.get("LS_ND_ORDER"):
            if 100_000 <= csr.V <= 600_000 and self._served.get(self._class_key, 0) >= self.AUTO_TRIAL_CUTS_AFTER:
                ordering = "trial-cuts"
            elif self._suspect.get(self._surface_key(csr)):
                ordering = "trial-cuts"
        self.ordering_used = ordering
        if not _native.is_symmetric(csr):
            raise ValueError("NestedDissectionSolver: the matrix is not symmetric")
        t0 = time.perf_counter()
        tier = max(-1, min(6, int(os.environ.get("LS_ND_TIER_H", "-1"))))
        sparse = not os.environ.get("LS_ND_DENSE_LEAVES")
        self._direct = _NativeDirect(csr, leaf_size, arity, tier, sparse, shard=shard, ordering=ordering, tier_waves=tier_waves,
                                     refactorable=refactorable)
        self.refactorable = self._direct.refactorable
        self.retained_bytes = self._direct.retained_bytes
        torch.cuda.synchronize(csr.device)
        self.build_seconds = time.perf_counter() - t0
        self.timings = self._direct.timings
        self.plan_quality = self._direct.plan_quality
        if self.ordering_requested is None and self.ordering_used is None:
            if len(self._suspect) > 64:
                self._suspect.clear()
            self._suspect[self._surface_key(csr)] = self.plan_quality["ordering"] == "trial-cuts"

    @_native.retry_on_oom
    def solve(self, b, backward=False):
        _native.require_device(b, "b")
        if b.device != self._csr.device:
            raise RuntimeError(f"matrix ({self._csr.device}) and b ({b.device}) must be on the same device")
        if b.dtype != torch.float32:
            raise TypeError(f"b must be float32, got {b.dtype}")
        if b.dim() not in (1, 2) or b.shape[0] != self._csr.V:
            raise ValueError(f"Invalid right-hand side shape {tuple(b.shape)}: expected ({self._csr.V}, k)")
        squeeze = b.dim() == 1
        self.solves_served += 1
        if not squeeze and b.is_contiguous():
            b32 = b
            x = torch.empty(b.shape, dtype=torch.float32, device=b.device)
        else:
            b32 = (b.detach().unsqueeze(1) if squeeze else b.detach()).contiguous()
            x = torch.empty_like(b32)
        if b32.shape[1] <= _KMAX:
            self._direct.solve(b32, x)
        else:
            for c0 in range(0, b32.shape[1], _KMAX):
                c1 = min(b32.shape[1], c0 + _KMAX)
                xb = torch.empty((b32.shape[0], c1 - c0), dtype=torch.float32, device=b32.device)
                self._direct.solve(b32[:, c0:c1].contiguous(), xb)
                x[:, c0:c1] = xb
        self.last_info = _DIRECT_INFO
        return x.squeeze(1) if squeeze else x

    def refactor(self, M_new):
        csr = _refactor_operand(M_new, self._csr.V, self._csr.nnz, self._csr.device, "NestedDissectionSolver.refactor")
        if not self.refactorable:
            raise RuntimeError("NestedDissectionSolver.refactor: this solver was constructed with refactorable=False")
        if not _native.is_symmetric(csr):
            raise ValueError("NestedDissectionSolver.refactor: the matrix is not symmetric")
        self._direct.refactor(csr)
        self._csr = csr
        self.generation += 1

    @property
    def factored(self):
        return self._direct.factored
# ... 138 lines not shown
```

Measured before the change: 5217 solves/s.

## Add wave-owned tier plan to drop barrier between leaf and parent phases

Adds an 'owned' layout of the tier kernel's work lists, used only when the tier runs with 16 waves. Each wave gets the leaves and their parent nodes as a contiguous run, so the leaf phase and the parent phase that follows it can be separated by workgroup memory fences instead of a full __syncthreads. The goal is to remove one workgroup barrier per sweep and the idle time it causes across waves. In exchange, the per-workgroup header doubles to 256 bytes, the planner does more work and may fall back to the old plan, and the kernel adds one extra barrier after the dense gather whenever the owned form is in use.

```diff
diff --git a/include/largesteps_hip.h b/include/largesteps_hip.h
--- a/include/largesteps_hip.h
+++ b/include/largesteps_hip.h
@@ -143,6 +143,8 @@
 int ls_direct_pick_tree(int64_t V, int* leaf_size, int* arity);
 int ls_direct_tier_lds_bytes(int levels, int arity, const int32_t* h_s, const int32_t* h_b, const int32_t* h_own_start, int tier_levels,
                              int sparse_leaves, int waves, size_t* h_bytes);
+int ls_direct_tier_owned_layout(int levels, int arity, const int32_t* h_s, const int32_t* h_b, const int32_t* h_own_start, int tier_levels,
+                                int sparse_leaves, int waves, int64_t cap_rows, int32_t* h_out, int64_t* h_rows, size_t* h_bytes);
 int ls_direct_factor(const int32_t* d_rowptr, const int32_t* d_col, const float* d_val, int64_t V, int64_t nnz,
                      const float* d_positions, int leaf_size, int arity, int tier_levels, int sparse_leaves, int shard_rank,
                      int shard_count, int device, void* stream, ls_direct** out);
@@ -163,6 +165,7 @@
 int ls_release_scratch(int device);
 int ls_direct_shape(const ls_direct* d, int* h_levels, int* h_arity, int* h_tier_levels, int* h_tier_workgroups,
                     int64_t* h_words_up, int64_t* h_words_down, int64_t* h_n_bnd);
+int ls_direct_tier_form(const ls_direct* d, int* h_has_owned, int* h_owned, int* h_two_item_parents);
 int ls_direct_level_words(const ls_direct* d, int cap, int64_t* h_up, int64_t* h_down);
 int ls_direct_level_rows(const ls_direct* d, int cap, int64_t* h_rows, int64_t* h_bnd);
 int ls_direct_level_index_bytes(const ls_direct* d, int cap, int64_t* h_up, int64_t* h_down);
diff --git a/large-steps-pytorch_amd/csrc/direct.hip b/large-steps-pytorch_amd/csrc/direct.hip
--- a/large-steps-pytorch_amd/csrc/direct.hip
+++ b/large-steps-pytorch_amd/csrc/direct.hip
@@ -741,6 +741,9 @@
     int* pull = nullptr;
     int64_t pull_base = 0;
     TierWG* d_wgs = nullptr;
+    TierWG* d_wgs_owned = nullptr;
+    bool tier_owned = false;
+    int tier_two_item = 0;
     hipEvent_t busy = nullptr;
     hipStream_t last_stream = nullptr;
     bool used = false;
@@ -877,10 +880,58 @@
     return LS_OK;
 }
 
+static bool plan_tier_owned(const std::vector<int64_t>& level_off, int levels, int arity, int root, int64_t q, int wg, int waves, const TierWG& g,
+                            std::vector<TierItem>& items, std::vector<int64_t>& item_node, TierWG& o, std::vector<int32_t>* rows) {
+    const int H = levels - root;
+    o = g;
+    if (waves != TIER_WAVES_FULL || H < 2) return false;
+    if (!(g.up_leaf & 1u) || !((g.down_leaf >> (H - 1)) & 1u) || ((g.up_leaf >> 1) & 1u) || ((g.down_leaf >> (H - 2)) & 1u)) return false;
+    if (((g.up_split >> 1) & 1u) || ((g.down_split >> (H - 2)) & 1u)) return false;
+    int64_t P = 1;
+    for (int t = root; t < levels - 2; ++t) P *= arity;
+    if (P > waves && P % waves) return false;
+    const int64_t per = P <= waves ? 1 : P / waves, first = level_off[levels - 2] + q * P;
+    auto wave_of = [&](int64_t node, bool leaf) { return (int)(((leaf ? level_off[levels - 2] + (node - level_off[levels - 1]) / arity : node) - first) / per); };
+    const size_t mark = items.size();
+    for (int sweep = 0; sweep < 2; ++sweep) {
+        const bool up = sweep == 0;
+        const int* off = up ? g.up_off : g.down_off;
+        const int leaf_p = up ? 0 : H - 1, par_p = up ? 1 : H - 2;
+        const int base = (int)items.size();
+        for (int w = 0; w < waves; ++w) {
+            const int begin = (int)items.size() - base;
+            int cnt[2] = {0, 0};
+            for (int half = 0; half < 2; ++half) {
+                const bool leaf = up ? half == 0 : half == 1;
+                const int p = leaf ? leaf_p : par_p;
+                for (int k = off[p]; k < off[p + 1]; ++k) {
+                    if (wave_of(item_node[(size_t)k], leaf) != w) continue;
+                    const TierItem it = items[(size_t)k];
+                    const int64_t node = item_node[(size_t)k];
+                    items.push_back(it); item_node.push_back(node);
+                    ++cnt[leaf ? 0 : 1];
+                    if (rows) { rows->push_back(wg); rows->push_back(w); rows->push_back(up ? (leaf ? 0 : 1) : (leaf ? 3 : 2)); rows->push_back((int32_t)node); }
+                }
+            }
+            if (begin > 0xffff || cnt[0] > 0xff || cnt[1] > 0xff) { items.resize(mark); item_node.resize(mark); if (rows) rows->clear(); o = g; return false; }
+            (up ? o.own_up : o.own_down)[w] = (unsigned)begin | (unsigned)cnt[0] << 16 | (unsigned)cnt[1] << 24;
+        }
+        if (up) { o.up_off[0] = base; o.up_off[1] = (int)items.size(); }
+        else { o.down_off[H - 1] = base; o.down_off[H] = (int)items.size(); }
+    }
+    o.owned = 1;
+    return true;
+}
+
 static size_t plan_tier(const std::vector<NodeD>& nd, const std::vector<int64_t>& level_off, int levels, int arity, int root, int64_t q_lo,
-                        int64_t q_hi, std::vector<TierItem>& items, std::vector<TierWG>& wgs, int& vec_floats, int& tri_floats, int waves = TIER_WAVES) {
+                        int64_t q_hi, std::vector<TierItem>& items, std::vector<TierWG>& wgs, int& vec_floats, int& tri_floats, int waves = TIER_WAVES,
+                        std::vector<TierWG>* wgs_owned = nullptr, std::vector<int32_t>* owned_rows = nullptr) {
     const int H = levels - root;
     items.clear(); wgs.assign((size_t)(q_hi - q_lo), TierWG());
+    std::vector<int64_t> item_node;
+    bool all_owned = wgs_owned != nullptr;
+    if (wgs_owned) wgs_owned->assign(wgs.size(), TierWG());
+    if (owned_rows) owned_rows->clear();
     int vec_need = 0, pbuf_need = 0, leaf_need = 0, tri_cap = 0;
     for (int64_t i = level_off[levels - 1]; i < level_off[levels]; ++i)
         if (nd[i].flags & NODE_SPARSE) {
@@ -891,7 +942,8 @@
     for (int64_t q = q_lo; q < q_hi; ++q) {
         TierWG& g = wgs[(size_t)(q - q_lo)];
         g.up_split = g.down_split = g.up_leaf = g.down_leaf = 0;
-        g.n_dense = 0; g.pad = 0;
+        g.n_dense = 0; g.owned = 0;
+        for (int w = 0; w < TIER_WAVES_FULL; ++w) g.own_up[w] = g.own_down[w] = 0;
         for (int t = 0; t < 2 * TIER_MAX_H; ++t) g.dense_rng[t] = 0;
         for (int lv = root, t = 0; lv < levels - 1; ++lv, ++t) {
             int64_t span = 1;
@@ -929,7 +981,7 @@
                     it.pfront_off = n.pfront_off; it.cix = n.cix; it.flags = n.flags | (lv > root ? NODE_UPC : 0); it.finv_off = n.finv_off; it.w_off = n.w_off;
                     it.spb_off = n.spb_off; it.sps_off = n.sps_off; it.nparts = 1;
                     if (n.flags & NODE_SPARSE) {
-                        items.push_back(it);
+                        items.push_back(it); item_node.push_back(i);
                         leaf_need = std::max(leaf_need, std::max(tri_cap, (4 * n.b + 3) & ~3) + 256);
                         continue;
                     }
@@ -941,7 +993,7 @@
                         for (int pt = 0; pt < nparts; ++pt) {
                             it.row0 = r; it.r0 = (int)((int64_t)(L / 4) * pt / nparts) * 4; it.r1 = (int)((int64_t)(L / 4) * (pt + 1) / nparts) * 4;
                             it.part = pt; it.nparts = nparts;
-                            items.push_back(it);
+                            items.push_back(it); item_node.push_back(i);
                             vec_need = std::max(vec_need, 4 * (it.r1 - it.r0 + 32));
                         }
                     if (nparts > 1) { if (up) g.up_split |= 1u << ph; else g.down_split |= 1u << ph; }
@@ -953,13 +1005,20 @@
             }
             off[H] = (int)items.size();
         }
+        if (all_owned && !plan_tier_owned(level_off, levels, arity, root, q, (int)(q - q_lo), waves, g, items, item_node, (*wgs_owned)[(size_t)(q - q_lo)], owned_rows))
+            all_owned = false;
+    }
+    if (wgs_owned && !all_owned) {
+        wgs_owned->clear(); if (owned_rows) owned_rows->clear();
+        return plan_tier(nd, level_off, levels, arity, root, q_lo, q_hi, items, wgs, vec_floats, tri_floats, waves);
     }
     vec_floats = (vec_need + 3) & ~3;
     return (size_t)std::max(vec_floats + pbuf_need, leaf_need);
 }
 
 
-static size_t direct_tier_lds(int levels, int arity, const int* s, const int* b, const int* own_start, int tier_levels, bool sparse_leaves, int waves) {
+static size_t direct_tier_lds(int levels, int arity, const int* s, const int* b, const int* own_start, int tier_levels, bool sparse_leaves, int waves,
+                              std::vector<int32_t>* owned_rows = nullptr) {
     std::vector<int64_t> level_off((size_t)levels + 1);
     int64_t cnt = 1, off = 1;
     for (int lv = 0; lv <= levels; ++lv) { level_off[lv] = off; off += cnt; cnt *= arity; }
@@ -975,9 +1034,10 @@
             q.flags = (lv + 1 >= levels ? NODE_LEAF : 0) | (sparse ? NODE_SPARSE : NODE_QUAD);
         }
     std::vector<TierItem> items;
-    std::vector<TierWG> wgs;
+    std::vector<TierWG> wgs, wgs_owned;
     int vec = 0, tri = 0;
-    const size_t region = plan_tier(nd, level_off, levels, arity, root, 0, level_off[root + 1] - level_off[root], items, wgs, vec, tri, waves);
+    const size_t region = plan_tier(nd, level_off, levels, arity, root, 0, level_off[root + 1] - level_off[root], items, wgs, vec, tri, waves,
+                                    owned_rows ? &wgs_owned : nullptr, owned_rows);
     return region ? ((region + 3) & ~(size_t)3) * sizeof(float) * waves : 0;
 }
 
@@ -994,6 +1054,20 @@
                tier_levels >= 1 && tier_levels <= levels && tier_levels <= TIER_MAX_H && (waves == TIER_WAVES || waves == TIER_WAVES_WIDE || waves == TIER_WAVES_FULL),
                LS_E_INVALID, "ls_direct_tier_lds_bytes: bad argument (1 <= tier_levels <= min(levels, %d); waves 4, 8 or 16)", TIER_MAX_H);
     *h_bytes = direct_tier_lds(levels, arity, h_s, h_b, h_own_start, tier_levels, sparse_leaves != 0, waves);
+    return LS_OK;
+}
+
+extern "C" int ls_direct_tier_owned_layout(int levels, int arity, const int32_t* h_s, const int32_t* h_b, const int32_t* h_own_start, int tier_levels,
+                                           int sparse_leaves, int waves, int64_t cap_rows, int32_t* h_out, int64_t* h_rows, size_t* h_bytes) {
+    LS_REQUIRE(h_s && h_b && h_own_start && h_rows && cap_rows >= 0 && (h_out || !cap_rows) && levels >= 1 && levels <= 30 && (arity == 2 || arity == 4 || arity == 8) &&
+               tier_levels >= 1 && tier_levels <= levels && tier_levels <= TIER_MAX_H && (waves == TIER_WAVES || waves == TIER_WAVES_WIDE || waves == TIER_WAVES_FULL),
+               LS_E_INVALID, "ls_direct_tier_owned_layout: bad argument (1 <= tier_levels <= min(levels, %d); waves 4, 8 or 16)", TIER_MAX_H);
+    std::vector<int32_t> rows;
+    const size_t bytes = direct_tier_lds(levels, arity, h_s, h_b, h_own_start, tier_levels, sparse_leaves != 0, waves, &rows);
+    *h_rows = (int64_t)(rows.size() / 4);
+    if (h_bytes) *h_bytes = bytes;
+    LS_REQUIRE(cap_rows == 0 || (int64_t)(rows.size() / 4) <= cap_rows, LS_E_WORKSPACE, "ls_direct_tier_owned_layout: %lld rows needed", (long long)(rows.size() / 4));
+    if (cap_rows && !rows.empty()) memcpy(h_out, rows.data(), rows.size() * sizeof(int32_t));
     return LS_OK;
 }
 
@@ -1013,7 +1087,7 @@
     std::vector<int> parent;
     std::vector<unsigned char> mask;
     std::vector<TierItem> items;
-    std::vector<TierWG> wgs;
+    std::vector<TierWG> wgs, wgs_owned;
     std::vector<int> pull;
     std::vector<Tile> tiles;
     std::vector<PackedTile> ptiles;
@@ -1109,11 +1183,11 @@
     size_t region = 0;
     auto take_if_fits = [&](int waves, int budget) {
         std::vector<TierItem> items;
-        std::vector<TierWG> wgs;
+        std::vector<TierWG> wgs, wgs_owned;
         int vec = 0, tri = 0;
-        const size_t r = plan_tier(T.nd, T.level_off, levels, T.arity, root, q_lo, q_hi, items, wgs, vec, tri, waves);
+        const size_t r = plan_tier(T.nd, T.level_off, levels, T.arity, root, q_lo, q_hi, items, wgs, vec, tri, waves, &wgs_owned);
         if (!r || ((r + 3) & ~(size_t)3) * sizeof(float) * waves > (size_t)budget) return;
-        T.items.swap(items); T.wgs.swap(wgs); d->tier_vec = vec; d->tier_tri = tri; region = r; d->tier_waves = waves;
+        T.items.swap(items); T.wgs.swap(wgs); T.wgs_owned.swap(wgs_owned); d->tier_vec = vec; d->tier_tri = tri; region = r; d->tier_waves = waves;
     };
     if (H <= TIER_MAX_H && direct_tier_full16(d->V, T.arity, levels, H, d->shard_count, tier_waves > 0 ? tier_waves : env.tier_waves.value_or(0)))
         take_if_fits(TIER_WAVES_FULL, TIER_LDS_FULL);
@@ -1126,6 +1200,9 @@
         if (H >= 2 && (int)T.wgs.size() <= 768 && (tier_waves > 0 ? tier_waves : env.tier_waves.value_or(TIER_WAVES_WIDE)) == TIER_WAVES_WIDE)
             take_if_fits(TIER_WAVES_WIDE, TIER_LDS_WIDE);
     }
+    if (H >= 2)
+        for (int64_t i = T.level_off[levels - 2]; i < T.level_off[levels - 1]; ++i)
+            if (T.active(i, levels - 2) && T.nd[i].b > WAVE) ++d->tier_two_item;
     d->tier_root = root; d->tier_phases = H; d->tier_wgs = (int)T.wgs.size(); d->tier_region = (int)((region + 3) & ~(size_t)3);
     d->pull_base = T.nd[T.level_off[root]].front_off;
     T.pull.assign((size_t)std::max<int64_t>(0, T.nd[T.level_off[levels - 1]].front_off - d->pull_base) * T.arity, -1);
@@ -1379,6 +1456,10 @@
         (rc = up(&d->d_items, T.items.data(), T.items.size())) || (rc = up(&d->pull, T.pull.data(), T.pull.size())) ||
         (rc = up(&d->d_wgs, T.wgs.data(), T.wgs.size())))
         return rc;
+    if (!T.wgs_owned.empty()) {
+        if ((rc = up(&d->d_wgs_owned, T.wgs_owned.data(), T.wgs_owned.size()))) return rc;
+        d->tier_owned = true;
+    }
     hipError_t e = table((void**)&d->bp, sizeof(float) * (size_t)V * d->kmax);
     if (e == hipSuccess) e = table((void**)&d->braw, sizeof(float) * (size_t)V * d->kmax);
     if (e == hipSuccess) e = table((void**)&d->slots, sizeof(float) * (size_t)n_front * d->arity * d->kmax);
@@ -1433,7 +1514,7 @@
 static int direct_solve_k(ls_direct* d, const float* b, float* x, hipStream_t st, int part, float* exchange) {
     const int top = d->tier_root - 1;
     TierArgs ta;
-    ta.items = d->d_items; ta.wgs = d->d_wgs; ta.perm = d->perm; ta.mask = d->mask; ta.ppos = d->ppos;
+    ta.items = d->d_items; ta.wgs = d->tier_owned && d->d_wgs_owned ? d->d_wgs_owned : d->d_wgs; ta.perm = d->perm; ta.mask = d->mask; ta.ppos = d->ppos;
     ta.pull = d->pull ? d->pull - (size_t)d->pull_base * d->arity : nullptr; ta.push_ptr = d->push_ptr; ta.push_tgt = d->push_tgt; ta.u4 = d->u4; ta.d4 = d->d4; ta.tri = d->tri;
     ta.sp_ptr = d->sp_ptr; ta.sp_ent = d->sp_ent; ta.bprime = d->bp; ta.braw = d->braw; ta.slots = d->slots; ta.xb = d->xb;
     ta.arity = d->arity; ta.phases = d->tier_phases; ta.region_floats = d->tier_region; ta.vec_floats = d->tier_vec;
@@ -1630,6 +1711,11 @@
         d->nt_tier = value < 0 ? d->nt_rule[1] : value != 0;
         return LS_OK;
     }
+    if (!strcmp(name, "tier_owned")) {
+        LS_REQUIRE(value <= 0 || d->d_wgs_owned, LS_E_INVALID, "ls_direct_set: this plan has no owned form of the tier (ls_direct_tier_form)");
+        d->tier_owned = value != 0 && d->d_wgs_owned;
+        return LS_OK;
+    }
     set_error("ls_direct_set: unknown option '%s'", name);
     return LS_E_INVALID;
 }
@@ -1690,6 +1776,14 @@
     return LS_OK;
 }
 
+extern "C" int ls_direct_tier_form(const ls_direct* d, int* h_has_owned, int* h_owned, int* h_two_item_parents) {
+    LS_REQUIRE(d, LS_E_INVALID, "ls_direct_tier_form: bad argument");
+    if (h_has_owned) *h_has_owned = d->d_wgs_owned ? 1 : 0;
+    if (h_owned) *h_owned = d->tier_owned && d->d_wgs_owned ? 1 : 0;
+    if (h_two_item_parents) *h_two_item_parents = d->tier_two_item;
+    return LS_OK;
+}
+
 extern "C" int ls_direct_factor_seconds(const ls_direct* d, double* h_s3) {
     LS_REQUIRE(d && h_s3, LS_E_INVALID, "ls_direct_factor_seconds: bad argument");
     for (int i = 0; i < 3; ++i) h_s3[i] = d->factor_s[i];
diff --git a/large-steps-pytorch_amd/csrc/nd_tier.h b/large-steps-pytorch_amd/csrc/nd_tier.h
--- a/large-steps-pytorch_amd/csrc/nd_tier.h
+++ b/large-steps-pytorch_amd/csrc/nd_tier.h
@@ -37,10 +37,11 @@
     int down_off[TIER_MAX_H + 1];
     unsigned up_split, down_split;
     unsigned up_leaf, down_leaf;
-    int n_dense, pad;
+    int n_dense, owned;
     int dense_rng[2 * TIER_MAX_H];
+    unsigned own_up[TIER_WAVES_FULL], own_down[TIER_WAVES_FULL];
 };
-static_assert(sizeof(TierWG) == 128, "TierWG layout (read as 32 dwords)");
+static_assert(sizeof(TierWG) == 256, "TierWG layout (read as 64 dwords)");
 
 struct TierArgs {
     const TierItem* items;
@@ -368,13 +369,12 @@
 }
 
 template <int K, bool UP, int W, bool NT>
-__device__ __forceinline__ void leaf_phase(const TierArgs& a, int k0, int k1, const float* __restrict__ b_in, float* __restrict__ x_out,
+__device__ __forceinline__ void leaf_phase(const TierArgs& a, int k0, int k1, int S, const float* __restrict__ b_in, float* __restrict__ x_out,
                                            float* region, int tri_floats, long long* stamp_base) {
     const int lane = threadIdx.x & 63;
     int leaf_no = 0;
     (void)leaf_no; (void)stamp_base;
     if (k0 >= k1) return;
-    constexpr int S = W;
     TierItem it = rec_unpack(rec_load(a.items, k0, lane));
     int rec_n = k0 + S < k1 ? rec_load(a.items, k0 + S, lane) : 0;
     LeafIdx ix;
@@ -674,6 +674,22 @@
     wave_lds_sync();
 }
 
+struct WaveRun { int k0, k1, st; };
+template <bool UP, int W>
+__device__ __forceinline__ WaveRun wave_run(int hdr, int obase, int p, int wave, bool owned, int own_p, unsigned own_w) {
+    WaveRun r;
+    if (owned && (p == own_p || p == own_p + 1)) {
+        const int base = rl(hdr, obase + (UP ? own_p : own_p + 1)) + (int)(own_w & 0xffffu), nl = (int)((own_w >> 16) & 0xffu), nn = (int)(own_w >> 24);
+        const bool leaf_half = UP ? p == own_p : p != own_p;
+        r.k0 = leaf_half ? (UP ? base : base + nn) : (UP ? base + nl : base);
+        r.k1 = r.k0 + (leaf_half ? nl : nn);
+        r.st = 1;
+    } else {
+        r.k0 = rl(hdr, obase + p) + wave; r.k1 = rl(hdr, obase + p + 1); r.st = W;
+    }
+    return r;
+}
+
 template <int K, bool UP, int W, bool NT>
 __global__ __launch_bounds__(64 * W, 16 / W) void k_nd_tier(TierArgs a, const float* __restrict__ b_in, float* __restrict__ x_out,
                                                               int tri_floats) {
@@ -690,9 +706,12 @@
     long long* stamp_base = nullptr;
 #endif
     LS_STAMP(0);
-    const int hdr = lane < 32 ? reinterpret_cast<const int*>(a.wgs + sub)[lane] : 0;
+    const int hdr = reinterpret_cast<const int*>(a.wgs + sub)[lane];
     const int obase = UP ? 0 : TIER_MAX_H + 1;
     const unsigned split = (unsigned)rl(hdr, UP ? 14 : 15), leafy = (unsigned)rl(hdr, UP ? 16 : 17);
+    const bool owned = rl(hdr, 19) != 0;
+    const int own_p = UP ? 0 : a.phases - 2;
+    const unsigned own_w = owned ? (unsigned)rl(hdr, (UP ? 32 : 48) + wave) : 0u;
     if (UP) {
         const int n_dense = rl(hdr, 18);
         for (int r = threadIdx.x; r < n_dense; r += blockDim.x) {
@@ -713,6 +732,7 @@
 #pragma unroll
             for (int q = 0; q < K; ++q) a.braw[(size_t)r * K + q] = b_in[g * K + q];
         }
+        if (owned) __syncthreads();
     }
     LS_STAMP(1);
     DensePre<K> pre;
@@ -726,25 +746,25 @@
     TierItem it_pre = rec_unpack(0);
     bool pre_valid = false;
     for (int ph = 0; ph < a.phases; ++ph) {
-        const int i0 = rl(hdr, obase + ph), i1 = rl(hdr, obase + ph + 1);
+        const WaveRun run = wave_run<UP, W>(hdr, obase, ph, wave, owned, own_p, own_w);
         int rec_nx = 0;
         bool has_nx = false;
         if (ph + 1 < a.phases && !((leafy >> (ph + 1)) & 1u)) {
-            const int j0 = rl(hdr, obase + ph + 1) + wave;
-            has_nx = j0 < rl(hdr, obase + ph + 2);
-            if (has_nx) rec_nx = rec_load(a.items, j0, lane);
+            const WaveRun nx = wave_run<UP, W>(hdr, obase, ph + 1, wave, owned, own_p, own_w);
+            has_nx = nx.k0 < nx.k1;
+            if (has_nx) rec_nx = rec_load(a.items, nx.k0, lane);
         }
         if ((leafy >> ph) & 1u) {
-            leaf_phase<K, UP, W, NT>(a, i0 + wave, i1, b_in, x_out, region, tri_floats, stamp_base);
+            leaf_phase<K, UP, W, NT>(a, run.k0, run.k1, run.st, b_in, x_out, region, tri_floats, stamp_base);
         } else {
-            int rec = (!pre_valid && i0 + wave < i1) ? rec_load(a.items, i0 + wave, lane) : 0;
+            int rec = (!pre_valid && run.k0 < run.k1) ? rec_load(a.items, run.k0, lane) : 0;
             int head_k = -1, head_idx = 0, head_p0 = 0, head_p1 = 0, head_flags = 0;
-            for (int k = i0 + wave; k < i1; k += W) {
-                const int rec_next = k + W < i1 ? rec_load(a.items, k + W, lane) : 0;
-                const bool first = k == i0 + wave && pre_valid;
+            for (int k = run.k0; k < run.k1; k += run.st) {
+                const int rec_next = k + run.st < run.k1 ? rec_load(a.items, k + run.st, lane) : 0;
+                const bool first = k == run.k0 && pre_valid;
                 const TierItem it = first ? it_pre : rec_unpack(rec);
                 rec = rec_next;
-                float* pbuf = region + a.vec_floats + ((k - i0) / W) * 256;
+                float* pbuf = region + a.vec_floats + ((k - run.k0) / run.st) * 256;
                 if (!first) { if (UP) node_up_pre<K, NT>(a, it, pre); else node_down_pre<K, NT>(a, it, pre); }
                 if (UP) node_up<K, NT>(a, it, pre, b_in, region, pbuf);
                 else node_down<K, NT>(a, it, pre, x_out, region, pbuf);
@@ -758,6 +778,7 @@
 #pragma unroll
                 for (int c = 0; c < 4; ++c) head_tg[c] = (!UP && head_k >= 0 && head_p0 + c < head_p1 && !(head_flags & NODE_LEAF)) ? a.push_tgt[head_p0 + c] : -1;
                 __syncthreads();
+                const int i0 = run.k0 - wave, i1 = run.k1;
                 for (int k = i0 + wave; k < i1; k += W) {
                     const bool mine = k == head_k;
                     const TierItem it = rec_unpack(mine ? rec_head : rec_load(a.items, k, lane));
@@ -782,7 +803,7 @@
                 }
             }
         }
-        if (ph < 6) { LS_STAMP(2 + 2 * ph); LS_STAMP_VAL(24 + ph, (i1 - i0 - wave + W - 1) / W); }
+        if (ph < 6) { LS_STAMP(2 + 2 * ph); LS_STAMP_VAL(24 + ph, (run.k1 - run.k0 + run.st - 1) / run.st); }
         pre_valid = has_nx;
         it_pre = rec_unpack(rec_nx);
         if (pre_valid) {
@@ -796,7 +817,12 @@
 #pragma unroll
             for (int c = 0; c < 4; ++c) { pre.plo[c] = -1; pre.plb[c] = -1; }
         }
-        __syncthreads();
+        if (owned && ph == own_p) {
+            __builtin_amdgcn_fence(__ATOMIC_RELEASE, "workgroup");
+            __builtin_amdgcn_fence(__ATOMIC_ACQUIRE, "workgroup");
+        } else {
+            __syncthreads();
+        }
         if (ph < 6) LS_STAMP(3 + 2 * ph);
     }
 }
diff --git a/large-steps-pytorch_amd/largesteps/_native.py b/large-steps-pytorch_amd/largesteps/_native.py
--- a/large-steps-pytorch_amd/largesteps/_native.py
+++ b/large-steps-pytorch_amd/largesteps/_native.py
@@ -113,6 +113,9 @@
     "ls_direct_tier_lds_bytes": (c_int, [c_int, c_int, c_void_p, c_void_p, c_void_p, c_int, c_int, c_int, ctypes.POINTER(c_size_t)]),
     "ls_direct_level_index_bytes": (c_int, [c_void_p, c_int, c_void_p, c_void_p]),
     "ls_direct_tier_balance": (c_int, [c_void_p, ctypes.POINTER(c_double * 4)]),
+    "ls_direct_tier_owned_layout": (c_int, [c_int, c_int, c_void_p, c_void_p, c_void_p, c_int, c_int, c_int, c_i64, c_void_p, ctypes.POINTER(c_i64),
+                                            ctypes.POINTER(c_size_t)]),
+    "ls_direct_tier_form": (c_int, [c_void_p, ctypes.POINTER(c_int), ctypes.POINTER(c_int), ctypes.POINTER(c_int)]),
     "ls_direct_level_rows": (c_int, [c_void_p, c_int, c_void_p, c_void_p]),
     "ls_direct_exchange_region": (c_int, [c_void_p, c_int, ctypes.POINTER(c_void_p), ctypes.POINTER(c_i64)]),
     "ls_dist_unique_id": (c_int, [c_void_p]),
diff --git a/large-steps-pytorch_amd/largesteps/solvers.py b/large-steps-pytorch_amd/largesteps/solvers.py
--- a/large-steps-pytorch_amd/largesteps/solvers.py
+++ b/large-steps-pytorch_amd/largesteps/solvers.py
@@ -254,8 +254,11 @@
         wu, wd, nb = ctypes.c_int64(0), ctypes.c_int64(0), ctypes.c_int64(0)
         _native.check(_native.lib().ls_direct_shape(self._h, ctypes.byref(lv), ctypes.byref(ar), ctypes.byref(th), ctypes.byref(tw),
                                                     ctypes.byref(wu), ctypes.byref(wd), ctypes.byref(nb)))
+        has, own, two = ctypes.c_int(0), ctypes.c_int(0), ctypes.c_int(0)
+        _native.check(_native.lib().ls_direct_tier_form(self._h, ctypes.byref(has), ctypes.byref(own), ctypes.byref(two)))
         return dict(factor_entries=fe.value, launches=nl.value, up_ms=ms[0], down_ms=ms[1], mid_ms=ms[2], levels=lv.value, arity=ar.value,
-                    tier_levels=th.value, tier_workgroups=tw.value, words_up=wu.value, words_down=wd.value, n_bnd=nb.value)
+                    tier_levels=th.value, tier_workgroups=tw.value, words_up=wu.value, words_down=wd.value, n_bnd=nb.value,
+                    tier_owned=own.value, tier_owned_plan=has.value, tier_two_item_parents=two.value)
 
 
     def level_words(self):
```

After: 5133 solves/s. 1.6% lower.
